# senresearch/BulkLMM.jl

Measured on AMD Instinct MI355X. Metric: trait x marker LOD tests/sec, higher is better.
Workload: dtype f64

## Files before the change

bulklmm.jl_amd/csrc/blmm_api.hip:

```cpp
#include "blmm_internal.h"
#include "fastmath.h"
#include <algorithm>
#include <cmath>
#include <cstddef>
#include <chrono>
#include <cstring>
#include <limits>
#include <cstdlib>
#include <mutex>

using namespace blmm;

namespace blmm {

int fail(blmm_ctx* ctx, int code, const std::string& msg) {
  if (ctx) ctx->err = msg;
  return code;
}

int ensure(blmm_ctx* ctx, DevBuf& b, size_t bytes) {
  if (&b == &ctx->outL) clear_last(ctx);
  if (&b == &ctx->outL || &b == &ctx->outP) ctx->last_P = nullptr;
  if (bytes == 0) bytes = 8;
  if (b.cap >= bytes) return BLMM_OK;
// ... 109 lines not shown
};

void phase_times(const blmm_ctx::EvSet& s, double out[6]) {
  for (int i = 0; i < 6; ++i) out[i] = 0.0;
  for (int i = 0; i + 1 < s.n && i < 5; ++i) { float ms = 0; (void)hipEventElapsedTime(&ms, s.e[i], s.e[i + 1]); out[i] = ms; }
  if (s.n >= 2) { float tot = 0; (void)hipEventElapsedTime(&tot, s.e[0], s.e[s.n - 1]); out[5] = tot; }
}

int to_rowmajor(blmm_ctx* ctx, const double* In, int n, int64_t ncols, double* Out, int npad, int64_t ld) {
  dim3 grid((unsigned)((ld + 31) / 32), (unsigned)((npad + 31) / 32));
  hipLaunchKernelGGL(k_to_rowmajor, grid, dim3(256), 0, ctx->stream, In, n, ncols, Out, npad, ld);
  hipError_t e = hipGetLastError();
  if (e != hipSuccess) return fail(ctx, BLMM_ERR_HIP, std::string("k_to_rowmajor: ") + hipGetErrorString(e));
  return BLMM_OK;
}

int fill(blmm_ctx* ctx, double* p, int64_t n, double v) {
  if (n <= 0) return BLMM_OK;
  hipLaunchKernelGGL(k_fill, dim3((unsigned)((n + 255) / 256)), dim3(256), 0, ctx->stream, p, n, v);
  hipError_t e = hipGetLastError();
  if (e != hipSuccess) return fail(ctx, BLMM_ERR_HIP, std::string("k_fill: ") + hipGetErrorString(e));
  return BLMM_OK;
}

int check_opts(blmm_ctx* ctx, const blmm_opts* o) {
  if (!o) return fail(ctx, BLMM_ERR_INVALID, "opts is NULL");
  if (o->decomp_scheme != BLMM_EIGEN && o->decomp_scheme != BLMM_SVD)
    return fail(ctx, BLMM_ERR_DECOMP, "Please choose either `eigen` or `svd` for decomposition of the kinship matrix.");
  return BLMM_OK;
}

int check_method(blmm_ctx* ctx, const blmm_opts* o) {
  if (o->method != BLMM_NULL_EXACT && o->method != BLMM_NULL_GRID && o->method != BLMM_ALT_GRID)
    return fail(ctx, BLMM_ERR_METHOD, "Unknown method; choose null-exact, null-grid or alt-grid.");
  return BLMM_OK;
}

int reset_stat(blmm_ctx* ctx, int64_t** stat) {
  int rc = ensure(ctx, ctx->stat, sizeof(int64_t) * NSTAT);
  if (rc) return rc;
  *stat = ptr<int64_t>(ctx->stat);
  ctx->audit_ran = false;
  ctx->brent_cnt_used = false;
  BLMM_HIP(hipMemsetAsync(*stat, 0, sizeof(int64_t) * NSTAT, ctx->stream));
  return BLMM_OK;
}

int fill_status(blmm_ctx* ctx, const int64_t* h, blmm_status* st) {
  std::memset(st, 0, sizeof(*st));
  st->n_neg_eig = h[ST_NEG_EIG];
  st->n_nonpos_weight = h[ST_NONPOS_W];
  st->n_zero_norm = h[ST_ZERO_NORM];
  st->n_nan_lod = h[ST_NAN_LOD];
  st->n_brent_maxiter = h[ST_BRENT_MAXIT];
  st->jacobi_sweeps = h[ST_JACOBI_SWEEPS];
  st->jacobi_cycles = h[ST_EIG_CYCLES]; st->jacobi_ticks_100mhz = h[ST_EIG_TICKS];
  st->lowrank_rank = h[ST_LR_RANK];
  st->lowrank_fallback = h[ST_LR_FIX];
  st->lowrank_shared = h[ST_LR_SHARED0] + h[ST_LR_SHARED1];
  st->n_h2_boundary = h[ST_H2_BOUNDARY];
  st->n_h2_multimodal = ctx->audit_ran ? h[ST_H2_MULTIMODAL] : -1;
  st->n_illcond_rescan = h[ST_ILLCOND];
  if (h[ST_LR_RANK] < 0) return fail(ctx, BLMM_ERR_HIP, "weight-basis kernel: a workgroup timed out at the grid barrier");
  if (h[ST_EIG_ABORT] != 0) return fail(ctx, BLMM_ERR_HIP, "the eigensolver did not converge (code " + std::to_string((long long)h[ST_EIG_ABORT]) +
                              ": -7 grid barrier of the tridiagonalisation timed out, -8 QL iteration limit)");
  if (ctx->hflag && *ctx->hflag) return check_sticky(ctx);
  { double r2; std::memcpy(&r2, &h[ST_LR_RESID2], sizeof(double)); st->lowrank_resid = std::sqrt(r2 < 0 ? 0.0 : r2); }
  return BLMM_OK;
}

void add_status(blmm_status* sum, const blmm_status& one) {
  sum->n_neg_eig += one.n_neg_eig; sum->n_nonpos_weight += one.n_nonpos_weight; sum->n_zero_norm += one.n_zero_norm;
  sum->n_nan_lod += one.n_nan_lod; sum->n_brent_maxiter += one.n_brent_maxiter; sum->jacobi_sweeps += one.jacobi_sweeps;
  sum->jacobi_cycles += one.jacobi_cycles; sum->jacobi_ticks_100mhz += one.jacobi_ticks_100mhz;
  sum->lowrank_rank = std::max(sum->lowrank_rank, one.lowrank_rank);
  sum->lowrank_fallback += one.lowrank_fallback; sum->lowrank_shared += one.lowrank_shared;
  sum->lowrank_resid = std::max(sum->lowrank_resid, one.lowrank_resid);
  sum->n_h2_boundary += one.n_h2_boundary; sum->n_h2_multimodal += one.n_h2_multimodal; sum->n_illcond_rescan += one.n_illcond_rescan;
}

double add_phase_times(blmm_status* st, const Timer& tm) {
  if (!tm.set || tm.set->n < 2) return 0.0;
  double t[6];
  phase_times(*tm.set, t);
  st->t_eigen_ms += t[0]; st->t_rotate_ms += t[1]; st->t_h2_ms += t[2]; st->t_prep_ms += t[3]; st->t_scan_ms += t[4];
  return t[5];
}

int finish_status(blmm_ctx* ctx, blmm_status* st, Timer* tm) {
  if (!st) return BLMM_OK;
  int64_t h[NSTAT];
  BLMM_HIP(hipMemcpyAsync(h, ctx->stat.p, sizeof(h), hipMemcpyDeviceToHost, ctx->stream));
  BLMM_HIP(hipStreamSynchronize(ctx->stream));
  int rc = fill_status(ctx, h, st);
  if (rc) return rc;
  if (tm) st->t_total_ms = add_phase_times(st, *tm);
  return BLMM_OK;
}

int end_call(blmm_ctx* ctx, const Pipe& P, blmm_status* st, Timer* tm) {
  if (P.big && ctx->hflag && P.stat) {
    hipLaunchKernelGGL(k_sticky, dim3(1), dim3(1), 0, ctx->stream, P.stat, const_cast<int64_t*>(ctx->hflag));
    hipError_t e = hipGetLastError();
    if (e != hipSuccess) return fail(ctx, BLMM_ERR_HIP, std::string("k_sticky: ") + hipGetErrorString(e));
  }
  return finish_status(ctx, st, tm);
}

struct EigPre { double* Ks; double* V; double* lraw; int64_t* stat; };

struct NullCov { const double* d; int64_t ncov; int add_int; int64_t c; };
NullCov null_cov(const blmm_opts* o, const double* dCovar, int64_t ncov) {
  if (ncov == 0 || !dCovar) return {nullptr, 0, 1, 1};
  const int add_int = o->add_intercept ? 1 : 0;
  return {dCovar, ncov, add_int, ncov + add_int};
}

int prepare_eigen(blmm_ctx* ctx, const blmm_opts* o, int64_t n, const double* dCovar, int64_t ncov, const double* dK,
                  const double* dweights, int centered, Pipe& P, Timer& tm, const EigPre* pre = nullptr) {
  ctx->prep_valid = false;
  if (n < 1 || ncov < 0) return fail(ctx, BLMM_ERR_DIM, "Dimension mismatch.");
  if (n > 2048) return fail(ctx, BLMM_ERR_UNSUPPORTED, "more than 2048 individuals: the device eigensolver (tridiagonalisation + divide and conquer) stops at n = 2048");
  const NullCov nc = null_cov(o, dCovar, ncov);
  const int c = (int)nc.c;
  if (c < 1 || c > CMAX) return fail(ctx, BLMM_ERR_UNSUPPORTED, BLMM_C_ERR);
  if (c >= n) return fail(ctx, BLMM_ERR_DIM, "Dimension mismatch.");
  P.n = (int)n; P.c = c; P.npad = (int)round_up(n, 8); P.ldr = (int)round_up(P.npad, 16);
  int rc;
  if ((rc = ensure(ctx, ctx->U, sizeof(double) * n * n))) return rc;
  if ((rc = ensure(ctx, ctx->lam, sizeof(double) * n))) return rc;
  if ((rc = ensure(ctx, ctx->Zs, sizeof(double) * n * c))) return rc;
  if ((rc = ensure(ctx, ctx->Z0, sizeof(double) * n * c))) return rc;
  if ((rc = ensure(ctx, ctx->Rp, sizeof(double) * (size_t)P.npad * P.ldr))) return rc;
  P.Z0 = ptr<double>(ctx->Z0); P.lam = ptr<double>(ctx->lam);
  if (pre) {
    P.stat = pre->stat;
    ctx->audit_ran = false;
    ctx->brent_cnt_used = false;
    P.big = n > jacobi_lds_max_n();
    bool post_done = false;
    tm.mark();
    if ((rc = launch_jacobi_post(ctx, pre->Ks, pre->V, (int)n, pre->lraw, P.stat, ptr<double>(ctx->Zs), dweights, c, P.npad, P.ldr,
                                 o->decomp_scheme, centered, P.lam, ptr<double>(ctx->U), P.Z0, ptr<double>(ctx->Rp), &post_done))) return rc;
    if (!post_done && (rc = launch_post_eigen(ctx, pre->lraw, pre->V, ptr<double>(ctx->Zs), dweights, (int)n, c, P.npad, P.ldr,
                                              o->decomp_scheme, centered, P.lam, ptr<double>(ctx->U), P.Z0, ptr<double>(ctx->Rp), P.stat))) return rc;
    tm.mark();
    return BLMM_OK;
  }
  if ((rc = ensure(ctx, ctx->Ks, sizeof(double) * n * n))) return rc;
  if ((rc = ensure(ctx, ctx->V, sizeof(double) * (n * n + 4 * n + 16)))) return rc;
  if ((rc = ensure(ctx, ctx->lraw, sizeof(double) * n))) return rc;
  if ((rc = reset_stat(ctx, &P.stat))) return rc;
  tm.mark();
  if ((rc = launch_design(ctx, dK, nc.d, (int)nc.ncov, nc.add_int, dweights, (int)n, ptr<double>(ctx->Ks), ptr<double>(ctx->Zs)))) return rc;
  const double* evec = ptr<double>(ctx->V);
  const char* eig_env = dev_env("BLMM_EIGEN");
  if (!eig_env && ctx->tune.eigen_solver == 1) eig_env = "jacobi";
  if (!eig_env && ctx->tune.eigen_solver == 2) eig_env = "dc";
  const bool big = n > jacobi_lds_max_n();
  P.big = big;
  bool done = false, post_done = false;
  const bool want_dc = eig_env ? std::strcmp(eig_env, "dc") == 0 : big;
  if (!done && want_dc && n >= 3) {
    rc = launch_eig_dc(ctx, ptr<double>(ctx->Ks), (int)n, ptr<double>(ctx->lraw), ptr<double>(ctx->V), P.stat);
    if (rc == BLMM_OK) { done = true; P.big = true; }
    else if (rc != BLMM_ERR_UNSUPPORTED) return rc;
  }
  if (!done) {
    const bool want_fast = !(eig_env && std::strcmp(eig_env, "jacobi") == 0) && n >= 3 && n <= eig_fast_max_n();
    if (want_fast) {
      rc = launch_eig_fast(ctx, ptr<double>(ctx->Ks), (int)n, ptr<double>(ctx->lraw), ptr<double>(ctx->V), P.stat);
      if (rc != BLMM_OK && rc != BLMM_ERR_UNSUPPORTED) return rc;
    }
    if ((rc = launch_jacobi_post(ctx, ptr<double>(ctx->Ks), ptr<double>(ctx->V), (int)n, ptr<double>(ctx->lraw), P.stat, ptr<double>(ctx->Zs),
                                 dweights, c, P.npad, P.ldr, o->decomp_scheme, centered, P.lam, ptr<double>(ctx->U), P.Z0, ptr<double>(ctx->Rp),
                                 &post_done))) return rc;
  }
  if (!post_done && (rc = launch_post_eigen(ctx, ptr<double>(ctx->lraw), evec, ptr<double>(ctx->Zs), dweights, (int)n, c,
                              P.npad, P.ldr, o->decomp_scheme, centered, P.lam, ptr<double>(ctx->U), P.Z0,
                              ptr<double>(ctx->Rp), P.stat))) return rc;
  tm.mark();
  return BLMM_OK;
}

static int flush_upload(blmm_ctx* ctx) {
  if (!ctx->up_pending) return BLMM_OK;
  ctx->up_pending = false;
  for (int i = 0; i < 2; ++i) {
    if (ctx->up_bytes[i]) BLMM_HIP(hipMemcpyAsync(ctx->up_dst[i], ctx->up_src[i], ctx->up_bytes[i], hipMemcpyHostToDevice, ctx->copy));
    if (i == 0) BLMM_HIP(hipEventRecord(ctx->ev_inY, ctx->copy));
  }
  BLMM_HIP(hipEventRecord(ctx->ev_in, ctx->copy));
  ctx->in_wait = true;
  return BLMM_OK;
}

int rotate_markers(blmm_ctx* ctx, Pipe& P, const double* dG, int64_t p);
int start_wbasis(blmm_ctx* ctx, Pipe& P, const double* dG = nullptr, int64_t p = 0, bool xt_recorded = false) {
  int rc;
  const int64_t n = P.n;
  const LrSeg seg = lr_segments(ctx, P.n);
  if ((rc = ensure(ctx, ctx->wbQ, sizeof(double) * (size_t)seg.S * P.npad * n))) return rc;
  if ((rc = ensure(ctx, ctx->wbW, sizeof(double) * (size_t)n * (256 + 16)))) return rc;
  if ((rc = ensure(ctx, ctx->wbRk, sizeof(int) * 4 * LR_SEG_MAX))) return rc;
  if (!xt_recorded) BLMM_HIP(hipEventRecord(ctx->ev_xt, ctx->stream));
  BLMM_HIP(hipStreamWaitEvent(ctx->side, ctx->ev_xt, 0));
  ctx->wb_on_side2 = false;
  if (!dG) {
    OnStream on(ctx, ctx->side);
    return launch_wbasis(ctx, P.lam, (int)n, P.npad, seg, ptr<double>(ctx->wbW), ptr<double>(ctx->wbQ), ptr<int>(ctx->wbRk), P.stat);
  }
  {
    BLMM_HIP(hipStreamWaitEvent(ctx->side2, ctx->ev_xt, 0));
    ctx->wb_on_side2 = true;
    OnStream on(ctx, ctx->side2);
    if ((rc = launch_wbasis(ctx, P.lam, (int)n, P.npad, seg, ptr<double>(ctx->wbW), ptr<double>(ctx->wbQ), ptr<int>(ctx->wbRk), P.stat))) return rc;
  }
  OnStream on(ctx, ctx->side);
  if (ctx->in_wait) BLMM_HIP(hipStreamWaitEvent(ctx->side, ctx->ev_in, 0));
  if ((rc = rotate_markers(ctx, P, dG, p))) return rc;
  BLMM_HIP(hipEventRecord(ctx->ev_wb, ctx->side));
  return BLMM_OK;
}

int rotate_traits(blmm_ctx* ctx, Pipe& P, const double* dY, int64_t m) {
  if (m < 0) return fail(ctx, BLMM_ERR_DIM, "Dimension mismatch.");
  P.m = m; P.ldy = round_up(m > 0 ? m : 1, 128);
  int rc = ensure(ctx, ctx->Yt, sizeof(double) * (size_t)P.npad * P.ldy);
  if (rc) return rc;
  P.Yt = ptr<double>(ctx->Yt);
  return launch_rotate(ctx, ptr<double>(ctx->Rp), P.ldr, P.n, P.npad, dY, m, P.Yt, P.ldy, P.ldy);
}
int rotate_markers(blmm_ctx* ctx, Pipe& P, const double* dG, int64_t p) {
  if (p < 0) return fail(ctx, BLMM_ERR_DIM, "Dimension mismatch.");
  P.p = p; P.ldx = round_up(p > 0 ? p : 1, 128);
  int rc = ensure(ctx, ctx->Xt, sizeof(double) * (size_t)P.npad * P.ldx);
  if (rc) return rc;
  P.Xt = ptr<double>(ctx->Xt);
  return launch_rotate(ctx, ptr<double>(ctx->Rp), P.ldr, P.n, P.npad, dG, p, P.Xt, P.ldx, P.ldx);
}

int prepare(blmm_ctx* ctx, const blmm_opts* o, const double* dY, int64_t n, int64_t m, const double* dG, int64_t p,
            const double* dCovar, int64_t ncov, const double* dK, const double* dweights, int centered, Pipe& P, Timer& tm,
            bool early_wbasis = false, bool grid_side = false, bool skip_markers = false, const EigPre* pre = nullptr) {
  if (m < 0 || p < 0) return fail(ctx, BLMM_ERR_DIM, "Dimension mismatch.");
  const bool forks = m > 0 && p > 0 && (early_wbasis || grid_side);
  ctx->stop_event_used = false;
  ctx->stop_event_next = forks ? ctx->ev_xt : nullptr;
  int rc = prepare_eigen(ctx, o, n, dCovar, ncov, dK, dweights, centered, P, tm, pre);
  const bool xt_recorded = ctx->stop_event_used;
  ctx->stop_event_next = nullptr; ctx->stop_event_used = false;
  if (rc) return rc;
  if (ctx->up_pending) {
    if ((rc = flush_upload(ctx))) return rc;
    BLMM_HIP(hipStreamWaitEvent(ctx->stream, ctx->ev_inY, 0));
  }
  const bool up_flight = ctx->in_wait;
  static const bool rot_side = !(dev_env("BLMM_ROTATE_SIDE") && dev_env("BLMM_ROTATE_SIDE")[0] == '0');
  const bool side_g = early_wbasis && m > 0 && p > 0 && rot_side && n <= 160;
  if (early_wbasis && m > 0 && p > 0 && (rc = start_wbasis(ctx, P, side_g ? dG : nullptr, p, xt_recorded))) return rc;
  P.xt_side = side_g;
  if (grid_side && !early_wbasis && m > 0 && p > 0 && rot_side && n <= 160) {
    if (!xt_recorded) BLMM_HIP(hipEventRecord(ctx->ev_xt, ctx->stream));
    BLMM_HIP(hipStreamWaitEvent(ctx->side, ctx->ev_xt, 0));
    if (ctx->in_wait) BLMM_HIP(hipStreamWaitEvent(ctx->side, ctx->ev_in, 0));
    OnStream on(ctx, ctx->side);
    if ((rc = rotate_markers(ctx, P, dG, p))) return rc;
    P.xt_side = true;
  }
  if ((rc = rotate_traits(ctx, P, dY, m))) return rc;
  if (skip_markers) { P.p = p; P.ldx = round_up(p > 0 ? p : 1, 128); P.Xt = nullptr; }
  else if (!P.xt_side) {
    if (up_flight) BLMM_HIP(hipStreamWaitEvent(ctx->stream, ctx->ev_in, 0));
    if ((rc = rotate_markers(ctx, P, dG, p))) return rc;
  }
  ctx->in_wait = false;
  tm.mark();
  return BLMM_OK;
}

NullModel null_model(const Pipe& P, const blmm_opts* o) {
  NullModel nm;
  nm.n = P.n; nm.c = P.c; nm.npad = P.npad; nm.reml = o->reml ? 1 : 0;
  nm.optim_interval = o->optim_interval < 1 ? 1 : o->optim_interval;
  nm.prior_a = o->prior_variance; nm.prior_b = o->prior_sample_size;
  return nm;
}

int stage_to_device(blmm_ctx* ctx, DevBuf& dst, const void* src, size_t bytes) {
  blmm_ctx::GridSlot* slot = nullptr;
  for (auto& g : ctx->gstage)
    if (g.cap >= bytes && (!g.used || hipEventQuery(g.ev) == hipSuccess)) { slot = &g; break; }
  if (!slot) {
    blmm_ctx::GridSlot g;
    g.cap = bytes < 4096 ? 4096 : bytes;
    void* h = nullptr;
    BLMM_HIP(hipHostMalloc(&h, g.cap, hipHostMallocDefault));
    g.h = h;
    if (hipEventCreateWithFlags(&g.ev, hipEventDisableTiming) != hipSuccess) { (void)hipHostFree(h); return fail(ctx, BLMM_ERR_HIP, "hipEventCreate failed"); }
    ctx->gstage.push_back(g);
    slot = &ctx->gstage.back();
  }
  std::memcpy(slot->h, src, bytes);
  BLMM_HIP(hipMemcpyAsync(dst.p, slot->h, bytes, hipMemcpyHostToDevice, ctx->stream));
  BLMM_HIP(hipEventRecord(slot->ev, ctx->stream));
  slot->used = true;
  return BLMM_OK;
}

int check_grid(blmm_ctx* ctx, const double* h2_grid_host, int64_t ngrid) {
  if (!h2_grid_host || ngrid < 1) return fail(ctx, BLMM_ERR_INVALID, "h2 grid is empty");
  for (int64_t g = 0; g < ngrid; ++g) {
    const double h = h2_grid_host[g];
    if (std::isinf(h / (1.0 - h))) return fail(ctx, BLMM_ERR_H2_ONE, "Heritability of 1 is not allowed.");
  }
  return BLMM_OK;
}

int grid_to_device(blmm_ctx* ctx, const double* h2_grid_host, int64_t ngrid, double** out) {
  int rc;
  if ((rc = check_grid(ctx, h2_grid_host, ngrid)) || (rc = ensure(ctx, ctx->gridd, sizeof(double) * ngrid))) return rc;
  const size_t bytes = sizeof(double) * (size_t)ngrid;
  if (ctx->grid_async) {
    if ((rc = stage_to_device(ctx, ctx->gridd, h2_grid_host, bytes))) return rc;
  } else {
    BLMM_HIP(hipMemcpyAsync(ctx->gridd.p, h2_grid_host, bytes, hipMemcpyHostToDevice, ctx->stream));
    BLMM_HIP(hipStreamSynchronize(ctx->stream));
  }
  *out = ptr<double>(ctx->gridd);
  return BLMM_OK;
}

ScanArgs scan_args(blmm_ctx* ctx, const Pipe& P, const double* panels, int64_t ldp, double* L, int64_t ldL, int64_t m) {
  ScanArgs a;
  a.Xt = P.Xt; a.ldx = P.ldx; a.P = panels; a.ldp = ldp; a.pstride = (int64_t)P.npad * ldp;
  a.ks = P.npad / 4; a.n = P.n; a.p = P.p; a.m = m; a.L = L; a.ldL = ldL;
  a.isx = nullptr; a.ld_isx = 0; a.bin = nullptr; a.stat = P.stat; a.logtab = ptr<double>(ctx->logtab); a.lodtab = ptr<double>(ctx->lodtab);
  a.Pv = ctx->pv_cur; a.ldPv = ctx->pv_cur_ld; a.pvtab = ptr<double>(ctx->pvtab);
  a.red = ctx->red_cur;
  a.c = P.c;
  lod_poly5_host(-0.5 * (double)P.n, a.lodc);
  return a;
}

double lr_tolerance(const blmm_ctx* ctx) {
  const char* e = dev_env("BLMM_LR_TOL");
  return e ? atof(e) : ctx->tune.lr_tol;
}

int64_t lr_ldq(const Pipe& P) { return P.ldy + 128 + LR_TILE * LR_SEG_MAX; }
static LrRegion lr_region(const Pipe& P, int r) {
  LrRegion rg;
  rg.col0 = r * lr_ldq(P); rg.ncol = lr_ldq(P); rg.counts = P.stat + ST_LR_SHARED0 + 2 * r; rg.segcnt = P.stat + 24 + 20 * r;
  return rg;
}

int lr_begin(blmm_ctx* ctx, const Pipe& P, bool wbasis_started) {
  int rc;
  ctx->lr_last_ldq = lr_ldq(P); ctx->lr_last_m = P.m;
  const int64_t ldp = 2 * lr_ldq(P), tstride = (int64_t)P.npad * P.ldx;
  if ((rc = ensure(ctx, ctx->lrPerm, sizeof(int) * (size_t)ldp))) return rc;
  if ((rc = ensure(ctx, ctx->lrDen0, sizeof(double) * (size_t)P.ldx))) return rc;
  const LrSeg seg = lr_segments(ctx, P.n);
  if ((rc = ensure(ctx, ctx->lrT, sizeof(double) * (size_t)seg.S * (1 + P.c) * tstride))) return rc;
  if ((rc = ensure(ctx, ctx->lrC, sizeof(double) * (size_t)P.npad * ldp))) return rc;
  if ((rc = ensure(ctx, ctx->lrL, sizeof(double) * (size_t)(P.c * (P.c + 1) / 2) * ldp))) return rc;
  if ((rc = ensure(ctx, ctx->lrFlag, sizeof(int) * (size_t)ldp))) return rc;
  if ((rc = ensure(ctx, ctx->lrPart, sizeof(double) * 2 * (size_t)((P.n + 63) / 64) * ldp))) return rc;
  if ((rc = ensure(ctx, ctx->panels, sizeof(double) * (size_t)P.npad * ldp))) return rc;
  if ((rc = ensure(ctx, ctx->wbQ, sizeof(double) * (size_t)seg.S * P.npad * P.n))) return rc;
  if ((rc = ensure(ctx, ctx->wbW, sizeof(double) * (size_t)P.n * (256 + 16)))) return rc;
  if ((rc = ensure(ctx, ctx->wbRk, sizeof(int) * 4 * LR_SEG_MAX))) return rc;
  int* rk = ptr<int>(ctx->wbRk);
  if (!(wbasis_started && P.xt_side)) {
    BLMM_HIP(hipEventRecord(ctx->ev_fork, ctx->stream));
    BLMM_HIP(hipStreamWaitEvent(ctx->side, ctx->ev_fork, 0));
  }
  const bool on2 = wbasis_started && P.xt_side && ctx->wb_on_side2;
  hipStream_t lr_side = on2 ? ctx->side2 : ctx->side;
  OnStream on(ctx, lr_side);
  if (!wbasis_started && (rc = launch_wbasis(ctx, P.lam, P.n, P.npad, seg, ptr<double>(ctx->wbW), ptr<double>(ctx->wbQ), rk, P.stat))) return rc;
  BLMM_HIP(hipEventRecord(ctx->ev_q, lr_side));
  if (on2) BLMM_HIP(hipStreamWaitEvent(lr_side, ctx->ev_wb, 0));
  if ((rc = launch_lr_tpanels(ctx, P.Xt, P.ldx, P.p, P.n, P.c, P.npad, P.Z0, ptr<double>(ctx->wbQ), rk, seg, ptr<double>(ctx->lrT), tstride,
                              ptr<double>(ctx->lrDen0)))) return rc;
  BLMM_HIP(hipEventRecord(ctx->ev_join, lr_side));
  return BLMM_OK;
}

namespace {
double lr_shared_tol(const blmm_ctx* ctx) {
  const char* e = dev_env("BLMM_LR_SHARED");
  const bool on = e ? e[0] != '0' : ctx->tune.lr_shared != 0;
  return on ? lr_tolerance(ctx) : 0.0;
}
LrArgs lr_args(blmm_ctx* ctx, const Pipe& P, const LrRegion& rg, double* dL, int64_t ldL) {
  const int64_t ldp = 2 * lr_ldq(P);
  LrArgs la;
  la.s = scan_args(ctx, P, ptr<double>(ctx->panels), ldp, dL, ldL, P.m + 192 < rg.ncol ? P.m + 192 : rg.ncol);
  la.Cp = ptr<double>(ctx->lrC); la.T = ptr<double>(ctx->lrT); la.tstride = (int64_t)P.npad * P.ldx; la.Ls = ptr<double>(ctx->lrL);
  la.rk = ptr<int>(ctx->wbRk); la.c = P.c; la.perm = ptr<int>(ctx->lrPerm); la.rg = rg; la.den0 = ptr<double>(ctx->lrDen0);
  la.skip_shared = 0;
  la.seg = lr_segments(ctx, P.n);
  return la;
}
int lr_region_scan(blmm_ctx* ctx, const Pipe& P, const LrRegion& rg, double* dL, int64_t ldL) {
  static const bool lean = !(dev_env("BLMM_LR_LEAN") && dev_env("BLMM_LR_LEAN")[0] == '0');
  static const bool serial = dev_env("BLMM_LR_SERIAL") && dev_env("BLMM_LR_SERIAL")[0] == '1';
  if (serial) { (void)hipStreamSynchronize(ctx->side); (void)hipStreamSynchronize(ctx->side2); (void)hipStreamSynchronize(ctx->stream); }
  LrArgs la = lr_args(ctx, P, rg, dL, ldL);
  int rc;
  if (lean) {
    ScanArgs a = la.s;
    a.isx = la.den0; a.ld_isx = P.ldx; a.bin = nullptr;
    a.perm = la.perm; a.col0 = rg.col0; a.count = rg.counts;
    if ((rc = launch_scan_shared(ctx, a))) return rc;
    la.skip_shared = 1;
  }
  return launch_scan_lr(ctx, la);
}
int lr_region_panels(blmm_ctx* ctx, const Pipe& P, const NullModel& nm, const double* dh2, const LrRegion& rg) {
  return launch_lr_panels(ctx, nm, P.Yt, P.ldy, P.m, P.Z0, P.lam, dh2, ptr<double>(ctx->wbQ), ptr<int>(ctx->wbRk), lr_segments(ctx, P.n), ptr<int>(ctx->lrPerm),
                          rg, ptr<double>(ctx->panels), ptr<double>(ctx->lrC), ptr<double>(ctx->lrL), 2 * lr_ldq(P), P.stat);
// ... 173 lines not shown
      ensure(ctx, ctx->lodtab, sizeof(blmm_lod_table_host)) != BLMM_OK ||
      hipMemcpy(ctx->lodtab.p, blmm_lod_table_host, sizeof(blmm_lod_table_host), hipMemcpyHostToDevice) != hipSuccess ||
      ensure(ctx, ctx->pvtab, sizeof(blmm_pv_table_host)) != BLMM_OK ||
      hipMemcpy(ctx->pvtab.p, blmm_pv_table_host, sizeof(blmm_pv_table_host), hipMemcpyHostToDevice) != hipSuccess) {
    blmm_destroy(ctx);
    return BLMM_ERR_HIP;
  }
  *out = ctx;
  return BLMM_OK;
}

void blmm_destroy(blmm_ctx* ctx) {
  if (!ctx) return;
  hipSetDevice(ctx->device);
  hipStreamSynchronize(ctx->stream);
  DevBuf* bufs[] = {&ctx->Ks, &ctx->V, &ctx->lam, &ctx->U, &ctx->Zs, &ctx->Z0, &ctx->Rp, &ctx->Yt, &ctx->Xt, &ctx->panels,
                    &ctx->iyy, &ctx->h2, &ctx->h2idx, &ctx->sig2, &ctx->ell, &ctx->isx, &ctx->stat, &ctx->gridd, &ctx->misc,
                    &ctx->EllTab, &ctx->inY, &ctx->inG, &ctx->inK, &ctx->inCov, &ctx->inW, &ctx->outL, &ctx->outH2,
                    &ctx->tmpA, &ctx->tmpB, &ctx->tmpC, &ctx->perm, &ctx->r0, &ctx->altbuf, &ctx->logtab, &ctx->lraw,
                    &ctx->wbQ, &ctx->wbW, &ctx->wbRk, &ctx->lrT, &ctx->lrC, &ctx->lrL, &ctx->lrFlag, &ctx->lrPart, &ctx->lrPerm, &ctx->lrDen0, &ctx->eigW, &ctx->xf32, &ctx->pf32, &ctx->brSt, &ctx->brList, &ctx->illList, &ctx->qrSlab, &ctx->lodtab, &ctx->dynFac, &ctx->pvtab, &ctx->outP, &ctx->redbuf, &ctx->redtrip, &ctx->altC, &ctx->rf32, &ctx->btG, &ctx->redflag, &ctx->bperm,
                    &ctx->locoK, &ctx->locoPart, &ctx->locoChr, &ctx->locoStat, &ctx->locoKs, &ctx->locoV, &ctx->locoLraw,
                    &ctx->locoCmx, &ctx->locoCarg, &ctx->locoPerm, &ctx->mdfR, &ctx->mdfT, &ctx->mdfScr,
                    &ctx->effX, &ctx->effIdx, &ctx->effWork, &ctx->effOut, &ctx->effSlab, &ctx->condIdx, &ctx->condWork,
                    &ctx->stepWork, &ctx->stepOut, &ctx->condScr};
  for (DevBuf* b : bufs) if (b->p) hipFree(b->p);
  for (auto& s : ctx->evsets) for (auto& e : s.e) (void)hipEventDestroy(e);
  if (ctx->side) { (void)hipStreamSynchronize(ctx->side); (void)hipStreamDestroy(ctx->side); }
  if (ctx->ev_fork) (void)hipEventDestroy(ctx->ev_fork);
  if (ctx->ev_join) (void)hipEventDestroy(ctx->ev_join);
  if (ctx->ev_xt) (void)hipEventDestroy(ctx->ev_xt);
  if (ctx->ev_b1) (void)hipEventDestroy(ctx->ev_b1);
  if (ctx->ev_b2) (void)hipEventDestroy(ctx->ev_b2);
  if (ctx->ev_q) (void)hipEventDestroy(ctx->ev_q);
  if (ctx->ev_m) (void)hipEventDestroy(ctx->ev_m);
  if (ctx->ev_wb) (void)hipEventDestroy(ctx->ev_wb);
  if (ctx->ev_in) (void)hipEventDestroy(ctx->ev_in);
  if (ctx->ev_inY) (void)hipEventDestroy(ctx->ev_inY);
  if (ctx->ev_call) (void)hipEventDestroy(ctx->ev_call);
  for (auto& g : ctx->gstage) {
    if (g.ev) { (void)hipEventSynchronize(g.ev); (void)hipEventDestroy(g.ev); }
    if (g.h) (void)hipHostFree(g.h);
  }
  if (ctx->copy) { (void)hipStreamSynchronize(ctx->copy); (void)hipStreamDestroy(ctx->copy); }
  if (ctx->side2) { (void)hipStreamSynchronize(ctx->side2); (void)hipStreamDestroy(ctx->side2); }
  if (ctx->own_stream) hipStreamDestroy(ctx->stream);
  if (ctx->hflag) (void)hipHostFree(const_cast<int64_t*>(ctx->hflag));
  destroy_host_stage(ctx->hstage);
  delete ctx;
}

const char* blmm_last_error(const blmm_ctx* ctx) { return ctx ? ctx->err.c_str() : "ctx is NULL"; }

int blmm_set_stream(blmm_ctx* ctx, void* hip_stream) {
  if (!ctx) return BLMM_ERR_INVALID;
  hipStreamSynchronize(ctx->stream);
  if (ctx->own_stream) { hipStreamDestroy(ctx->stream); ctx->own_stream = false; }
  if (hip_stream == BLMM_STREAM_NULL) ctx->stream = nullptr;
  else if (hip_stream) ctx->stream = reinterpret_cast<hipStream_t>(hip_stream);
  else {
    if (hipStreamCreateWithFlags(&ctx->stream, hipStreamNonBlocking) != hipSuccess) return fail(ctx, BLMM_ERR_HIP, "hipStreamCreate");
    ctx->own_stream = true;
  }
  return BLMM_OK;
}

int blmm_set_timing(blmm_ctx* ctx, int on) {
  if (!ctx) return BLMM_ERR_INVALID;
  ctx->timing = on != 0;
  return BLMM_OK;
}

int blmm_read_timings(blmm_ctx* ctx, double* sums_ms, int64_t* ncalls) {
  if (!ctx || !sums_ms || !ncalls) return BLMM_ERR_INVALID;
  BLMM_HIP(hipStreamSynchronize(ctx->stream));
  for (int i = 0; i < 6; ++i) sums_ms[i] = 0.0;
  for (size_t k = 0; k < ctx->ev_used; ++k) {
    double t[6];
    phase_times(ctx->evsets[k], t);
    for (int i = 0; i < 6; ++i) sums_ms[i] += t[i];
  }
  *ncalls = (int64_t)ctx->ev_used;
  ctx->ev_used = 0;
  return BLMM_OK;
}

int blmm_lowrank_profile(blmm_ctx* ctx, int64_t* out) {
  if (!ctx || !out) return BLMM_ERR_INVALID;
  for (int i = 0; i < 2 + 2 * LR_SEG_MAX; ++i) out[i] = 0;
  if (!ctx->stat.p || !ctx->wbRk.p) return BLMM_OK;
  BLMM_HIP(hipSetDevice(ctx->device));
  int64_t h[NSTAT];
  int rk[4 * LR_SEG_MAX];
  BLMM_HIP(hipMemcpyAsync(h, ctx->stat.p, sizeof(h), hipMemcpyDeviceToHost, ctx->stream));
  BLMM_HIP(hipMemcpyAsync(rk, ctx->wbRk.p, sizeof(rk), hipMemcpyDeviceToHost, ctx->stream));
  BLMM_HIP(hipStreamSynchronize(ctx->stream));
  int S = 0;
  for (int s = 0; s < LR_SEG_MAX; ++s) {
    const int64_t cnt = h[24 + s] + h[44 + s];
    if (cnt > 0) { S = s + 1; out[2 + 2 * s] = cnt; out[3 + 2 * s] = rk[4 * s]; }
  }
  out[0] = S; out[1] = h[ST_LR_SHARED0] + h[ST_LR_SHARED1];
  return BLMM_OK;
}

int blmm_lowrank_columns(blmm_ctx* ctx, int64_t m, int32_t* col_out, int64_t* region_width, int64_t* counts_out) {
  if (!ctx || !col_out || m < 0) return BLMM_ERR_INVALID;
  for (int64_t j = 0; j < m; ++j) col_out[j] = -1;
  if (region_width) *region_width = ctx->lr_last_ldq;
  if (counts_out) for (int i = 0; i < 4; ++i) counts_out[i] = 0;
  if (!ctx->lrPerm.p || !ctx->stat.p || ctx->lr_last_ldq <= 0) return BLMM_OK;
  BLMM_HIP(hipSetDevice(ctx->device));
  const int64_t ldq = ctx->lr_last_ldq;
  std::vector<int> perm((size_t)(2 * ldq));
  int64_t h[NSTAT];
  BLMM_HIP(hipMemcpyAsync(perm.data(), ctx->lrPerm.p, sizeof(int) * perm.size(), hipMemcpyDeviceToHost, ctx->stream));
  BLMM_HIP(hipMemcpyAsync(h, ctx->stat.p, sizeof(h), hipMemcpyDeviceToHost, ctx->stream));
  BLMM_HIP(hipStreamSynchronize(ctx->stream));
  for (int r = 0; r < 2; ++r) {
    const int64_t nsh = h[ST_LR_SHARED0 + 2 * r], noth = h[ST_LR_OTHER0 + 2 * r];
    if (counts_out) { counts_out[2 * r] = nsh; counts_out[2 * r + 1] = noth; }
    for (int64_t cidx = 0; cidx < ldq; ++cidx) {
      if (!(cidx < nsh || cidx >= ldq - noth)) continue;
      const int t = perm[(size_t)(r * ldq + cidx)];
      if (t >= 0 && t < m) col_out[t] = (int32_t)(r * ldq + cidx);
    }
  }
  return BLMM_OK;
}

int blmm_synchronize(blmm_ctx* ctx) {
  if (!ctx) return BLMM_ERR_INVALID;
  BLMM_HIP(hipStreamSynchronize(ctx->stream));
  return check_sticky(ctx);
}

void blmm_default_opts(blmm_opts* o) {
  if (!o) return;
  std::memset(o, 0, sizeof(*o));
  o->method = BLMM_NULL_GRID; o->reml = 0; o->add_intercept = 1; o->decomp_scheme = BLMM_EIGEN;
  o->optim_interval = 1; o->compat_flags = 0; o->prior_variance = 1.0; o->prior_sample_size = 0.0;
}

static const struct { const char* key; int kind; size_t off; double lo, hi; } kTune[] = {
  {"lr_tol", 0, offsetof(blmm::Tuning, lr_tol), 0.0, 1.0},
  {"illcond_rho", 0, offsetof(blmm::Tuning, illcond_rho), 0.0, 1e300},
  {"exact_full_rank", 1, offsetof(blmm::Tuning, exact_full_rank), 0, 1},
  {"pval_libm", 1, offsetof(blmm::Tuning, pval_libm), 0, 1},
  {"pval_fused", 1, offsetof(blmm::Tuning, pval_fused), 0, 1},
  {"lr_segments", 1, offsetof(blmm::Tuning, lr_segments), 0, LR_SEG_MAX},
  {"lr_shared", 1, offsetof(blmm::Tuning, lr_shared), 0, 1},
  {"lr_split", 1, offsetof(blmm::Tuning, lr_split), -1, 1},
  {"eigen_solver", 1, offsetof(blmm::Tuning, eigen_solver), 0, 2},
  {"f32_rotation", 1, offsetof(blmm::Tuning, f32_rotation), 0, 1},
  {"bulk_perm_cols", 1, offsetof(blmm::Tuning, bulk_perm_cols), 0, 2147483647.0},
  {"mdf_red_chunk", 1, offsetof(blmm::Tuning, mdf_red_chunk), 0, 2147483647.0},
  {"cond_red_chunk", 1, offsetof(blmm::Tuning, cond_red_chunk), 0, 2147483647.0},
};
int blmm_set_tuning(blmm_ctx* ctx, const char* key, double value) {
  if (!ctx) return BLMM_ERR_INVALID;
  if (!key) return fail(ctx, BLMM_ERR_INVALID, "set_tuning: key is NULL");
  if (std::strcmp(key, "defaults") == 0) { ctx->tune = blmm::Tuning(); return BLMM_OK; }
  for (const auto& t : kTune)
    if (std::strcmp(key, t.key) == 0) {
      if (!(value >= t.lo && value <= t.hi) || (t.kind == 1 && value != std::floor(value)))
        return fail(ctx, BLMM_ERR_INVALID, std::string("set_tuning: value out of range for ") + key);
      char* base = reinterpret_cast<char*>(&ctx->tune) + t.off;
      if (t.kind == 0) *reinterpret_cast<double*>(base) = value; else *reinterpret_cast<int*>(base) = (int)value;
      return BLMM_OK;
    }
  return fail(ctx, BLMM_ERR_INVALID, std::string("set_tuning: unknown key ") + key);
}
int blmm_get_tuning(const blmm_ctx* ctx, const char* key, double* value) {
  if (!ctx || !key || !value) return BLMM_ERR_INVALID;
  for (const auto& t : kTune)
    if (std::strcmp(key, t.key) == 0) {
      const char* base = reinterpret_cast<const char*>(&ctx->tune) + t.off;
      *value = t.kind == 0 ? *reinterpret_cast<const double*>(base) : (double)*reinterpret_cast<const int*>(base);
      return BLMM_OK;
    }
  return BLMM_ERR_INVALID;
}

int blmm_kinship_dev(blmm_ctx* ctx, const double* dG, int64_t n, int64_t p, double* dK_out) {
  if (!ctx) return BLMM_ERR_INVALID;
  if (!dG || !dK_out || n < 1 || p < 1) return fail(ctx, BLMM_ERR_INVALID, "calcKinship: bad arguments");
  BLMM_HIP(hipSetDevice(ctx->device));
  int rc = ensure(ctx, ctx->tmpA, sizeof(double) * (size_t)64 * n * n);
  if (rc) return rc;
  return launch_kinship(ctx, dG, n, p, dK_out, ptr<double>(ctx->tmpA));
}

__global__ void k_round_digits(double* __restrict__ v, int64_t cnt, double scale) {
  const int64_t i = (int64_t)blockIdx.x * blockDim.x + threadIdx.x;
  if (i < cnt) v[i] = rint(v[i] * scale) / scale;
}

int blmm_kinship_rounded(blmm_ctx* ctx, const double* G, int64_t n, int64_t p, int64_t digits, double* K_out) {
  if (!ctx) return BLMM_ERR_INVALID;
  if (!G || !K_out || n < 1 || p < 1 || digits > 300) return fail(ctx, BLMM_ERR_INVALID, "calcKinship: bad arguments");
  HostCall hc(ctx);
  int rc;
  if ((rc = hc.begin()) || (rc = ensure(ctx, ctx->inK, sizeof(double) * n * n)) || (rc = hc.up(ctx->inG, G, sizeof(double) * n * p))) return rc;
  if ((rc = blmm_kinship_dev(ctx, ptr<double>(ctx->inG), n, p, ptr<double>(ctx->inK)))) return rc;
  if (digits >= 0 && digits <= 17)
    hipLaunchKernelGGL(k_round_digits, dim3((unsigned)((n * n + 255) / 256)), dim3(256), 0, ctx->stream, ptr<double>(ctx->inK), n * n, std::pow(10.0, (double)digits));
  if ((rc = hc.down(K_out, ctx->inK.p, sizeof(double) * n * n))) return rc;
  return hc.finish();
}

int blmm_kinship(blmm_ctx* ctx, const double* G, int64_t n, int64_t p, double* K_out) {
  return blmm_kinship_rounded(ctx, G, n, p, -1, K_out);
}

int blmm_lod_colmax_dev(blmm_ctx* ctx, const double* dL, int64_t p, int64_t m, int64_t ldL, double* dmax_out, int64_t* dargmax_out) {
  if (!ctx) return BLMM_ERR_INVALID;
  if (!dL || !dmax_out || p < 1 || m < 0 || ldL < p) return fail(ctx, BLMM_ERR_INVALID, "lod_colmax: bad arguments");
  BLMM_HIP(hipSetDevice(ctx->device));
  return launch_colmax(ctx, dL, p, m, ldL, dmax_out, dargmax_out);
}

int blmm_lod_colmax(blmm_ctx* ctx, const double* L, int64_t p, int64_t m, double* max_out, int64_t* argmax_out) {
  if (!ctx) return BLMM_ERR_INVALID;
  if (!L || !max_out || p < 1 || m < 0) return fail(ctx, BLMM_ERR_INVALID, "lod_colmax: bad arguments");
  HostCall hc(ctx);
  const size_t mm = m > 0 ? m : 1;
  int rc;
  if ((rc = hc.begin()) || (rc = hc.up(ctx->outL, L, sizeof(double) * (size_t)p * m)) || (rc = ensure(ctx, ctx->tmpA, sizeof(double) * mm)) ||
      (rc = ensure(ctx, ctx->tmpB, sizeof(int64_t) * mm))) return rc;
  if (m > 0) set_last(ctx, ptr<double>(ctx->outL), p, m);
  if ((rc = launch_colmax(ctx, ptr<double>(ctx->outL), p, m, p, ptr<double>(ctx->tmpA), ptr<int64_t>(ctx->tmpB))) ||
      (rc = hc.down(max_out, ctx->tmpA.p, sizeof(double) * (size_t)m)) || (rc = hc.down(argmax_out, ctx->tmpB.p, sizeof(int64_t) * (size_t)m)))
    return rc;
  return hc.finish();
}

int blmm_lod2log10p(blmm_ctx* ctx, const double* L, int64_t p, int64_t m, int64_t chisq_df, double* P_out) {
  if (!ctx) return BLMM_ERR_INVALID;
  if (!L || !P_out || p < 0 || m < 0 || chisq_df < 1 || chisq_df > 1000000) return fail(ctx, BLMM_ERR_INVALID, "lod2log10p: bad arguments");
  if ((size_t)p * m == 0) return BLMM_OK;
  HostCall hc(ctx);
  int rc;
  if ((rc = hc.begin()) || (rc = ensure(ctx, ctx->altbuf, sizeof(double) * (size_t)p * m * 2))) return rc;
  double* dL = ptr<double>(ctx->altbuf);
  double* dP = dL + (size_t)p * m;
  if ((rc = hc.up(dL, L, sizeof(double) * (size_t)p * m)) || (rc = launch_lod2log10p(ctx, dL, p, m, p, (int)chisq_df, dP, p)) ||
      (rc = copy_to_host(ctx, P_out, dP, sizeof(double) * (size_t)p * m))) return rc;
  return hc.finish(false);
}

int blmm_lod_threshold(blmm_ctx* ctx, const double* L, int64_t p, int64_t m, double thr, int64_t cap, int32_t* i_out,
                       int32_t* j_out, double* lod_out, int64_t* count_out) {
  if (!ctx) return BLMM_ERR_INVALID;
  if (!L || p < 1 || m < 1) return fail(ctx, BLMM_ERR_INVALID, "lod_threshold: bad arguments");
  HostCall hc(ctx);
  int rc;
  if ((rc = hc.begin()) || (rc = hc.up(ctx->outL, L, sizeof(double) * (size_t)p * m))) return rc;
  set_last(ctx, ptr<double>(ctx->outL), p, m);
  if ((rc = blmm_last_lod_threshold(ctx, thr, cap, i_out, j_out, lod_out, count_out))) return rc;
  return hc.finish(false);
}

int blmm_get_thresholds(blmm_ctx* ctx, const double* Lperms, int64_t p, int64_t nperms, const double* probs, int64_t nprobs,
                        double* thrs_out) {
  if (!ctx) return BLMM_ERR_INVALID;
  if (!Lperms || p < 1 || nperms < 1) return fail(ctx, BLMM_ERR_INVALID, "get_thresholds: bad arguments");
  HostCall hc(ctx);
  int rc;
  if ((rc = hc.begin()) || (rc = hc.up(ctx->altbuf, Lperms, sizeof(double) * (size_t)p * nperms)) ||
      (rc = blmm_get_thresholds_dev(ctx, ptr<double>(ctx->altbuf), p, nperms, p, probs, nprobs, thrs_out))) return rc;
  return hc.finish(false);
}

extern "C++" {
namespace {
struct PvReq { bool armed = false; double* out = nullptr; int64_t ld = 0, df = 1; };
PvReq pv_take(blmm_ctx* ctx) {
  PvReq r; r.armed = ctx->pv_armed; r.out = ctx->pv_out; r.ld = ctx->pv_ld; r.df = ctx->pv_df;
  ctx->pv_armed = false; ctx->pv_out = nullptr; ctx->pv_ld = 0; ctx->pv_df = 1;
  return r;
}
void pv_hand_over(blmm_ctx* ctx, const PvReq& r) {
  ctx->pv_armed = r.armed; ctx->pv_out = r.out; ctx->pv_ld = r.ld; ctx->pv_df = r.df;
}
struct PvCall {
  blmm_ctx* ctx; PvReq req; double* P = nullptr; int64_t ld = 0; bool fused = false, owned = false;
  PvCall(blmm_ctx* c, const PvReq& r) : ctx(c), req(r) {}
  ~PvCall() { ctx->pv_cur = nullptr; ctx->pv_cur_ld = 0; }
  int resolve(int64_t p, int64_t m) {
    if (!req.armed) return BLMM_OK;
    if (p <= 0 || m <= 0) return BLMM_OK;
    P = req.out; ld = req.ld;
    if (P && ld < p) { P = nullptr; return fail(ctx, BLMM_ERR_INVALID, "log10p output: ldP < p"); }
    if (!P) {
      int rc = ensure(ctx, ctx->outP, sizeof(double) * (size_t)p * (size_t)m);
      if (rc) return rc;
      P = ptr<double>(ctx->outP); ld = p; owned = true;
    }
    return BLMM_OK;
  }
  int begin(const Pipe& Pp, const blmm_opts* o) {
    int rc = resolve(Pp.p, Pp.m);
    if (rc || !P) return rc;
    const char* pf = dev_env("BLMM_PVAL_FUSED");
    fused = req.df == 1 && o->method != BLMM_ALT_GRID && (pf ? pf[0] != '0' : ctx->tune.pval_fused != 0);
    if (fused) { ctx->pv_cur = P; ctx->pv_cur_ld = ld; }
    return BLMM_OK;
  }
  int finish(int64_t p, int64_t m, const double* dL, int64_t ldL) {
    ctx->pv_cur = nullptr; ctx->pv_cur_ld = 0;
    if (!P) return BLMM_OK;
    if (!fused) { int rc = launch_lod2log10p(ctx, dL, p, m, ldL, (int)req.df, P, ld); if (rc) return rc; }
    if (owned) { ctx->last_P = P; ctx->last_P_ld = ld; ctx->last_P_df = req.df; }
    return BLMM_OK;
  }
};
}
}

static int isx_maybe_side(blmm_ctx* ctx, const Pipe& P, const NullModel& nm, const double* dgrid, int ngrid) {
  int rc;
  if ((rc = ensure(ctx, ctx->isx, sizeof(double) * (size_t)ngrid * P.ldx))) return rc;
  {
    OnStream on(ctx, P.xt_side ? ctx->side : ctx->stream);
    if ((rc = launch_isx(ctx, nm, P.Xt, P.ldx, P.p, P.Z0, P.lam, dgrid, ngrid, ptr<double>(ctx->isx), P.ldx, P.stat))) return rc;
  }
  if (P.xt_side) {
    BLMM_HIP(hipEventRecord(ctx->ev_join, ctx->side));
    BLMM_HIP(hipStreamWaitEvent(ctx->stream, ctx->ev_join, 0));
  }
  return BLMM_OK;
}

static int scan_pipeline(blmm_ctx* ctx, const blmm_opts* opts, Pipe& P, Timer& tm, bool lowrank, bool wbasis_started, double* dgrid,
                         const double* h2_grid_host, int64_t ngrid, double* dL_out, int64_t ldL, double* dh2_out, blmm_status* status,
                         const PvReq& pvreq, int64_t ldH = -1) {
  int rc;
  const int64_t m = P.m, p = P.p;
  const NullModel nm = null_model(P, opts);
  const int64_t ldp = P.ldy;
  PvCall pvc(ctx, pvreq);
  if ((rc = pvc.begin(P, opts))) return rc;
  if (m == 0) { tm.mark(); tm.mark(); tm.mark(); return end_call(ctx, P, status, &tm); }
  if (p == 0) {
    if (opts->method == BLMM_NULL_EXACT) {
      if ((rc = launch_brent(ctx, nm, P.Yt, P.ldy, m, P.Z0, P.lam, dh2_out, nullptr, nullptr, P.stat))) return rc;
    } else if (opts->method == BLMM_NULL_GRID) {
      if ((rc = ensure(ctx, ctx->h2idx, sizeof(int) * (size_t)m))) return rc;
      if ((rc = launch_loglik_grid(ctx, nm, P.Yt, P.ldy, m, P.Z0, P.lam, dgrid, (int)ngrid, nullptr, ptr<int>(ctx->h2idx), dh2_out, P.stat))) return rc;
    }
    tm.mark(); tm.mark(); tm.mark();
    return end_call(ctx, P, status, &tm);
  }

  if (opts->method == BLMM_NULL_EXACT) {
    if (lowrank) {
      if ((rc = lr_begin(ctx, P, wbasis_started))) return rc;
      const char* split_env = dev_env("BLMM_LR_SPLIT");
      const bool split_on = (ctx->red_cur.flags && P.c >= 2) ? false
                          : split_env ? split_env[0] != '0' : (ctx->tune.lr_split < 0 ? m >= 8192 : ctx->tune.lr_split != 0);
      BrentSplit sp;
      if ((rc = launch_brent(ctx, nm, P.Yt, P.ldy, m, P.Z0, P.lam, dh2_out, nullptr, nullptr, P.stat, split_on ? 1 : 0, &sp))) return rc;
      tm.mark();
      if (sp.active) { if ((rc = lr_finish_split(ctx, P, nm, dh2_out, dL_out, ldL, tm, sp))) return rc; }
      else if ((rc = lr_finish(ctx, P, nm, dh2_out, dL_out, ldL, tm))) return rc;
    } else {
      if ((rc = launch_brent(ctx, nm, P.Yt, P.ldy, m, P.Z0, P.lam, dh2_out, nullptr, nullptr, P.stat))) return rc;
      tm.mark();
      if ((rc = ensure(ctx, ctx->panels, sizeof(double) * (size_t)(2 + P.c) * P.npad * ldp))) return rc;
      if ((rc = launch_panels(ctx, nm, P.Yt, P.ldy, m, P.Z0, P.lam, dh2_out, 1, ptr<double>(ctx->panels), ldp, P.stat))) return rc;
      tm.mark();
      ScanArgs a = scan_args(ctx, P, ptr<double>(ctx->panels), ldp, dL_out, ldL, m);
      if ((rc = launch_scan_exact(ctx, a, P.c))) return rc;
      if ((rc = illcond_rescan(ctx, P, nm, m, dh2_out, dL_out, ldL))) return rc;
      tm.mark();
    }
    if (opts->compat_flags & BLMM_FLAG_H2_AUDIT) {
      double gridh[16];
      for (int g = 0; g < 16; ++g) gridh[g] = g / 16.0;
      double* dg = nullptr;
      if ((rc = grid_to_device(ctx, gridh, 16, &dg))) return rc;
      if ((rc = ensure(ctx, ctx->EllTab, sizeof(double) * (size_t)16 * m))) return rc;
      if ((rc = launch_loglik_grid(ctx, nm, P.Yt, P.ldy, m, P.Z0, P.lam, dg, 16, ptr<double>(ctx->EllTab), nullptr, nullptr, P.stat))) return rc;
      if ((rc = launch_h2_audit(ctx, ptr<double>(ctx->EllTab), 16, m, P.stat))) return rc;
      ctx->audit_ran = true;
    }
  } else if (opts->method == BLMM_NULL_GRID) {
    if ((rc = ensure(ctx, ctx->h2idx, sizeof(int) * (size_t)m))) return rc;
    if ((rc = launch_loglik_grid(ctx, nm, P.Yt, P.ldy, m, P.Z0, P.lam, dgrid, (int)ngrid, nullptr, ptr<int>(ctx->h2idx), dh2_out, P.stat))) return rc;
    tm.mark();
    if ((rc = ensure(ctx, ctx->panels, sizeof(double) * (size_t)P.npad * ldp))) return rc;
    if ((rc = launch_panels(ctx, nm, P.Yt, P.ldy, m, P.Z0, P.lam, dh2_out, 0, ptr<double>(ctx->panels), ldp, P.stat))) return rc;
    if ((rc = isx_maybe_side(ctx, P, nm, dgrid, (int)ngrid))) return rc;
    tm.mark();
    ScanArgs a = scan_args(ctx, P, ptr<double>(ctx->panels), ldp, dL_out, ldL, m);
    a.isx = ptr<double>(ctx->isx); a.ld_isx = P.ldx; a.bin = ptr<int>(ctx->h2idx);
    if ((rc = launch_scan_table(ctx, a))) return rc;
    tm.mark();
  } else {
    if ((rc = ensure(ctx, ctx->EllTab, sizeof(double) * (size_t)ngrid * m))) return rc;
    if ((rc = launch_loglik_grid(ctx, nm, P.Yt, P.ldy, m, P.Z0, P.lam, dgrid, (int)ngrid, ptr<double>(ctx->EllTab), nullptr, nullptr, P.stat))) return rc;
    tm.mark();
    if ((rc = ensure(ctx, ctx->panels, sizeof(double) * (size_t)ngrid * P.npad * ldp))) return rc;
    if ((rc = ensure(ctx, ctx->h2, sizeof(double) * (size_t)m))) return rc;
    if (nm.c <= CTPL) {
      if ((rc = launch_panels(ctx, nm, P.Yt, P.ldy, m, P.Z0, P.lam, nullptr, 0, ptr<double>(ctx->panels), ldp, P.stat, dgrid, (int)ngrid))) return rc;
    } else {
      for (int64_t g = 0; g < ngrid; ++g) {
        if ((rc = fill(ctx, ptr<double>(ctx->h2), m, h2_grid_host[g]))) return rc;
        if ((rc = launch_panels(ctx, nm, P.Yt, P.ldy, m, P.Z0, P.lam, ptr<double>(ctx->h2), 0,
                                ptr<double>(ctx->panels) + (size_t)g * P.npad * ldp, ldp, P.stat))) return rc;
      }
    }
    if ((rc = isx_maybe_side(ctx, P, nm, dgrid, (int)ngrid))) return rc;
    if ((rc = ensure(ctx, ctx->altC, sizeof(double) * (size_t)ngrid * m))) return rc;
    if ((rc = launch_alt_ctab(ctx, ptr<double>(ctx->EllTab), (int)ngrid, m, P.n, ptr<double>(ctx->altC)))) return rc;
    tm.mark();
    AltArgs aa;
    aa.s = scan_args(ctx, P, ptr<double>(ctx->panels), ldp, dL_out, ldL, m);
    aa.s.isx = ptr<double>(ctx->isx); aa.s.ld_isx = P.ldx;
    aa.ngrid = (int)ngrid; aa.EllTab = ptr<double>(ctx->EllTab); aa.grid_dev = dgrid; aa.H2 = dh2_out; aa.ldH = ldH < 0 ? p : ldH;
    aa.Ctab = ptr<double>(ctx->altC);
    aa.counter_quirk = (opts->compat_flags & BLMM_COMPAT_ALT_COUNTER) ? 1 : 0;
    if ((rc = launch_scan_alt(ctx, aa))) return rc;
    tm.mark();
  }
  if ((rc = pvc.finish(p, m, dL_out, ldL))) return rc;
  return end_call(ctx, P, status, &tm);
}

int blmm_set_log10p_output(blmm_ctx* ctx, double* dP_out, int64_t ldP, int64_t chisq_df) {
  if (!ctx) return BLMM_ERR_INVALID;
  if (chisq_df < 0 || chisq_df > 1000000 || (dP_out && ldP < 1)) return fail(ctx, BLMM_ERR_INVALID, "set_log10p_output: bad arguments");
  ctx->pv_armed = chisq_df > 0;
  ctx->pv_out = dP_out; ctx->pv_ld = ldP; ctx->pv_df = chisq_df > 0 ? chisq_df : 1;
  return BLMM_OK;
}

static bool exact_full(const blmm_ctx* ctx) {
  const char* e = dev_env("BLMM_EXACT");
  return e ? std::strcmp(e, "full") == 0 : ctx->tune.exact_full_rank != 0;
}
static bool lowrank_form(const blmm_ctx* ctx, int c, int64_t n) { return !exact_full(ctx) && c <= 3 && n <= 6000; }
static bool wants_lowrank(const blmm_ctx* ctx, const blmm_opts* opts, int64_t n, const double* dCovar, int64_t ncov) {
  return opts->method == BLMM_NULL_EXACT && lowrank_form(ctx, (int)null_cov(opts, dCovar, ncov).c, n);
}

static int bulkscan_dev_impl(blmm_ctx* ctx, const blmm_opts* opts, const double* dY, int64_t n, int64_t m, const double* dG,
                             int64_t p, const double* dCovar, int64_t ncov, const double* dK, const double* dweights,
                             const double* h2_grid_host, int64_t ngrid, double* dL_out, int64_t ldL, double* dh2_out,
                             blmm_status* status, const PvReq& pvreq) {
  int rc = check_opts(ctx, opts);
  if (rc) return rc;
  if (!dY || !dG || !dK || (!dL_out && !ctx->red_cur.pmax) || !dh2_out) return fail(ctx, BLMM_ERR_INVALID, "bulkscan: NULL buffer");
  if (ldL < p) return fail(ctx, BLMM_ERR_INVALID, "bulkscan: ldL < p");
  if ((rc = check_method(ctx, opts)) || (rc = enter_device(ctx))) return rc;
  Timer tm(ctx);
  Pipe P;
  double* dgrid = nullptr;
  if (opts->method != BLMM_NULL_EXACT) {
    if ((rc = grid_to_device(ctx, h2_grid_host, ngrid, &dgrid))) return rc;
  }
  const bool lowrank = wants_lowrank(ctx, opts, n, dCovar, ncov);
  if ((rc = prepare(ctx, opts, dY, n, m, dG, p, dCovar, ncov, dK, dweights, 1, P, tm, lowrank, opts->method != BLMM_NULL_EXACT))) return rc;
  return scan_pipeline(ctx, opts, P, tm, lowrank,  lowrank && m > 0 && p > 0, dgrid, h2_grid_host, ngrid, dL_out, ldL, dh2_out, status, pvreq);
}

int blmm_bulkscan_dev(blmm_ctx* ctx, const blmm_opts* opts, const double* dY, int64_t n, int64_t m, const double* dG,
                      int64_t p, const double* dCovar, int64_t ncov, const double* dK, const double* dweights,
                      const double* h2_grid_host, int64_t ngrid, double* dL_out, int64_t ldL, double* dh2_out,
                      blmm_status* status) {
  if (!ctx) return BLMM_ERR_INVALID;
  const PvReq pvreq = pv_take(ctx);
  ctx->red_cur = RedArgs();
  return bulkscan_dev_impl(ctx, opts, dY, n, m, dG, p, dCovar, ncov, dK, dweights, h2_grid_host, ngrid, dL_out, ldL, dh2_out, status, pvreq);
}

static int reduced_check(blmm_ctx* ctx, const blmm_opts* opts, const double* dY, int64_t n, int64_t m, const double* dG, int64_t p,
                         const double* dK, const blmm_reduced* out, const double* dh2_out, const char* who) {
  int rc = check_opts(ctx, opts);
  if (rc) return rc;
  if (!out || !dY || !dG || !dK || (!dh2_out && opts->method != BLMM_ALT_GRID)) return fail(ctx, BLMM_ERR_INVALID, std::string(who) + ": NULL buffer");
  if (out->cap < 0 || (out->cap > 0 && (!out->ti || !out->tj || !out->tlod)) || (out->want_triplets && !out->count))
    return fail(ctx, BLMM_ERR_INVALID, std::string(who) + ": triplet buffers");
  if ((rc = check_method(ctx, opts))) return rc;
  if (n < 1 || m < 0 || p < 0 || p > 0x7fffffffLL || m > 0x7fffffffLL) return fail(ctx, BLMM_ERR_DIM, "Dimension mismatch.");
  return BLMM_OK;
}

static int red_state(blmm_ctx* ctx, const blmm_reduced* out, int64_t nslot, int64_t m, RedArgs* r) {
  const int64_t ldm = round_up(m, 64);
  int rc = ensure(ctx, ctx->redbuf, (sizeof(double) + sizeof(int)) * (size_t)nslot * (size_t)ldm);
  if (rc) return rc;
  r->pmax = ptr<double>(ctx->redbuf); r->parg = reinterpret_cast<int*>(r->pmax + (size_t)nslot * ldm); r->ldm = ldm;
  r->want_trip = out->want_triplets ? 1 : 0; r->thr = out->thr; r->cap = out->cap;
  r->ti = out->ti; r->tj = out->tj; r->tl = out->tlod; r->cnt = reinterpret_cast<unsigned long long*>(out->count);
  if (out->count) BLMM_HIP(hipMemsetAsync(out->count, 0, sizeof(int64_t), ctx->stream));
  return BLMM_OK;
}
static int reduced_args(blmm_ctx* ctx, const blmm_reduced* out, int64_t p, int64_t m, RedArgs* r, int* nslot) {
  *nslot = 2 * (int)((p + 127) / 128);
  return red_state(ctx, out, *nslot, m, r);
}

static int reduced_resident(blmm_ctx* ctx, const blmm_opts* opts, const double* dY, int64_t n, int64_t m, const double* dG, int64_t p,
                            const double* dCovar, int64_t ncov, const double* dK, const double* dweights, const double* h2_grid_host,
                            int64_t ngrid, const blmm_reduced* out, double* dh2_out, blmm_status* status) {
  const int64_t ldL = p > 0 ? p : 1;
  const size_t pm = (size_t)ldL * (size_t)(m > 0 ? m : 1);
  int rc;
  if ((rc = ensure(ctx, ctx->outL, sizeof(double) * pm))) return rc;
  double* dL = ptr<double>(ctx->outL);
  double* dH = dh2_out;
  if (opts->method == BLMM_ALT_GRID) {
    if ((rc = ensure(ctx, ctx->altbuf, sizeof(double) * pm))) return rc;
    dH = ptr<double>(ctx->altbuf);
  }
  if ((rc = bulkscan_dev_impl(ctx, opts, dY, n, m, dG, p, dCovar, ncov, dK, dweights, h2_grid_host, ngrid, dL, ldL, dH, status, PvReq()))) return rc;
  if (m > 0) set_last(ctx, dL, p, m);
  if (out->colmax && m > 0 && (rc = launch_colmax(ctx, dL, p, m, ldL, out->colmax, out->argmax))) return rc;
  if (out->want_triplets && (rc = launch_threshold(ctx, dL, p, m, ldL, out->thr, out->cap, out->ti, out->tj, out->tlod, out->count))) return rc;
  return BLMM_OK;
}

static int reduced_impl(blmm_ctx* ctx, const blmm_opts* opts, const double* dY, int64_t n, int64_t m, const double* dG, int64_t p,
                        const double* dCovar, int64_t ncov, const double* dK, const double* dweights, const double* h2_grid_host,
                        int64_t ngrid, const blmm_reduced* out, double* dh2_out, blmm_status* status, int* route_out) {
  int rc = reduced_check(ctx, opts, dY, n, m, dG, p, dK, out, dh2_out, "bulkscan_reduced");
  if (rc) return rc;
  BLMM_HIP(hipSetDevice(ctx->device));
  const bool native = p > 0 && m > 0 && (opts->method == BLMM_NULL_GRID || wants_lowrank(ctx, opts, n, dCovar, ncov));
  if (route_out) *route_out = 0;
  if (native) {
    RedArgs r;
    int nslot;
    if ((rc = reduced_args(ctx, out, p, m, &r, &nslot))) return rc;
    ctx->red_cur = r;
    rc = bulkscan_dev_impl(ctx, opts, dY, n, m, dG, p, dCovar, ncov, dK, dweights, h2_grid_host, ngrid, nullptr, p, dh2_out, status, PvReq());
    ctx->red_cur = RedArgs();
    if (rc) { (void)hipStreamSynchronize(ctx->stream); return rc; }
    if ((rc = launch_red_final(ctx, r, nslot, m, out->colmax, out->argmax))) return rc;
    int64_t h[NSTAT];
    BLMM_HIP(hipMemcpyAsync(h, ctx->stat.p, sizeof(h), hipMemcpyDeviceToHost, ctx->stream));
    BLMM_HIP(hipStreamSynchronize(ctx->stream));
    if ((rc = check_sticky(ctx))) return rc;
    if (h[ST_LR_FIX] == 0 && h[ST_ILLCOND] == 0) { if (route_out) *route_out = 1; return BLMM_OK; }
  }
  if ((rc = reduced_resident(ctx, opts, dY, n, m, dG, p, dCovar, ncov, dK, dweights, h2_grid_host, ngrid, out, dh2_out, status))) {
    (void)hipStreamSynchronize(ctx->stream);
    return rc;
  }
  BLMM_HIP(hipStreamSynchronize(ctx->stream));
  if (route_out) *route_out = 2;
  return check_sticky(ctx);
}

int blmm_bulkscan_reduced_dev(blmm_ctx* ctx, const blmm_opts* opts, const double* dY, int64_t n, int64_t m, const double* dG,
                              int64_t p, const double* dCovar, int64_t ncov, const double* dK, const double* dweights,
                              const double* h2_grid_host, int64_t ngrid, const blmm_reduced* out, double* dh2_out,
                              blmm_status* status) {
  if (!ctx) return BLMM_ERR_INVALID;
  (void)pv_take(ctx);
  return reduced_impl(ctx, opts, dY, n, m, dG, p, dCovar, ncov, dK, dweights, h2_grid_host, ngrid, out, dh2_out, status, &ctx->last_reduced_route);
}

int blmm_prepare_dev(blmm_ctx* ctx, const blmm_opts* opts, int64_t n, const double* dCovar, int64_t ncov, const double* dK,
                     const double* dweights, blmm_status* status) {
  if (!ctx) return BLMM_ERR_INVALID;
  int rc = check_opts(ctx, opts);
  if (rc) return rc;
  if (!dK) return fail(ctx, BLMM_ERR_INVALID, "prepare: NULL buffer");
  if ((rc = enter_device(ctx))) return rc;
  ctx->prep_valid = false;
  Timer tm(ctx);
  Pipe P;
  if ((rc = prepare_eigen(ctx, opts, n, dCovar, ncov, dK, dweights, 1, P, tm))) return rc;
  ctx->prep = P;
  ctx->prep_valid = true;
  return end_call(ctx, P, status, &tm);
}

static Pipe prepared_pipe(blmm_ctx* ctx) {
  Pipe P = ctx->prep;
  P.Z0 = ptr<double>(ctx->Z0); P.lam = ptr<double>(ctx->lam); P.stat = ptr<int64_t>(ctx->stat);
  P.Yt = nullptr; P.Xt = nullptr;
  return P;
}

int64_t blmm_rotated_rows(const blmm_ctx* ctx) { return (ctx && ctx->prep_valid) ? ctx->prep.npad : 0; }

int blmm_rotate_block_dev(blmm_ctx* ctx, const double* dG_block, int64_t pb, double* dXt_block, int64_t ld) {
  if (!ctx) return BLMM_ERR_INVALID;
  if (!ctx->prep_valid) return fail(ctx, BLMM_ERR_INVALID, "rotate_block: blmm_prepare_dev has not run on this context");
  if (!dG_block || !dXt_block || pb < 0 || ld < pb) return fail(ctx, BLMM_ERR_INVALID, "rotate_block: bad arguments");
  BLMM_HIP(hipSetDevice(ctx->device));
  const Pipe P = prepared_pipe(ctx);
  return launch_rotate(ctx, ptr<double>(ctx->Rp), P.ldr, P.n, P.npad, dG_block, pb, dXt_block, ld, ld);
}

static int assemble_prerotated(blmm_ctx* ctx, Pipe& P, int64_t p, const double* dXt_blocks, int64_t nblocks, int64_t block_cols,
                               int64_t block_ld) {
  int rc;
  P.p = p; P.ldx = round_up(p > 0 ? p : 1, 128);
  if ((rc = ensure(ctx, ctx->Xt, sizeof(double) * (size_t)P.npad * P.ldx))) return rc;
  P.Xt = ptr<double>(ctx->Xt);
  if (P.ldx > p) BLMM_HIP(hipMemset2DAsync(P.Xt + p, sizeof(double) * P.ldx, 0, sizeof(double) * (P.ldx - p), P.npad, ctx->stream));
  for (int64_t b = 0; b < nblocks; ++b) {
    const int64_t lo = b * block_cols, hi = (lo + block_cols < p) ? lo + block_cols : p;
    if (hi <= lo) break;
    BLMM_HIP(hipMemcpy2DAsync(P.Xt + lo, sizeof(double) * P.ldx, dXt_blocks + (size_t)b * P.npad * block_ld, sizeof(double) * block_ld,
                              sizeof(double) * (hi - lo), P.npad, hipMemcpyDeviceToDevice, ctx->stream));
  }
  return BLMM_OK;
}

static int reset_prepared(blmm_ctx* ctx, const Pipe& P, Timer& tm) {
  BLMM_HIP(hipMemsetAsync(P.stat + ST_NONPOS_W, 0, sizeof(int64_t) * (ST_JACOBI_SWEEPS - ST_NONPOS_W), ctx->stream));
// ... 1971 lines not shown
```

bulklmm.jl_amd/csrc/blmm_internal.h:

```cpp
#pragma once
#include <hip/hip_runtime.h>
#include <hip/hip_ext.h>
#include <stdint.h>
#include <stdlib.h>
#include <string>
#include <vector>
#include "../../include/bulklmm_hip.h"

namespace blmm {

typedef double d2 __attribute__((ext_vector_type(2)));
typedef double d4 __attribute__((ext_vector_type(4)));

constexpr int CMAX = 32;
constexpr int CTPL = 8;
constexpr int CFAST = 4;
#define BLMM_C_ERR "number of null covariates (incl. intercept) must be 1..32"
#define BLMM_FOR_EACH_C(M) \
  case 1: M(1); break; case 2: M(2); break; case 3: M(3); break; case 4: M(4); break; \
  case 5: M(5); break; case 6: M(6); break; case 7: M(7); break; case 8: M(8); break;
constexpr int TILE_T = 64;
constexpr int TILE_I = 128;
constexpr int NSTAT = 64;

enum StatIdx { ST_NEG_EIG = 0, ST_NONPOS_W = 1, ST_ZERO_NORM = 2, ST_NAN_LOD = 3, ST_BRENT_MAXIT = 4, ST_JACOBI_SWEEPS = 5,
               ST_EIG_CYCLES = 6, ST_EIG_TICKS = 7 ,
               ST_LR_RANK = 8 ,
               ST_LR_RESID2 = 9 , ST_LR_FIX = 10 ,
               ST_EIG_ABORT = 11 ,
               ST_LR_SHARED0 = 12, ST_LR_OTHER0 = 13, ST_LR_SHARED1 = 14, ST_LR_OTHER1 = 15
               ,
               ST_H2_BOUNDARY = 16, ST_H2_MULTIMODAL = 17, ST_ILLCOND = 18,
               ST_EIG_FAST = 19 , ST_EIG_BAD = 20 ,
               ST_BRENT_CNT = 21 ,
               ST_EIG_DONE = 23  };

inline int64_t round_up(int64_t x, int64_t q) { return (x + q - 1) / q * q; }

inline const char* dev_env(const char* name) {
  const char* on = getenv("BLMM_DEV_ENV");
  return (on && on[0] == '1') ? getenv(name) : nullptr;
}
struct Tuning {
  double lr_tol = 1e-13;
  double illcond_rho = 1e-4;
  int exact_full_rank = 0;
  int pval_libm = 0;
  int pval_fused = 1;
  int lr_segments = 0;
  int lr_shared = 1;
  int lr_split = -1;
  int f32_rotation = 1;
  int eigen_solver = 0;
  int mdf_red_chunk = 0;
  int cond_red_chunk = 0;
  int bulk_perm_cols = 0;
};

struct DevBuf {
  void* p = nullptr;
  size_t cap = 0;
};

struct Pipe {
  int n = 0, c = 0, npad = 0, ldr = 0;
  int64_t m = 0, p = 0, ldy = 0, ldx = 0;
  double *Yt = nullptr, *Xt = nullptr, *Z0 = nullptr, *lam = nullptr;
  int64_t* stat = nullptr;
  bool big = false;
  bool xt_side = false;
};

struct RedArgs {
  double* pmax = nullptr; int* parg = nullptr; int64_t ldm = 0;
  int want_trip = 0; double thr = 0.0; int64_t cap = 0;
  int32_t* ti = nullptr; int32_t* tj = nullptr; double* tl = nullptr; unsigned long long* cnt = nullptr;
  int* flags = nullptr;
  int64_t row0 = 0;
};
}

namespace blmm { struct HostStage; }

struct blmm_ctx {
  int device = 0;
  hipStream_t stream = nullptr;
  bool own_stream = false;
  bool timing = false;
  std::string err;
  blmm::DevBuf Ks, V, lam, U, Zs, Z0, Rp, Yt, Xt, panels, iyy, h2, h2idx, sig2, ell, isx, stat, gridd, misc, EllTab,
      inY, inG, inK, inCov, inW, outL, outH2, tmpA, tmpB, tmpC, perm, r0, altbuf, logtab, lraw, wbQ, wbW, wbRk, lrT, lrC, lrL, lrFlag, lrPart, lrPerm, lrDen0, eigW, xf32, pf32, brSt, brList, illList, qrSlab, lodtab, dynFac, pvtab, outP, redbuf, redtrip, altC, rf32, btG, redflag, bperm,
      locoK, locoPart, locoChr, locoStat, locoKs, locoV, locoLraw,
      locoCmx, locoCarg,
      locoPerm,
      mdfR, mdfT,
      mdfScr,
      condIdx, condWork,
      stepWork, stepOut, condScr,
      effX, effIdx, effWork, effOut, effSlab;
  struct EvSet { hipEvent_t e[8]; int n; };
  std::vector<EvSet> evsets;
  size_t ev_used = 0;
  hipStream_t side = nullptr, side2 = nullptr;
  hipEvent_t ev_fork = nullptr, ev_join = nullptr, ev_xt = nullptr, ev_b1 = nullptr, ev_b2 = nullptr, ev_q = nullptr, ev_m = nullptr, ev_wb = nullptr;
  hipEvent_t stop_event_next = nullptr; bool stop_event_used = false;
  bool wb_on_side2 = false;
  hipStream_t copy = nullptr; hipEvent_t ev_in = nullptr, ev_inY = nullptr;
  bool up_pending = false, in_wait = false;
  const void* up_src[2] = {nullptr, nullptr}; void* up_dst[2] = {nullptr, nullptr}; size_t up_bytes[2] = {0, 0};
  int num_cus = 0;
  volatile int64_t* hflag = nullptr;
  const double* last_L = nullptr; int64_t last_p = 0, last_m = 0; bool last_f32 = false;
  bool pv_armed = false; double* pv_out = nullptr; int64_t pv_ld = 0, pv_df = 1;
  double* pv_cur = nullptr; int64_t pv_cur_ld = 0;
  const double* last_P = nullptr; int64_t last_P_ld = 0, last_P_df = 0;
  blmm::RedArgs red_cur; int last_reduced_route = 0;
  bool grid_async = false;
  struct GridSlot { void* h = nullptr; size_t cap = 0; hipEvent_t ev = nullptr; bool used = false; };
  std::vector<GridSlot> gstage;
  hipEvent_t ev_call = nullptr;
  blmm::Tuning tune;
  bool perm_ready = false; int perm_ready_n = 0; int64_t perm_ready_nperms = 0; uint64_t perm_ready_seed = 0;
  int64_t lr_last_ldq = 0, lr_last_m = 0;
  blmm::Pipe prep; bool prep_valid = false;
  bool brent_cnt_used = false;
  bool audit_ran = false;
  int eig_plan_n = -1;
  blmm::HostStage* hstage = nullptr;
};

namespace blmm {

inline void set_last(blmm_ctx* ctx, const double* L, int64_t p, int64_t m, bool f32 = false) {
  ctx->last_L = L; ctx->last_p = p; ctx->last_m = m; ctx->last_f32 = f32;
}
inline void clear_last(blmm_ctx* ctx) { set_last(ctx, nullptr, 0, 0); }

int fail(blmm_ctx* ctx, int code, const std::string& msg);
#define BLMM_HIP(call)                                                                              \
  do {                                                                                              \
    hipError_t e__ = (call);                                                                        \
    if (e__ != hipSuccess)                                                                          \
      return blmm::fail(ctx, BLMM_ERR_HIP, std::string(#call) + ": " + hipGetErrorString(e__));     \
  } while (0)

int ensure(blmm_ctx* ctx, DevBuf& b, size_t bytes);
struct GridKernelGuard {
  blmm_ctx* ctx; int dev; int rc = 0;
  explicit GridKernelGuard(blmm_ctx* c);
  int record();
  ~GridKernelGuard();
  GridKernelGuard(const GridKernelGuard&) = delete;
  GridKernelGuard& operator=(const GridKernelGuard&) = delete;
};
int copy_to_host(blmm_ctx* ctx, void* dst, const void* dsrc, size_t bytes);
struct HostCall {
  blmm_ctx* ctx;
  bool done = false;
  explicit HostCall(blmm_ctx* c) : ctx(c) {}
  ~HostCall();
  HostCall(const HostCall&) = delete;
  HostCall& operator=(const HostCall&) = delete;
  int begin();
  int up(void* dst, const void* src, size_t bytes);
  int up(DevBuf& b, const void* src, size_t bytes);
  int up_opt(DevBuf& b, const double* src, int64_t count, const double** dev);
  int defer_yg(const double* Y, size_t ybytes, const double* G, size_t gbytes);
  struct In { const double *Y, *G, *K, *Cov, *W; int64_t ncov; };
  int inputs(const double* Y, int64_t n, int64_t m, const double* G, int64_t p, const double* K, const double* Covar, int64_t ncov,
             const double* weights, bool defer, In* in);
  int down(void* dst, const void* dsrc, size_t bytes);
  int finish(bool sync = true);
};
void destroy_host_stage(HostStage* hs);
template <typename T>
inline T* ptr(DevBuf& b) { return reinterpret_cast<T*>(b.p); }

struct Design {
  int n = 0, c = 0, npad = 0;
  int ldr = 0;
};

int launch_design(blmm_ctx* ctx, const double* dK, const double* dCovar, int ncov, int add_intercept,
                  const double* dweights, int n, double* Ks, double* Zs);
struct PostEigenArgs;
int launch_jacobi(blmm_ctx* ctx, double* A, double* V, int n, double* lraw, int64_t* stat, const PostEigenArgs* pe = nullptr, bool* fused = nullptr);
int launch_jacobi_post(blmm_ctx* ctx, double* A, double* V, int n, double* lraw, int64_t* stat, const double* Zs, const double* dweights,
                       int c, int npad, int ldr, int decomp, int centered, double* lam, double* U, double* Z0, double* Rp, bool* fused);
int launch_eig_dc(blmm_ctx* ctx, const double* A, int n, double* lraw, double* evec, int64_t* stat);
int eig_dc_max_n(const blmm_ctx* ctx);
int launch_eig_fast(blmm_ctx* ctx, const double* A, int n, double* lraw, double* evec, int64_t* stat);
int launch_eig_fast_batch(blmm_ctx* ctx, const double* A, int64_t sA, int n, int nb, double* lraw, int64_t sL, double* evec, int64_t sE,
                          int64_t* stat, int64_t sS);
int eig_fast_max_n();
int jacobi_lds_max_n();
int launch_post_eigen(blmm_ctx* ctx, const double* lraw, const double* V, const double* Zs, const double* dweights, int n,
                      int c, int npad, int ldr, int decomp, int centered, double* lam, double* U, double* Z0, double* Rp,
                      int64_t* stat);
int launch_rotate(blmm_ctx* ctx, const double* Rp, int ldr, int n, int npad, const double* In, int64_t ncols,
                  double* Out, int64_t ldo, int64_t ncols_pad);
int launch_rotate_single(blmm_ctx* ctx, const double* Rp, int ldr, int n, int npad, const double* In, int64_t ncols, double* Out, int64_t ldo);
int launch_untranspose(blmm_ctx* ctx, const double* In, int64_t ld, int n, int64_t ncols, double* Out);

struct NullModel {
  int n, c, npad, reml, optim_interval;
  double prior_a, prior_b;
};
struct BrentSplit {
  bool active = false;
  const int* fin = nullptr;
  const int* list = nullptr;
  const unsigned int* cnt = nullptr;
};
int launch_brent(blmm_ctx* ctx, const NullModel& nm, const double* Yt, int64_t ldy, int64_t m, const double* Z0,
                 const double* lam, double* h2, double* sigma2, double* ell, int64_t* stat, int phase = 0,
                 BrentSplit* sp = nullptr);
int launch_alt_brent(blmm_ctx* ctx, const NullModel& nm, const double* Yt, int64_t ldy, const double* Xt, int64_t ldx, int64_t p,
                     const double* Z0, const double* lam, const double* h2null, int true_w, double* lod, double* h2each,
                     int64_t* stat, int64_t m = 1, int64_t ldL = 0, int64_t ldH = 0);
int launch_loglik_grid(blmm_ctx* ctx, const NullModel& nm, const double* Yt, int64_t ldy, int64_t m, const double* Z0,
                       const double* lam, const double* grid_dev, int ngrid, double* EllTab, int* h2idx, double* h2,
                       int64_t* stat);
int launch_h2_audit(blmm_ctx* ctx, const double* EllTab, int ngrid, int64_t m, int64_t* stat);
int launch_panels(blmm_ctx* ctx, const NullModel& nm, const double* Yt, int64_t ldy, int64_t m, const double* Z0,
                  const double* lam, const double* h2, int full, double* panels, int64_t ldp, int64_t* stat,
                  const double* gridv = nullptr, int ngrid = 0);
int launch_isx(blmm_ctx* ctx, const NullModel& nm, const double* Xt, int64_t ldx, int64_t p, const double* Z0,
               const double* lam, const double* grid_dev, int ngrid, double* isx, int64_t ld_isx, int64_t* stat);
int launch_kinship(blmm_ctx* ctx, const double* dG, int64_t n, int64_t p, double* dK, double* partial);
int loco_kinship_splits(int64_t n, int64_t nchr);
int launch_kinship_loco(blmm_ctx* ctx, const double* dG, int64_t n, const int64_t* dchr, int64_t nchr, int64_t digits, double* dK,
                        double* partial, int nsplit);
int launch_colmax(blmm_ctx* ctx, const double* L, int64_t p, int64_t m, int64_t ldL, double* mx, int64_t* arg);
int launch_colmax_rows(blmm_ctx* ctx, const double* L, int64_t p, int64_t m, int64_t ldL, double* mx, int64_t* arg, int64_t row0);
int launch_lod2log10p(blmm_ctx* ctx, const double* dL, int64_t p, int64_t m, int64_t ldL, int df, double* dP, int64_t ldP);
int launch_perm_gen(blmm_ctx* ctx, int n, int64_t nperms, uint64_t seed);
int launch_perm_panel(blmm_ctx* ctx, const NullModel& nm, const double* Yt, int64_t ldy, const double* Z0,
                      const double* lam, const double* h2, const int32_t* perm_idx, int64_t nperms, uint64_t seed,
                      int orig, double* panel, int64_t ldp, int64_t* stat);

struct ScanArgs {
  const double* Xt; int64_t ldx;
  const double* P; int64_t ldp; int64_t pstride;
  int ks;
  int n;
  int64_t p, m;
  double* L; int64_t ldL;
  const double* isx; int64_t ld_isx; const int* bin;
  const int* perm = nullptr; int64_t col0 = 0; const int64_t* count = nullptr;
  int c = 1;
  const double* logtab;
  const double* lodtab;
  double lodc[6];
  int64_t* stat;
  double* Pv = nullptr; int64_t ldPv = 0; const double* pvtab = nullptr;
  RedArgs red;
  const int* cflag = nullptr; int64_t* cinfo = nullptr;
};
int launch_threshold(blmm_ctx* ctx, const double* dL, int64_t p, int64_t m, int64_t ldL, double thr, int64_t cap,
                     int32_t* di, int32_t* dj, double* dlod, int64_t* dcount);
int launch_threshold_rows(blmm_ctx* ctx, const double* dL, int64_t p, int64_t m, int64_t ldL, double thr, int64_t cap,
                          int32_t* di, int32_t* dj, double* dlod, int64_t* dcount, int64_t row0);
int launch_red_final(blmm_ctx* ctx, const RedArgs& r, int nslot, int64_t m, double* mx, int64_t* arg);
int launch_red_final_loco(blmm_ctx* ctx, const double* pmax, const int* parg, int64_t ldm, const int64_t* dchr, int64_t nchr, int64_t m,
                          double* cmx, int64_t* carg, double* mx, int64_t* arg);
int launch_red_info(blmm_ctx* ctx, const int64_t* stat, int route, const int64_t* count, int64_t* info);
int launch_scan_exact(blmm_ctx* ctx, const ScanArgs& a, int c);
int launch_scan_cond(blmm_ctx* ctx, const ScanArgs& a, int ct);
constexpr int LR_TILE = 64;
struct LrRegion {
  int64_t col0 = 0, ncol = 0;
  int64_t* counts = nullptr;
  int64_t* segcnt = nullptr;
};
constexpr int LR_SEG_MAX = 8;
struct LrSeg {
  int S = 1;
  double edge[LR_SEG_MAX + 1] = {0.0, 2.0, 2.0, 2.0, 2.0, 2.0, 2.0, 2.0, 2.0};
};
__host__ __device__ inline int64_t lr_seg_width(int64_t cnt) { return (cnt + LR_TILE - 1) / LR_TILE * LR_TILE; }
__host__ __device__ inline int lr_seg_of(int64_t dist, const int64_t* segcnt, int S) {
  for (int s = 0; s + 1 < S; ++s) {
    const int64_t w = lr_seg_width(segcnt[s]);
    if (dist < w) return s;
    dist -= w;
  }
  return S - 1;
}
struct LrArgs {
  ScanArgs s;
  const double* Cp;
  const double* T; int64_t tstride;
  const double* Ls;
  const int* rk;
  LrSeg seg;
  const int* perm;
  LrRegion rg;
  const double* den0;
  int skip_shared;
  int c;
};
int launch_scan_lr(blmm_ctx* ctx, const LrArgs& la);
int launch_lr_resid(blmm_ctx* ctx, const NullModel& nm, int64_t m, double tol, const double* lam, const double* h2,
                    const double* Q, const int* rk, const LrSeg& seg, const int* perm, const LrRegion& rg, const double* Cp, int64_t ldp,
                    int* flag_list, double* part, int64_t* stat, int* flags = nullptr);
int launch_scan_fix(blmm_ctx* ctx, const NullModel& nm, const double* Xt, int64_t ldx, int64_t p, const double* P0,
                    const double* Ls, int64_t ldp, const double* Z0, const double* lam, const double* h2,
                    const int* flag_list, const int* perm, double* L, int64_t ldL, int64_t* stat, const RedArgs& red = RedArgs());
int launch_lr_classify(blmm_ctx* ctx, int n, int64_t m, double tol, const double* lam, const double* h2, const int* fin,
                       const int* list, const unsigned int* list_cnt, int* perm, const LrRegion& rg, const LrSeg& seg);
int launch_cvt_f32(blmm_ctx* ctx, const double* M, int64_t ld_in, int rows_valid, int64_t cols_valid, float* F,
                   int64_t ld_out, int kblocks);
int launch_rotate_f32(blmm_ctx* ctx, const double* Rp, int ldr, int n, int npad, const double* dG, int64_t p, float* RF, float* XF, int64_t ldxf,
                      const double* a0, int64_t lda, double* v_work , double* num );
int launch_lod_from_num(blmm_ctx* ctx, const double* num, const double* isx, int n, int64_t p, double* lod, int64_t* stat);
int launch_isx_f32(blmm_ctx* ctx, const NullModel& nm, const float* XF, int64_t ldxf, int64_t p, const double* Z0, const double* lam,
                   const double* h2_dev, double* isx, int64_t ld_isx, int64_t* stat);
int launch_scan_f32(blmm_ctx* ctx, const float* XF, int64_t ldxf, const float* PF, int64_t ldpf, int npad, int n,
                    int64_t p, int64_t m, const double* isx, float* L, int64_t ldL, int64_t* stat);
int launch_dyn_brent(blmm_ctx* ctx, const NullModel& nm, const double* Yt, int64_t ldy, int64_t m, const double* Z0, const double* lam,
                     double* h2, double* sigma2, double* ell, int64_t* stat);
int launch_dyn_alt_brent(blmm_ctx* ctx, const NullModel& nm, const double* Yt, int64_t ldy, const double* Xt, int64_t ldx, int64_t p,
                         const double* Z0, const double* lam, const double* h2null, int true_w, double* lod, double* h2each,
                         int64_t* stat, int64_t m, int64_t ldL, int64_t ldH);
int launch_dyn_loglik_grid(blmm_ctx* ctx, const NullModel& nm, const double* Yt, int64_t ldy, int64_t m, const double* Z0,
                           const double* lam, const double* grid_dev, int ngrid, double* EllTab, int* h2idx, double* h2, int64_t* stat);
int launch_dyn_panels(blmm_ctx* ctx, const NullModel& nm, const double* Yt, int64_t ldy, int64_t m, const double* Z0, const double* lam,
                      const double* h2, int full, double* panels, int64_t ldp, int64_t* stat);
int launch_dyn_isx(blmm_ctx* ctx, const NullModel& nm, const double* Xt, int64_t ldx, int64_t p, const double* Z0, const double* lam,
                   const double* grid_dev, int ngrid, double* isx, int64_t ld_isx, int64_t* stat);
int launch_dyn_perm(blmm_ctx* ctx, const NullModel& nm, const double* Yt, int64_t ldy, const double* Z0, const double* lam, const double* h2,
                    const int32_t* perm, int64_t ncols, int orig, double* r0, double* panel, int64_t ldp, int64_t* stat);
int launch_illcond_flag(blmm_ctx* ctx, const NullModel& nm, int64_t m, const double* Z0, const double* lam, const double* h2,
                        int* list, int64_t* stat, int* flags = nullptr);
int launch_scan_qr(blmm_ctx* ctx, const NullModel& nm, const double* Yt, int64_t ldy, const double* Xt, int64_t ldx, int64_t p,
                   const double* Z0, const double* lam, const double* h2, const int* list, double* L, int64_t ldL, int64_t* stat,
                   const RedArgs& red = RedArgs());
inline int qr_workspace(blmm_ctx* ctx, int cols, int n, size_t* lds, double** slab, unsigned* grid) {
  const size_t per = (size_t)(cols + 2) * n;
  *grid = (unsigned)(2 * (ctx->num_cus > 0 ? ctx->num_cus : 256));
  *lds = sizeof(double) * per;
  *slab = nullptr;
  if (*lds <= 64 * 1024) return BLMM_OK;
  if (int rc = ensure(ctx, ctx->qrSlab, sizeof(double) * per * *grid)) return rc;
  *slab = ptr<double>(ctx->qrSlab);
  *lds = 0;
  return BLMM_OK;
}
LrSeg lr_segments(const blmm_ctx* ctx, int n);
int launch_wbasis(blmm_ctx* ctx, const double* lam, int n, int npad, const LrSeg& seg, double* Wk, double* Q, int* rk, int64_t* stat);
int launch_lr_tpanels(blmm_ctx* ctx, const double* Xt, int64_t ldx, int64_t p, int n, int c, int npad, const double* Z0,
                      const double* Q, const int* rk, const LrSeg& seg, double* T, int64_t tstride, double* den0);
int launch_lr_panels(blmm_ctx* ctx, const NullModel& nm, const double* Yt, int64_t ldy, int64_t m, const double* Z0,
                     const double* lam, const double* h2, const double* Q, const int* rk, const LrSeg& seg, const int* perm, const LrRegion& rg,
                     double* P0, double* Cp, double* Ls, int64_t ldp, int64_t* stat);
int launch_scan_table(blmm_ctx* ctx, const ScanArgs& a);
int launch_scan_shared(blmm_ctx* ctx, const ScanArgs& a);
struct AltArgs {
  ScanArgs s;
  int ngrid; const double* EllTab;  const double* grid_dev; double* H2; int64_t ldH; int counter_quirk;
  const double* Ctab;
};
int launch_scan_alt(blmm_ctx* ctx, const AltArgs& a);
int launch_alt_ctab(blmm_ctx* ctx, const double* EllTab, int ngrid, int64_t m, int n, double* C);
int launch_bperm_panels(blmm_ctx* ctx, const NullModel& nm, const double* Yt, int64_t ldy, const double* Z0, const double* lam,
                        const double* h2c, int64_t mt, const int32_t* perm, int64_t nperms, double* panel, int64_t ldp, int* bin,
                        int64_t* stat);
__host__ __device__ inline bool key_less(double a, double b) {
  if (a != a) return false;
// ... 96 lines not shown
```

bulklmm.jl_amd/csrc/kernels_prep.hip:

```cpp
#include "blmm_internal.h"
#include "fastmath.h"
#include <cmath>
#include <cstring>
#include <algorithm>
#include <cstdlib>
#include <type_traits>

namespace blmm {

#define KCHECK()                                                                                      \
  do {                                                                                                \
    hipError_t e__ = hipGetLastError();                                                               \
    if (e__ != hipSuccess) return fail(ctx, BLMM_ERR_HIP, std::string("kernel launch: ") + hipGetErrorString(e__)); \
  } while (0)

__global__ void k_design(const double* __restrict__ K, const double* __restrict__ Covar, int ncov, int add_intercept,
                         const double* __restrict__ wd, int n, double* __restrict__ Ks, double* __restrict__ Zs) {
  const int64_t tid = blockIdx.x * (int64_t)blockDim.x + threadIdx.x;
  const int64_t stride = (int64_t)gridDim.x * blockDim.x;
  for (int64_t e = tid; e < (int64_t)n * n; e += stride) {
    const int i = (int)(e % n), j = (int)(e / n);
    double v = K[e];
    if (wd) v *= wd[i] * wd[j];
    Ks[e] = v;
  }
  const int c = ncov + (add_intercept ? 1 : 0);
  for (int64_t e = tid; e < (int64_t)n * c; e += stride) {
    const int i = (int)(e % n), q = (int)(e / n);
    double v;
    if (add_intercept) v = (q == 0) ? 1.0 : Covar[(int64_t)(q - 1) * n + i];
    else v = Covar[(int64_t)q * n + i];
    if (wd) v *= wd[i];
    Zs[e] = v;
  }
}

int launch_design(blmm_ctx* ctx, const double* dK, const double* dCovar, int ncov, int add_intercept,
                  const double* dweights, int n, double* Ks, double* Zs) {
  int blocks = (int)std::min<int64_t>(1024, ((int64_t)n * n + 255) / 256);
  hipLaunchKernelGGL(k_design, dim3(blocks), dim3(256), 0, ctx->stream, dK, dCovar, ncov, add_intercept, dweights, n, Ks, Zs);
  KCHECK();
  return BLMM_OK;
}


constexpr int JAC_NMAX = 124;
constexpr int JAC_NWG = 20;

__device__ __forceinline__ int jac_pi(int pos, int NP2) {
  if (NP2 <= 1 || pos == 0) return pos;
  const int s = pos >> 1;
  if (pos & 1) return (s == 0) ? 2 : 2 * (s - 1) + 1;
  return (s == NP2 - 1) ? 2 * s + 1 : 2 * (s + 1);
}

struct PostEigenArgs {
  const double* Zs; const double* wd; int c, npad, ldr, decomp, centered;
  double* lam; double* U; double* Z0; double* Rp; double* tmp;
};
template <bool VLDS>
__device__ __forceinline__ void post_eigen_body(const double* __restrict__ lraw_in, const double* __restrict__ Vg, int n, const PostEigenArgs& pa,
                                                int64_t* stat, double* shv, double* Ginv , double* Gw ,
                                                int* s_neg) {
  const double* __restrict__ Zs_g = pa.Zs; const double* __restrict__ wd = pa.wd;
  const int c = pa.c, npad = pa.npad, ldr = pa.ldr, decomp = pa.decomp, centered = pa.centered;
  double* __restrict__ lam = pa.lam; double* __restrict__ Ug = pa.U; double* __restrict__ Z0g = pa.Z0; double* __restrict__ Rp = pa.Rp;
  double* __restrict__ tmp = pa.tmp;
  const int tid = threadIdx.x, nt = blockDim.x;
  double* Vl = shv;
  double* Ul = shv + (size_t)n * n;
  double* Zsl = Ul + (size_t)n * n;
  double* Z0l = Zsl + (size_t)n * c;
  double* Bql = Z0l + (size_t)n * c;
  double* lrl = Bql + (size_t)n * c;
  if (VLDS) {
    for (int e = tid; e < n * n; e += nt) Vl[e] = Vg[e];
    for (int e = tid; e < n * c; e += nt) Zsl[e] = Zs_g[e];
  }
  const double* V = VLDS ? Vl : Vg;
  const double* Zs = VLDS ? Zsl : Zs_g;
  double* U = VLDS ? Ul : Ug;
  double* Z0 = VLDS ? Z0l : Z0g;
  double* lraw = VLDS ? lrl : tmp;
  double* Bq = VLDS ? Bql : tmp + n;
  if (tid == 0) *s_neg = 0;
  for (int i = tid; i < n; i += nt) lraw[i] = (decomp == BLMM_SVD) ? fabs(lraw_in[i]) : lraw_in[i];
  __syncthreads();
  for (int i = tid; i < n; i += nt) {
    const double li = lraw[i];
    int rank = 0;
    for (int j = 0; j < n; ++j) {
      const double lj = lraw[j];
      if (decomp == BLMM_SVD) rank += (lj > li) || (lj == li && j < i);
      else rank += (lj < li) || (lj == li && j < i);
    }
    lam[rank] = li;
    if (li < -1e-7) atomicAdd(s_neg, 1);
    double big = 0.0;
    for (int k = 0; k < n; ++k) { const double v = V[(size_t)i * n + k]; if (fabs(v) > fabs(big)) big = v; }
    const double sg = (big < 0.0) ? -1.0 : 1.0;
    for (int k = 0; k < n; ++k) U[(size_t)rank * n + k] = sg * V[(size_t)i * n + k];
  }
  __syncthreads();
  if (tid == 0 && *s_neg) stat[ST_NEG_EIG] += *s_neg;
  if (VLDS) { for (int e = tid; e < n * n; e += nt) Ug[e] = Ul[e]; }
  for (int e = tid; e < n * c; e += nt) {
    const int k = e % n, q = e / n;
    double s = 0;
    for (int i = 0; i < n; ++i) s = fma(U[(size_t)k * n + i], Zs[(size_t)q * n + i], s);
    Z0[e] = s;
    if (VLDS) Z0g[e] = s;
  }
  __syncthreads();
  if (tid == 0) {
    auto G = [&](int r_, int c_) -> double& { return Gw[r_ * (2 * CMAX) + c_]; };
    for (int a = 0; a < c; ++a)
      for (int b = 0; b < c; ++b) {
        double s = 0;
        for (int k = 0; k < n; ++k) s = fma(Z0[(size_t)a * n + k], Z0[(size_t)b * n + k], s);
        G(a, b) = s; G(a, c + b) = (a == b) ? 1.0 : 0.0;
      }
    for (int a = 0; a < c; ++a) {
      int piv = a;
      for (int r = a + 1; r < c; ++r) if (fabs(G(r, a)) > fabs(G(piv, a))) piv = r;
      if (piv != a) for (int b = 0; b < 2 * c; ++b) { double t = G(a, b); G(a, b) = G(piv, b); G(piv, b) = t; }
      const double d = 1.0 / G(a, a);
      for (int b = 0; b < 2 * c; ++b) G(a, b) *= d;
      for (int r = 0; r < c; ++r) if (r != a) { const double f = G(r, a); for (int b = 0; b < 2 * c; ++b) G(r, b) -= f * G(a, b); }
    }
    for (int a = 0; a < c; ++a) for (int b = 0; b < c; ++b) Ginv[a * CMAX + b] = G(a, c + b);
  }
  __syncthreads();
  for (int e = tid; e < n * c; e += nt) {
    const int i = e % n, q = e / n;
    double s = 0;
    for (int r = 0; r < c; ++r) s = fma(Ginv[q * CMAX + r], Zs[(size_t)r * n + i], s);
    Bq[(size_t)q * n + i] = s * (wd ? wd[i] : 1.0);
  }
  __syncthreads();
  for (int e = tid; e < npad * ldr; e += nt) {
    const int k = e % ldr, i = e / ldr;
    double v = 0.0;
    if (i < n && k < n) {
      v = U[(size_t)k * n + i] * (wd ? wd[i] : 1.0);
      if (centered)
        for (int q = 0; q < c; ++q) v = fma(-Z0[(size_t)q * n + k], Bq[(size_t)q * n + i], v);
    }
    Rp[e] = v;
  }
}

template <bool VLDS>
__global__ void __launch_bounds__(1024) k_post_eigen(const double* __restrict__ lraw_in, const double* __restrict__ Vg, int n, PostEigenArgs pa,
                                                     int64_t* stat) {
  __shared__ double Ginv[CMAX * CMAX];
  __shared__ double Gw[CMAX * 2 * CMAX];
  __shared__ int s_neg;
  extern __shared__ __attribute__((aligned(16))) double shv[];
  post_eigen_body<VLDS>(lraw_in, Vg, n, pa, stat, shv, Ginv, Gw, &s_neg);
}

__global__ void __launch_bounds__(1024) k_jacobi_lds(const double* __restrict__ Ag, double* __restrict__ Vg, int n,
                                                     double* __restrict__ lraw, int64_t* stat, double stop2, PostEigenArgs pa, int fuse_post,
                                                     int pe_off ) {
  extern __shared__ __attribute__((aligned(16))) double smem[];
  __shared__ double s_anorm;
  __shared__ int s_pe_neg, s_pe_last;
  if (stat[ST_EIG_FAST] == 1 && __longlong_as_double((long long)stat[ST_EIG_BAD]) <= 1.0) {
    if (fuse_post && blockIdx.x == 0) post_eigen_body<true>(lraw, Vg, n, pa, stat, smem, smem + pe_off, smem + pe_off + CMAX * CMAX, &s_pe_neg);
    return;
  }
  const int tid = threadIdx.x, nt = blockDim.x;
  const unsigned long long dbg_t0 = __builtin_amdgcn_s_memtime(), dbg_r0 = __builtin_amdgcn_s_memrealtime();
  const int N = n + (n & 1), NP2 = N / 2, ld = N + 1;
  const int rows_per = (n + gridDim.x - 1) / gridDim.x;
  const int r0 = blockIdx.x * rows_per, r1 = min(n, r0 + rows_per), nr = max(0, r1 - r0);
  const int PL = (NP2 * (NP2 - 1) / 2 + 1) & ~1;
  const int DG = 4 * PL;
  const int AO = (4 * PL + 3 * NP2 + 1) & ~1;
  const int VO = rows_per * ld;
  const int V0 = 2 * AO;
  const int REC = (2 * AO + 2 * VO + 1) & ~1;
  const int REL = REC + 4 * NP2;
  auto aidx = [&](int r, int c) -> int {
    if (r > c) { const int t = r; r = c; c = t; }
    const int sr = r >> 1, sc = c >> 1;
    if (sr == sc) return DG + ((r == c) ? ((r & 1) ? NP2 + sr : sr) : 2 * NP2 + sr);
    return ((r & 1) * 2 + (c & 1)) * PL + sc * (sc - 1) / 2 + sr;
  };
  for (int e = tid; e < 2 * AO + 2 * VO; e += nt) smem[e] = 0.0;
  __syncthreads();
  for (int e = tid; e < n * n; e += nt) { const int i = e % n, j = e / n; if (i <= j) smem[aidx(i, j)] = Ag[e]; }
  for (int r = tid; r < nr; r += nt) smem[V0 + r * ld + (r0 + r)] = 1.0;
  __syncthreads();
  if (tid == 0) {
    double m = 0.0;
    for (int i = 0; i < n; ++i) m = fmax(m, fabs(smem[aidx(i, i)]));
    s_anorm = m;
  }
  __syncthreads();
  const double eps = 2.220446049250313e-16;
  const double tol2 = (4.0 * eps) * (4.0 * eps);
  const double floor2 = (eps * s_anorm) * (eps * s_anorm);
  const int nblk = NP2 * (NP2 - 1) / 2;
  constexpr int MAXB = 2;
  const int NW = nt - 64;
  int b_s1[MAXB], b_s2[MAXB], b_src[MAXB], b_dst[MAXB][4];
  bool b_ok[MAXB];
#pragma unroll
  for (int u = 0; u < MAXB; ++u) {
    const int b = (tid < NW) ? tid + u * NW : nblk;
    b_s1[u] = 0; b_s2[u] = 0; b_src[u] = 0; b_ok[u] = false;
#pragma unroll
    for (int w = 0; w < 4; ++w) b_dst[u][w] = 0;
    if (b < nblk) {
      b_ok[u] = true;
      int row = (int)((sqrt(8.0 * b + 1.0) - 1.0) * 0.5);
      while (row * (row + 1) / 2 > b) --row;
      while ((row + 1) * (row + 2) / 2 <= b) ++row;
      const int s2 = row + 1, s1 = b - row * (row + 1) / 2;
      b_s1[u] = s1; b_s2[u] = s2;
      b_src[u] = b;
      const int rp = jac_pi(2 * s1, NP2), rq = jac_pi(2 * s1 + 1, NP2), cp = jac_pi(2 * s2, NP2), cq = jac_pi(2 * s2 + 1, NP2);
      b_dst[u][0] = aidx(rp, cp); b_dst[u][1] = aidx(rp, cq);
      b_dst[u][2] = aidx(rq, cp); b_dst[u][3] = aidx(rq, cq);
    }
  }
  const int nvit = NP2 * nr;
  const int nvthr = NW;
  const int vitem = (tid < nvthr) ? nvthr - 1 - tid : -1;
// ... 173 lines not shown
#endif
  const double* A = smem + (cur ? AO : 0);
  const double* Vc = smem + V0 + (cur ? VO : 0);
  const bool odd = (n & 1) != 0;
  if (blockIdx.x == 0) {
    for (int pos = tid; pos < N; pos += nt) {
      if (odd && pos == dpos) continue;
      const int o = (odd && pos > dpos) ? pos - 1 : pos;
      lraw[o] = A[aidx(pos, pos)];
    }
    if (tid == 0) {
      stat[ST_JACOBI_SWEEPS] = sweep + 1;
      stat[ST_EIG_CYCLES] = (int64_t)(__builtin_amdgcn_s_memtime() - dbg_t0);
      stat[ST_EIG_TICKS] = (int64_t)(__builtin_amdgcn_s_memrealtime() - dbg_r0);
    }
  }
  for (int e = tid; e < nr * N; e += nt) {
    const int r = e % nr, pos = e / nr;
    if (odd && pos == dpos) continue;
    const int o = (odd && pos > dpos) ? pos - 1 : pos;
    Vg[(size_t)o * n + (r0 + r)] = Vc[r * ld + pos];
  }
  if (!fuse_post) return;
  __threadfence();
  __syncthreads();
  if (tid == 0) s_pe_last = (atomicAdd((unsigned long long*)&stat[ST_EIG_DONE], 1ull) == (unsigned long long)gridDim.x - 1ull) ? 1 : 0;
  __syncthreads();
  if (!s_pe_last) return;
  __threadfence();
  post_eigen_body<true>(lraw, Vg, n, pa, stat, smem, smem + pe_off, smem + pe_off + CMAX * CMAX, &s_pe_neg);
}

__global__ void __launch_bounds__(1024) k_jacobi_glb(double* __restrict__ A, double* __restrict__ V, int n,
                                                     double* __restrict__ lraw, int64_t* stat) {
  __shared__ int s_rot;
  __shared__ double s_anorm;
  const int tid = threadIdx.x, nt = blockDim.x;
  const int N = n + (n & 1), NP2 = N / 2, ld = n;
  double* cs = V + (size_t)n * n;
  int* pq = reinterpret_cast<int*>(cs + 2 * NP2);
  if (tid == 0) { s_rot = 0; s_anorm = 0.0; }
  for (int e = tid; e < n * n; e += nt) V[e] = ((e % n) == (e / n)) ? 1.0 : 0.0;
  __syncthreads();
  if (tid == 0) {
    double m = 0.0;
    for (int i = 0; i < n; ++i) m = fmax(m, fabs(A[(size_t)i * ld + i]));
    s_anorm = m;
  }
  __syncthreads();
  const double eps = 2.220446049250313e-16;
  const double tol2 = (4.0 * eps) * (4.0 * eps);
  const double floor2 = (eps * s_anorm) * (eps * s_anorm);
  int sweep = 0;
  for (; sweep < 30; ++sweep) {
    for (int round = 0; round < N - 1; ++round) {
      for (int slot = tid; slot < NP2; slot += nt) {
        int p, q;
        if (slot == 0) { p = N - 1; q = round; }
        else { p = (round + slot) % (N - 1); q = (round - slot + (N - 1)) % (N - 1); }
        if (p > q) { const int t = p; p = q; q = t; }
        double c = 1.0, s = 0.0;
        if (q < n) {
          const double app = A[(size_t)p * ld + p], aqq = A[(size_t)q * ld + q], apq = A[(size_t)q * ld + p];
          const double pp = fabs(app * aqq), a2 = apq * apq;
          if (a2 > tol2 * fmax(pp, floor2)) {
            const double d = aqq - app;
            const double h = sqrt(fma(d, d, 4.0 * a2));
            const double t = copysign(2.0 * apq, apq * copysign(1.0, d)) / (fabs(d) + h);
            c = 1.0 / sqrt(fma(t, t, 1.0));
            s = t * c;
            s_rot = 1;
          }
        } else { q = p; }
        cs[2 * slot] = c; cs[2 * slot + 1] = s;
        pq[2 * slot] = p; pq[2 * slot + 1] = q;
      }
      __threadfence_block();
      __syncthreads();
      for (int item = tid; item < NP2 * n * 2; item += nt) {
        const int slot = item / (2 * n), off = item % (2 * n);
        const double s = cs[2 * slot + 1];
        if (s != 0.0) {
          const double c = cs[2 * slot];
          const int p = pq[2 * slot], q = pq[2 * slot + 1];
          double* M = (off >= n) ? V : A;
          const int k = (off >= n) ? off - n : off;
          const double x = M[(size_t)p * ld + k], y = M[(size_t)q * ld + k];
          M[(size_t)p * ld + k] = fma(c, x, -s * y);
          M[(size_t)q * ld + k] = fma(s, x, c * y);
        }
      }
      __threadfence_block();
      __syncthreads();
      for (int item = tid; item < NP2 * n; item += nt) {
        const int slot = item / n, j = item - slot * n;
        const double s = cs[2 * slot + 1];
        if (s != 0.0) {
          const double c = cs[2 * slot];
          const int p = pq[2 * slot], q = pq[2 * slot + 1];
          const double x = A[(size_t)j * ld + p], y = A[(size_t)j * ld + q];
          A[(size_t)j * ld + p] = fma(c, x, -s * y);
          A[(size_t)j * ld + q] = fma(s, x, c * y);
        }
      }
      __threadfence_block();
      __syncthreads();
    }
    const int rot = s_rot;
    __syncthreads();
    if (tid == 0) s_rot = 0;
    __syncthreads();
    if (!rot) break;
  }
  for (int i = tid; i < n; i += nt) lraw[i] = A[(size_t)i * ld + i];
  if (tid == 0) stat[ST_JACOBI_SWEEPS] = sweep + 1;
}

int jacobi_lds_max_n() { return JAC_NMAX; }

int launch_jacobi(blmm_ctx* ctx, double* A, double* V, int n, double* lraw, int64_t* stat, const PostEigenArgs* pe, bool* fused) {
  if (fused) *fused = false;
  if (n <= JAC_NMAX) {
    const int N = n + (n & 1), NP2 = N / 2, ld = N + 1;
    static const int nwg_env = dev_env("BLMM_JAC_NWG") ? atoi(dev_env("BLMM_JAC_NWG")) : 0;
    const int nwg = (nwg_env >= 1 && nwg_env <= 64) ? nwg_env : JAC_NWG;
    const int rows_per = (n + nwg - 1) / nwg;
    const int PL = (NP2 * (NP2 - 1) / 2 + 1) & ~1, AO = (4 * PL + 3 * NP2 + 1) & ~1;
    size_t lds = sizeof(double) * ((size_t)2 * AO + (size_t)2 * rows_per * ld + 5 * NP2 + 2) + 64;
    static const bool fuse_on = !(dev_env("BLMM_EIG_FUSE_POST") && dev_env("BLMM_EIG_FUSE_POST")[0] == '0');
    PostEigenArgs pa{};
    int fuse = 0, pe_off = 0;
    if (pe && fuse_on) {
      pe_off = (int)(((size_t)2 * n * n + (size_t)3 * n * pe->c + n + 1) & ~(size_t)1);
      const size_t lds_pe = sizeof(double) * ((size_t)pe_off + 3 * CMAX * CMAX) + 64;
      if (lds_pe <= 150 * 1024) { fuse = 1; pa = *pe; if (lds_pe > lds) lds = lds_pe; }
    }
    if (fused) *fused = fuse != 0;
    BLMM_HIP(hipFuncSetAttribute(reinterpret_cast<const void*>(&k_jacobi_lds), hipFuncAttributeMaxDynamicSharedMemorySize, (int)lds));
    static const double stop2 = dev_env("BLMM_JAC_STOP2") ? atof(dev_env("BLMM_JAC_STOP2")) : 1e-15;
    static const int nt_env = dev_env("BLMM_JAC_NT") ? atoi(dev_env("BLMM_JAC_NT")) : 0;
    const int nblk = NP2 * (NP2 - 1) / 2;
    int nthr = (nblk <= 2 * (768 - 64)) ? 768 : 1024;
    if (nt_env >= 256 && nt_env <= 1024 && nt_env % 64 == 0 && nblk <= 2 * (nt_env - 64)) nthr = nt_env;
    if (fuse) BLMM_LAUNCH_STOP(ctx, k_jacobi_lds, dim3(nwg), dim3(nthr), lds, A, V, n, lraw, stat, stop2, pa, fuse, pe_off);
    else hipLaunchKernelGGL(k_jacobi_lds, dim3(nwg), dim3(nthr), lds, ctx->stream, A, V, n, lraw, stat, stop2, pa, fuse, pe_off);
  } else {
    hipLaunchKernelGGL(k_jacobi_glb, dim3(1), dim3(1024), 0, ctx->stream, A, V, n, lraw, stat);
  }
  KCHECK();
  return BLMM_OK;
}

int launch_jacobi_post(blmm_ctx* ctx, double* A, double* V, int n, double* lraw, int64_t* stat, const double* Zs, const double* dweights,
                       int c, int npad, int ldr, int decomp, int centered, double* lam, double* U, double* Z0, double* Rp, bool* fused) {
  const PostEigenArgs pa{Zs, dweights, c, npad, ldr, decomp, centered, lam, U, Z0, Rp, nullptr};
  return launch_jacobi(ctx, A, V, n, lraw, stat, &pa, fused);
}

__global__ void __launch_bounds__(256) k_pe_rank(const double* __restrict__ lraw_in, int n, int decomp, double* __restrict__ lam,
                                                 int* __restrict__ rankof, int64_t* stat) {
  __shared__ double s_l[256];
  const int i = blockIdx.x * blockDim.x + threadIdx.x;
  const bool svd = decomp == BLMM_SVD;
  const double li = (i < n) ? (svd ? fabs(lraw_in[i]) : lraw_in[i]) : 0.0;
  int unsorted = svd ? 1 : 0;
  if (!svd)
    for (int j = threadIdx.x; j + 1 < n; j += blockDim.x) unsorted |= !(lraw_in[j] <= lraw_in[j + 1]);
  if (!__syncthreads_or(unsorted)) {
    if (i >= n) return;
    lam[i] = li;
    rankof[i] = i;
    if (li < -1e-7) atomicAdd((unsigned long long*)&stat[ST_NEG_EIG], 1ull);
    return;
  }
  int rank = 0;
  for (int j0 = 0; j0 < n; j0 += 256) {
    const int jn = (n - j0 < 256) ? n - j0 : 256;
    __syncthreads();
    if ((int)threadIdx.x < jn) { const double v = lraw_in[j0 + threadIdx.x]; s_l[threadIdx.x] = svd ? fabs(v) : v; }
    __syncthreads();
    for (int u = 0; u < jn; ++u) {
      const double lj = s_l[u];
      const int j = j0 + u;
      if (svd) rank += (lj > li) || (lj == li && j < i);
      else rank += (lj < li) || (lj == li && j < i);
    }
  }
  if (i >= n) return;
  lam[rank] = li;
  rankof[i] = rank;
  if (li < -1e-7) atomicAdd((unsigned long long*)&stat[ST_NEG_EIG], 1ull);
}
__global__ void __launch_bounds__(256) k_pe_cols(const double* __restrict__ V, const int* __restrict__ rankof,
                                                 const double* __restrict__ Zs, int n, int c, double* __restrict__ U,
                                                 double* __restrict__ Z0) {
  __shared__ double s_v[256];
  __shared__ int s_k[256];
  __shared__ double s_z[CMAX][4];
  const int i = blockIdx.x, t = threadIdx.x, lane = t & 63, wave = t >> 6;
  const double* v = V + (size_t)i * n;
  double big = 0.0; int bk = n;
  for (int k = t; k < n; k += 256) { const double x = v[k]; if (fabs(x) > fabs(big)) { big = x; bk = k; } }
  s_v[t] = big; s_k[t] = bk;
  __syncthreads();
  for (int o = 128; o > 0; o >>= 1) {
    if (t < o) {
      const double a = s_v[t], b = s_v[t + o];
      if (fabs(b) > fabs(a) || (fabs(b) == fabs(a) && s_k[t + o] < s_k[t])) { s_v[t] = b; s_k[t] = s_k[t + o]; }
    }
    __syncthreads();
  }
  const double sg = (s_v[0] < 0.0) ? -1.0 : 1.0;
  const int rank = rankof[i];
  double zacc[CMAX] = {};
  for (int k = t; k < n; k += 256) {
    const double u = sg * v[k];
    U[(size_t)rank * n + k] = u;
    for (int q = 0; q < c; ++q) zacc[q] = fma(u, Zs[(size_t)q * n + k], zacc[q]);
  }
  for (int q = 0; q < c; ++q) {
    double z = zacc[q];
    for (int o = 32; o > 0; o >>= 1) z += __shfl_xor(z, o, 64);
    if (lane == 0) s_z[q][wave] = z;
  }
  __syncthreads();
  if (t < c) Z0[(size_t)t * n + rank] = (s_z[t][0] + s_z[t][1]) + (s_z[t][2] + s_z[t][3]);
}
__global__ void __launch_bounds__(256) k_pe_bq(const double* __restrict__ Z0, const double* __restrict__ Zs,
                                               const double* __restrict__ wd, int n, int c, double* __restrict__ Bq) {
  __shared__ double Ginv[CMAX * CMAX], s_g[CMAX * CMAX][4];
  const int t = threadIdx.x, lane = t & 63, wave = t >> 6;
  for (int ab = 0; ab < c * c; ++ab) {
    const int a = ab / c, b = ab % c;
    double g = 0.0;
    for (int k = t; k < n; k += 256) g = fma(Z0[(size_t)a * n + k], Z0[(size_t)b * n + k], g);
    for (int o = 32; o > 0; o >>= 1) g += __shfl_xor(g, o, 64);
    if (lane == 0) s_g[ab][wave] = g;
  }
  __syncthreads();
  if (t == 0) {
    __shared__ double G[CMAX][2 * CMAX];
    for (int a = 0; a < c; ++a)
      for (int b = 0; b < c; ++b) {
        const int ab = a * c + b;
        G[a][b] = (s_g[ab][0] + s_g[ab][1]) + (s_g[ab][2] + s_g[ab][3]);
        G[a][c + b] = (a == b) ? 1.0 : 0.0;
      }
    for (int a = 0; a < c; ++a) {
      int piv = a;
      for (int r = a + 1; r < c; ++r) if (fabs(G[r][a]) > fabs(G[piv][a])) piv = r;
      if (piv != a) for (int b = 0; b < 2 * c; ++b) { double tt = G[a][b]; G[a][b] = G[piv][b]; G[piv][b] = tt; }
      const double d = 1.0 / G[a][a];
      for (int b = 0; b < 2 * c; ++b) G[a][b] *= d;
      for (int r = 0; r < c; ++r) if (r != a) { const double f = G[r][a]; for (int b = 0; b < 2 * c; ++b) G[r][b] -= f * G[a][b]; }
    }
    for (int a = 0; a < c; ++a) for (int b = 0; b < c; ++b) Ginv[a * CMAX + b] = G[a][c + b];
  }
  __syncthreads();
  for (int e = t; e < n * c; e += 256) {
    const int i = e % n, q = e / n;
    double sacc = 0;
    for (int r = 0; r < c; ++r) sacc = fma(Ginv[q * CMAX + r], Zs[(size_t)r * n + i], sacc);
    Bq[(size_t)q * n + i] = sacc * (wd ? wd[i] : 1.0);
  }
}
__global__ void __launch_bounds__(256) k_pe_rp(const double* __restrict__ U, const double* __restrict__ Z0,
                                               const double* __restrict__ Bq, const double* __restrict__ wd, int n, int c,
                                               int npad, int ldr, int centered, double* __restrict__ Rp) {
  __shared__ double tile[32][33];
  const int k0 = blockIdx.x * 32, i0 = blockIdx.y * 32;
  const int tx = threadIdx.x & 31, ty = threadIdx.x >> 5;
  for (int r = ty; r < 32; r += 8) {
    const int k = k0 + r, i = i0 + tx;
    tile[r][tx] = (k < n && i < n) ? U[(size_t)k * n + i] : 0.0;
  }
  __syncthreads();
  for (int r = ty; r < 32; r += 8) {
    const int i = i0 + r, k = k0 + tx;
    if (i >= npad || k >= ldr) continue;
    double v = 0.0;
    if (i < n && k < n) {
      v = tile[tx][r] * (wd ? wd[i] : 1.0);
      if (centered)
        for (int q = 0; q < c; ++q) v = fma(-Z0[(size_t)q * n + k], Bq[(size_t)q * n + i], v);
    }
    Rp[(size_t)i * ldr + k] = v;
  }
}

int launch_post_eigen(blmm_ctx* ctx, const double* lraw, const double* V, const double* Zs, const double* dweights, int n,
                      int c, int npad, int ldr, int decomp, int centered, double* lam, double* U, double* Z0, double* Rp,
                      int64_t* stat) {
  int rc = ensure(ctx, ctx->misc, sizeof(double) * ((size_t)n + (size_t)c * n + 64));
  if (rc) return rc;
  const size_t lds = sizeof(double) * ((size_t)2 * n * n + (size_t)3 * n * c + n);
  static const size_t lds_static = [] {
    hipFuncAttributes fa;
    return hipFuncGetAttributes(&fa, reinterpret_cast<const void*>(&k_post_eigen<true>)) == hipSuccess ? (size_t)fa.sharedSizeBytes : (size_t)32768;
  }();
  const PostEigenArgs pa{Zs, dweights, c, npad, ldr, decomp, centered, lam, U, Z0, Rp, ptr<double>(ctx->misc)};
  if (lds + lds_static <= 158 * 1024) {
    BLMM_HIP(hipFuncSetAttribute(reinterpret_cast<const void*>(&k_post_eigen<true>), hipFuncAttributeMaxDynamicSharedMemorySize, (int)lds));
    BLMM_LAUNCH_STOP(ctx, (k_post_eigen<true>), dim3(1), dim3(1024), lds, lraw, V, n, pa, stat);
  } else {
    double* Bq = ptr<double>(ctx->misc);
    int* rankof = reinterpret_cast<int*>(Bq + (size_t)c * n);
    hipLaunchKernelGGL(k_pe_rank, dim3((unsigned)((n + 255) / 256)), dim3(256), 0, ctx->stream, lraw, n, decomp, lam, rankof, stat);
    hipLaunchKernelGGL(k_pe_cols, dim3((unsigned)n), dim3(256), 0, ctx->stream, V, rankof, Zs, n, c, U, Z0);
    hipLaunchKernelGGL(k_pe_bq, dim3(1), dim3(256), 0, ctx->stream, Z0, Zs, dweights, n, c, Bq);
    hipLaunchKernelGGL(k_pe_rp, dim3((unsigned)((ldr + 31) / 32), (unsigned)((npad + 31) / 32)), dim3(256), 0, ctx->stream, U, Z0,
                       Bq, dweights, n, c, npad, ldr, centered, Rp);
  }
  KCHECK();
  return BLMM_OK;
}

template <int MBLK>
__global__ void __launch_bounds__(256) k_rotate(const double* __restrict__ Rp, int ldr, int n, int npad,
                                                const double* __restrict__ In, int64_t ncols,
                                                double* __restrict__ Out, int64_t ldo, int64_t ncols_pad) {
  const int lane = threadIdx.x & 63, wave = threadIdx.x >> 6;
  const int64_t col = ((int64_t)blockIdx.x * 4 + wave) * 16 + (lane & 15);
  const int rb0 = blockIdx.y * MBLK;
  const int kk = lane >> 4;
  d4 acc[MBLK];
#pragma unroll
  for (int b = 0; b < MBLK; ++b) acc[b] = (d4){0, 0, 0, 0};
  const bool colok = col < ncols;
  const double* pin = In + (colok ? col : 0) * (int64_t)n;
  for (int i0 = 0; i0 < npad; i0 += 16) {
    double bv[4], av[4][MBLK];
#pragma unroll
    for (int u = 0; u < 4; ++u) {
      const int i = i0 + 4 * u + kk;
      bv[u] = (colok && i < n) ? pin[i] : 0.0;
      const double* pr = Rp + (size_t)(i < npad ? i : 0) * ldr + (lane & 15);
#pragma unroll
      for (int b = 0; b < MBLK; ++b) {
        const int r0 = (rb0 + b) * 16;
        av[u][b] = (r0 < ldr && i < npad) ? pr[r0] : 0.0;
      }
    }
#pragma unroll
    for (int u = 0; u < 4; ++u)
#pragma unroll
      for (int b = 0; b < MBLK; ++b) acc[b] = __builtin_amdgcn_mfma_f64_16x16x4f64(av[u][b], bv[u], acc[b], 0, 0, 0);
  }
  if (col < ncols_pad) {
#pragma unroll
    for (int b = 0; b < MBLK; ++b)
#pragma unroll
      for (int r = 0; r < 4; ++r) {
        const int row = (rb0 + b) * 16 + kk + 4 * r;
        if (row < npad) Out[(int64_t)row * ldo + col] = acc[b][r];
      }
  }
}

__global__ void __launch_bounds__(256) k_rotate_vec(const double* __restrict__ Rp, int ldr, int n, int npad,
                                                    const double* __restrict__ In, int64_t col, double* __restrict__ Out,
                                                    int64_t ldo) {
  __shared__ double s_acc[4][64];
  const int lane = threadIdx.x & 63, wave = threadIdx.x >> 6;
  const int k = blockIdx.x * 64 + lane;
  const double* x = In + col * (int64_t)n;
  double a0 = 0.0, a1 = 0.0, a2 = 0.0, a3 = 0.0;
  const int kc = (k < npad) ? k : 0;
  int i = wave;
  for (; i + 28 < n; i += 32) {
    double r[8], xv[8];
#pragma unroll
    for (int u = 0; u < 8; ++u) { r[u] = Rp[(size_t)(i + 4 * u) * ldr + kc]; xv[u] = x[i + 4 * u]; }
    a0 = fma(r[0], xv[0], a0); a1 = fma(r[1], xv[1], a1); a2 = fma(r[2], xv[2], a2); a3 = fma(r[3], xv[3], a3);
    a0 = fma(r[4], xv[4], a0); a1 = fma(r[5], xv[5], a1); a2 = fma(r[6], xv[6], a2); a3 = fma(r[7], xv[7], a3);
  }
  for (; i < n; i += 4) a0 = fma(Rp[(size_t)i * ldr + kc], x[i], a0);
  const double acc = (k < npad) ? (a0 + a1) + (a2 + a3) : 0.0;
  s_acc[wave][lane] = acc;
  __syncthreads();
  if (wave == 0 && k < npad) Out[(int64_t)k * ldo + col] = (s_acc[0][lane] + s_acc[1][lane]) + (s_acc[2][lane] + s_acc[3][lane]);
}

typedef double d2ua __attribute__((ext_vector_type(2), aligned(8)));
template <int NB, bool PREF, int TR = 8>
__global__ void __launch_bounds__(256, 2) k_rotate_big(const double* __restrict__ Rp, int ldr, int n, int npad,
                                                       const double* __restrict__ In, int64_t ncols,
                                                       double* __restrict__ Out, int64_t ldo, int64_t ncols_pad, int nkt,
                                                       int64_t nct) {
  constexpr int MB = 4;
  const int lane = threadIdx.x & 63, wave = threadIdx.x >> 6;
  const int c16 = lane & 15, gq = lane >> 4;
  const int64_t bid = blockIdx.x;
  const int64_t xcd = bid & 7, idx = bid >> 3;
  const int64_t ctile = (idx / nkt) * 8 + xcd;
  const int ktile = (int)(idx % nkt);
  if (ctile >= nct) return;
  const int k0 = ktile * 128 + (wave >> 1) * 64;
  const int64_t col0 = ctile * (32 * NB) + (wave & 1) * (16 * NB);
  d4 acc[MB][NB];
#pragma unroll
  for (int a = 0; a < MB; ++a)
#pragma unroll
    for (int b = 0; b < NB; ++b) acc[a][b] = (d4){0, 0, 0, 0};
  const double* pcol[NB];
  bool cok[NB];
#pragma unroll
  for (int b = 0; b < NB; ++b) {
    const int64_t col = col0 + 16 * b + c16;
    cok[b] = col < ncols;
    pcol[b] = In + (cok[b] ? col : 0) * (int64_t)n;
  }
  auto loadB = [&](double (&bv)[NB][TR], int i0) {
#pragma unroll
    for (int b = 0; b < NB; ++b) {
      const int ib = i0 + TR * gq;
      if (cok[b] && ib + TR <= n) {
#pragma unroll
        for (int h = 0; h < TR / 2; ++h) { const d2ua v = *reinterpret_cast<const d2ua*>(pcol[b] + ib + 2 * h); bv[b][2 * h] = v[0]; bv[b][2 * h + 1] = v[1]; }
      } else {
#pragma unroll
        for (int s = 0; s < TR; ++s) bv[b][s] = (cok[b] && ib + s < n) ? pcol[b][ib + s] : 0.0;
      }
    }
  };
  auto loadA = [&](double (&av)[MB], int i) {
    const double* pr = Rp + (size_t)(i < npad ? i : 0) * ldr + c16;
#pragma unroll
    for (int a = 0; a < MB; ++a) { const int k = k0 + 16 * a; av[a] = (i < npad && k + c16 < ldr) ? pr[k] : 0.0; }
  };
  typedef unsigned int u32x4r __attribute__((ext_vector_type(4)));
  typedef unsigned int u32x2r __attribute__((ext_vector_type(2)));
  const uint64_t bytesA = (uint64_t)npad * (uint64_t)ldr * 8u, bytesB = (uint64_t)ncols * (uint64_t)n * 8u;
  const bool fast = bytesA < 0xffffff00ull && bytesB < 0xffffff00ull;
  const __amdgpu_buffer_rsrc_t srdA = __builtin_amdgcn_make_buffer_rsrc(const_cast<double*>(Rp), 0, (unsigned)(fast ? bytesA : 0), 0x00020000);
  const __amdgpu_buffer_rsrc_t srdB = __builtin_amdgcn_make_buffer_rsrc(const_cast<double*>(In), 0, (unsigned)(fast ? bytesB : 0), 0x00020000);
  uint32_t voffA[MB];
#pragma unroll
  for (int a = 0; a < MB; ++a) {
    const int kc = k0 + 16 * a + c16;
    voffA[a] = (uint32_t)((((int64_t)TR * gq) * ldr + (kc < ldr ? kc : ldr - 1)) * 8);
  }
  uint32_t voffB[NB];
#pragma unroll
  for (int b = 0; b < NB; ++b) {
    const int64_t col = col0 + 16 * b + c16;
    voffB[b] = (col < ncols) ? (uint32_t)((col * (int64_t)n + TR * gq) * 8) : 0xffffff00u;
  }
  auto loadB_fast = [&](double (&bv)[NB][TR], int i0) {
#pragma unroll
    for (int b = 0; b < NB; ++b)
#pragma unroll
      for (int h = 0; h < TR / 2; ++h) {
        const u32x4r v = __builtin_amdgcn_raw_buffer_load_b128(srdB, voffB[b] + 16 * h, (unsigned)i0 * 8u, 0);
        const d2 w = __builtin_bit_cast(d2, v);
// ... 347 lines not shown
  const double rss = syy - tt;
  const double prior_df = prior_b > 0.0 ? prior_b + 2.0 : prior_b;
  const double num = rss + prior_a * prior_b;
  const double den = (reml ? (double)(n - C) : (double)n) + prior_df;
  const double sigma2 = num * fast_rcp(den);
  const double ls = (sigma2 >= 2.2250738585072014e-308) ? fast_log<false>(sigma2, s_ln) : log(sigma2);
  double ell = -0.5 * (((double)n + prior_b) * ls + logsum + den);
  if (reml) ell += 0.5 * ((double)C * ls - ((detA >= 2.2250738585072014e-308) ? fast_log<false>(detA, s_ln) : log(detA)));
  EllOut o; o.ell = ell; o.sigma2 = sigma2; o.yy = rss;
  return o;
}

constexpr int BRENT_LPT = 4;
#ifndef BRENT_PHASE1_IT
#define BRENT_PHASE1_IT 20
#endif
constexpr int BRENT_PHASE1 = BRENT_PHASE1_IT;

template <typename F>
__device__ __forceinline__ double brent_search(F& f, int nint, bool valid, int* hit_max) {
  const double golden = 0.5 * (3.0 - sqrt(5.0));
  const double rel_tol = 1.4901161193847656e-08, abs_tol = 2.220446049250313e-16;
  double best_x = 0.0, best_f = INFINITY;
  for (int iv = 0; iv < nint; ++iv) {
    double x_lower = (double)iv / (double)nint, x_upper = (iv + 1 == nint) ? 1.0 : (double)(iv + 1) / (double)nint;
    double new_minimizer = x_lower + golden * (x_upper - x_lower);
    double new_minimum = f(new_minimizer);
    double step = 0.0, old_step = 0.0;
    double old_minimizer = new_minimizer, old_old_minimizer = new_minimizer;
    double old_minimum = new_minimum, old_old_minimum = new_minimum;
    bool done = !valid;
    int it = 0;
    for (; it < 1000; ++it) {
      double p = 0.0, q = 0.0;
      const double x_tol = rel_tol * fabs(new_minimizer) + abs_tol;
      const double x_mid = (x_upper + x_lower) / 2;
      if (fabs(new_minimizer - x_mid) <= 2 * x_tol - (x_upper - x_lower) / 2) done = true;
      if (__all(done)) break;
      if (fabs(old_step) > x_tol) {
        const double r = (new_minimizer - old_minimizer) * (new_minimum - old_old_minimum);
        q = (new_minimizer - old_old_minimizer) * (new_minimum - old_minimum);
        p = (new_minimizer - old_old_minimizer) * q - (new_minimizer - old_minimizer) * r;
        q = 2 * (q - r);
        if (q > 0) p = -p; else q = -q;
      }
      double nstep, nold;
      if (fabs(p) < fabs(q * old_step / 2) && p < q * (x_upper - new_minimizer) && p < q * (new_minimizer - x_lower)) {
        nold = step;
        nstep = p / q;
        const double x_temp = new_minimizer + nstep;
        if ((x_temp - x_lower) < 2 * x_tol || (x_upper - x_temp) < 2 * x_tol) nstep = (new_minimizer < x_mid) ? x_tol : -x_tol;
      } else {
        nold = (new_minimizer < x_mid) ? x_upper - new_minimizer : x_lower - new_minimizer;
        nstep = golden * nold;
      }
      const double new_x = (fabs(nstep) >= x_tol) ? new_minimizer + nstep : new_minimizer + ((nstep > 0) ? x_tol : -x_tol);
      const double new_f = f(done ? new_minimizer : new_x);
      if (!done) {
        old_step = nold; step = nstep;
        if (new_f < new_minimum) {
          if (new_x < new_minimizer) x_upper = new_minimizer; else x_lower = new_minimizer;
          old_old_minimizer = old_minimizer; old_old_minimum = old_minimum;
          old_minimizer = new_minimizer; old_minimum = new_minimum;
          new_minimizer = new_x; new_minimum = new_f;
        } else {
          if (new_x < new_minimizer) x_lower = new_x; else x_upper = new_x;
          if (new_f <= old_minimum || old_minimizer == new_minimizer) {
            old_old_minimizer = old_minimizer; old_old_minimum = old_minimum;
            old_minimizer = new_x; old_minimum = new_f;
          } else if (new_f <= old_old_minimum || old_old_minimizer == new_minimizer || old_old_minimizer == old_minimizer) {
            old_old_minimizer = new_x; old_old_minimum = new_f;
          }
        }
      }
    }
    if (it >= 1000 && !done) *hit_max = 1;
    if (new_minimum < best_f || iv == 0) { best_f = new_minimum; best_x = new_minimizer; }
  }
  return best_x;
}

struct BrentState {
  double xl, xu, x, fx, step, old_step, ox, oox, ofx, oofx;
  int done;
};
template <typename F>
__device__ __forceinline__ void brent_init(F& f, BrentState& S, double a, double b, bool valid) {
  const double golden = 0.5 * (3.0 - sqrt(5.0));
  S.xl = a; S.xu = b;
  S.x = a + golden * (b - a);
  S.fx = f(S.x);
  S.step = 0.0; S.old_step = 0.0;
  S.ox = S.x; S.oox = S.x; S.ofx = S.fx; S.oofx = S.fx;
  S.done = !valid;
}
template <typename F>
__device__ __forceinline__ int brent_run(F& f, BrentState& S, int max_it) {
  const double golden = 0.5 * (3.0 - sqrt(5.0));
  const double rel_tol = 1.4901161193847656e-08, abs_tol = 2.220446049250313e-16;
  int it = 0;
  for (; it < max_it; ++it) {
    double p = 0.0, q = 0.0;
    const double x_tol = rel_tol * fabs(S.x) + abs_tol;
    const double x_mid = (S.xu + S.xl) / 2;
    if (fabs(S.x - x_mid) <= 2 * x_tol - (S.xu - S.xl) / 2) S.done = 1;
    if (__all(S.done)) break;
    if (fabs(S.old_step) > x_tol) {
      const double r = (S.x - S.ox) * (S.fx - S.oofx);
      q = (S.x - S.oox) * (S.fx - S.ofx);
      p = (S.x - S.oox) * q - (S.x - S.ox) * r;
      q = 2 * (q - r);
      if (q > 0) p = -p; else q = -q;
    }
    double nstep, nold;
    if (fabs(p) < fabs(q * S.old_step / 2) && p < q * (S.xu - S.x) && p < q * (S.x - S.xl)) {
      nold = S.step;
      nstep = p / q;
      const double x_temp = S.x + nstep;
      if ((x_temp - S.xl) < 2 * x_tol || (S.xu - x_temp) < 2 * x_tol) nstep = (S.x < x_mid) ? x_tol : -x_tol;
    } else {
      nold = (S.x < x_mid) ? S.xu - S.x : S.xl - S.x;
      nstep = golden * nold;
    }
    const double new_x = (fabs(nstep) >= x_tol) ? S.x + nstep : S.x + ((nstep > 0) ? x_tol : -x_tol);
    const double new_f = f(S.done ? S.x : new_x);
    if (!S.done) {
      S.old_step = nold; S.step = nstep;
      if (new_f < S.fx) {
        if (new_x < S.x) S.xu = S.x; else S.xl = S.x;
        S.oox = S.ox; S.oofx = S.ofx;
        S.ox = S.x; S.ofx = S.fx;
        S.x = new_x; S.fx = new_f;
      } else {
        if (new_x < S.x) S.xl = new_x; else S.xu = new_x;
        if (new_f <= S.ofx || S.ox == S.x) {
          S.oox = S.ox; S.oofx = S.ofx;
          S.ox = new_x; S.ofx = new_f;
        } else if (new_f <= S.oofx || S.oox == S.x || S.oox == S.ox) {
          S.oox = new_x; S.oofx = new_f;
        }
      }
    }
  }
  return it;
}

struct BrentCont {
  double* st;
  int* list;
  unsigned int* cnt;
  int* fin;
};

template <int C, int LPT, bool REG>
__global__ void __launch_bounds__(256, BRENT_MINW) k_brent(NullModel nm, const double* __restrict__ Yt, int64_t ldy, int64_t m,
                                               const double* __restrict__ Z0, const double* __restrict__ lam,
                                               const double* __restrict__ logtab, double* __restrict__ h2out,
                                               double* __restrict__ s2out, double* __restrict__ ellout, int64_t* stat,
                                               BrentCont cont) {
  extern __shared__ __attribute__((aligned(16))) double sh[];
  __shared__ dpair s_ln[BLMM_LOG_TABLE_N];
  const int n = nm.n;
  double* sLam = sh;
  double* sZ = sh + n;
  if (!REG) {
    for (int e = threadIdx.x; e < n; e += blockDim.x) sLam[e] = lam[e];
    for (int e = threadIdx.x; e < n * C; e += blockDim.x) sZ[e] = Z0[e];
  } else {
    stage_null_lz<C, LPT>(sh, n, Z0, lam);
  }
  stage_log_table<false>(s_ln, logtab);
  __syncthreads();
  const int64_t j = ((int64_t)blockIdx.x * blockDim.x + threadIdx.x) / LPT;
  const int sub = threadIdx.x % LPT;
  const bool valid = j < m;
  const double* ycol = Yt + (valid ? j : 0);
  int nonpos = 0, hit_max = 0;
  const int nint = nm.optim_interval < 1 ? 1 : nm.optim_interval;
  double best_x;
  EllOut fin;
  double* sY = sh + LPT * NULL_NK * (1 + C);
  if constexpr (REG) {
    stage_null_y<LPT>(sY, ycol, ldy, sub, n, valid);
    __syncthreads();
  }
  if constexpr (REG && (64 / LPT) > 1) {
    if (nint == 1) {
      constexpr int TPW = 256 / LPT;
      constexpr int TPV = 64 / LPT;
      __shared__ double s_bst[10][TPW];
      __shared__ int s_bit[TPW], s_blist[TPW], s_bnp[TPW], s_bcnt;
      NullRegs<C, LPT> R;
      R.base = sh; R.lo = sub * NULL_NK * (1 + C); R.yo = LPT * NULL_NK * (1 + C) + threadIdx.x;
      auto f = [&](double h2) { return -null_ell_reg<C, LPT>(h2, R, n, nm.prior_a, nm.prior_b, nm.reml, s_ln, &nonpos).ell; };
      BrentState S;
      brent_init(f, S, 0.0, 1.0, valid);
      const int it1 = brent_run(f, S, BRENT_PHASE1);
      fin = null_ell_reg<C, LPT>(S.x, R, n, nm.prior_a, nm.prior_b, nm.reml, s_ln, &nonpos);
      const int ts = threadIdx.x / LPT;
      wave_count(&stat[ST_H2_BOUNDARY], sub == 0 && valid && S.done && h2_on_boundary(S.x));
      if (sub == 0) {
        if (valid && cont.fin) cont.fin[j] = S.done ? 1 : 0;
        if (valid && S.done) {
          h2out[j] = S.x;
          if (s2out) s2out[j] = fin.sigma2;
          if (ellout) ellout[j] = fin.ell;
          if (nonpos) atomicAdd((unsigned long long*)&stat[ST_NONPOS_W], 1ull);
        }
        s_bst[0][ts] = S.xl; s_bst[1][ts] = S.xu; s_bst[2][ts] = S.x; s_bst[3][ts] = S.fx; s_bst[4][ts] = S.step;
        s_bst[5][ts] = S.old_step; s_bst[6][ts] = S.ox; s_bst[7][ts] = S.oox; s_bst[8][ts] = S.ofx; s_bst[9][ts] = S.oofx;
        s_bit[ts] = S.done ? -1 : it1;
        s_bnp[ts] = nonpos;
      }
      __syncthreads();
      if (threadIdx.x == 0) {
        int cnt = 0;
        for (int e = 0; e < TPW; ++e) if (s_bit[e] >= 0) s_blist[cnt++] = e;
        s_bcnt = cnt;
      }
      __syncthreads();
      const int U = s_bcnt;
      if (cont.list) {
        __shared__ unsigned int s_bbase;
        if (threadIdx.x == 0 && U > 0) s_bbase = atomicAdd(cont.cnt, (unsigned int)U);
        __syncthreads();
        for (int e = threadIdx.x; e < U; e += blockDim.x) cont.list[s_bbase + e] = (int)(blockIdx.x * TPW + s_blist[e]);
        for (int e = threadIdx.x; e < U * 12; e += blockDim.x) {
          const int fi = e / U, src = s_blist[e % U];
          const int64_t jt = (int64_t)blockIdx.x * TPW + src;
          cont.st[(int64_t)fi * m + jt] = (fi < 10) ? s_bst[fi][src] : (fi == 10 ? (double)s_bit[src] : (double)s_bnp[src]);
        }
        return;
      }
      const int wave = ((threadIdx.x >> 6) + 4 - (int)(blockIdx.x & 3)) & 3;
      if (wave * TPV >= U) return;
      const int qslot = wave * TPV + (threadIdx.x & 63) / LPT;
      const bool valid2 = qslot < U;
      const int src = s_blist[valid2 ? qslot : 0];
      const int64_t j2 = (int64_t)blockIdx.x * TPW + src;
      R.yo = LPT * NULL_NK * (1 + C) + src * LPT + sub;
      S.xl = s_bst[0][src]; S.xu = s_bst[1][src]; S.x = s_bst[2][src]; S.fx = s_bst[3][src]; S.step = s_bst[4][src];
      S.old_step = s_bst[5][src]; S.ox = s_bst[6][src]; S.oox = s_bst[7][src]; S.ofx = s_bst[8][src]; S.oofx = s_bst[9][src];
      S.done = !valid2;
      nonpos = s_bnp[src];
      const int it0 = s_bit[src];
      const int it2 = brent_run(f, S, 1000 - it0);
      fin = null_ell_reg<C, LPT>(S.x, R, n, nm.prior_a, nm.prior_b, nm.reml, s_ln, &nonpos);
      wave_count(&stat[ST_H2_BOUNDARY], valid2 && sub == 0 && h2_on_boundary(S.x));
      if (valid2 && sub == 0) {
        h2out[j2] = S.x;
        if (s2out) s2out[j2] = fin.sigma2;
        if (ellout) ellout[j2] = fin.ell;
        if (it0 + it2 >= 1000 && !S.done) atomicAdd((unsigned long long*)&stat[ST_BRENT_MAXIT], 1ull);
        if (nonpos) atomicAdd((unsigned long long*)&stat[ST_NONPOS_W], 1ull);
      }
      return;
    }
  }
  if constexpr (REG) {
    NullRegs<C, LPT> R;
    R.base = sh; R.lo = sub * NULL_NK * (1 + C); R.yo = LPT * NULL_NK * (1 + C) + threadIdx.x;
    auto f = [&](double h2) { return -null_ell_reg<C, LPT>(h2, R, n, nm.prior_a, nm.prior_b, nm.reml, s_ln, &nonpos).ell; };
    best_x = brent_search(f, nint, valid, &hit_max);
    fin = null_ell_reg<C, LPT>(best_x, R, n, nm.prior_a, nm.prior_b, nm.reml, s_ln, &nonpos);
  } else {
    auto f = [&](double h2) { return -null_ell<C, LPT>(h2, ycol, ldy, sub, n, sZ, sLam, nm.prior_a, nm.prior_b, nm.reml, &nonpos).ell; };
    best_x = brent_search(f, nint, valid, &hit_max);
    fin = null_ell<C, LPT>(best_x, ycol, ldy, sub, n, sZ, sLam, nm.prior_a, nm.prior_b, nm.reml, &nonpos);
  }
  wave_count(&stat[ST_H2_BOUNDARY], valid && sub == 0 && h2_on_boundary(best_x));
  if (valid && sub == 0) {
    h2out[j] = best_x;
    if (s2out) s2out[j] = fin.sigma2;
    if (ellout) ellout[j] = fin.ell;
    if (hit_max) atomicAdd((unsigned long long*)&stat[ST_BRENT_MAXIT], 1ull);
    if (nonpos) atomicAdd((unsigned long long*)&stat[ST_NONPOS_W], 1ull);
  }
}

template <int C, int LPT, int NK = NULL_NK>
__global__ void __launch_bounds__(256, BRENT_MINW2) k_brent2(NullModel nm, const double* __restrict__ Yt, int64_t ldy, int64_t m,
                                                const double* __restrict__ Z0, const double* __restrict__ lam,
                                                const double* __restrict__ logtab, double* __restrict__ h2out,
                                                double* __restrict__ s2out, double* __restrict__ ellout, int64_t* stat,
                                                BrentCont cont) {
  extern __shared__ __attribute__((aligned(16))) double sh[];
  __shared__ dpair s_ln[BLMM_LOG_TABLE_N];
  constexpr int TPW = 256 / LPT;
  const unsigned int U = *cont.cnt;
  if ((unsigned int)blockIdx.x * TPW >= U) return;
  const int n = nm.n;
  stage_null_lz<C, LPT, NK>(sh, n, Z0, lam);
  stage_log_table<false>(s_ln, logtab);
  double* sY = sh + LPT * NK * (1 + C);
  const unsigned int q = (unsigned int)blockIdx.x * TPW + threadIdx.x / LPT;
  const int sub = threadIdx.x % LPT;
  const bool valid = q < U;
  const int64_t j = cont.list[valid ? q : (unsigned int)blockIdx.x * TPW];
  stage_null_y<LPT, NK>(sY, Yt + j, ldy, sub, n, true);
  __syncthreads();
  int nonpos = (int)cont.st[(int64_t)11 * m + j];
  NullRegs<C, LPT> R;
  R.base = sh; R.lo = sub * NK * (1 + C); R.yo = LPT * NK * (1 + C) + threadIdx.x;
  auto f = [&](double h2) { return -null_ell_reg<C, LPT, (NK / 4 < BRENT_UNROLL2 ? NK / 4 : BRENT_UNROLL2), NK>(h2, R, n, nm.prior_a, nm.prior_b, nm.reml, s_ln, &nonpos).ell; };
  BrentState S;
  S.xl = cont.st[j]; S.xu = cont.st[m + j]; S.x = cont.st[2 * m + j]; S.fx = cont.st[3 * m + j];
  S.step = cont.st[4 * m + j]; S.old_step = cont.st[5 * m + j]; S.ox = cont.st[6 * m + j]; S.oox = cont.st[7 * m + j];
  S.ofx = cont.st[8 * m + j]; S.oofx = cont.st[9 * m + j];
  S.done = !valid;
  const int it0 = (int)cont.st[(int64_t)10 * m + j];
  const int it2 = brent_run(f, S, 1000 - it0);
  const EllOut fin = null_ell_reg<C, LPT, (NK / 4 < BRENT_UNROLL2 ? NK / 4 : BRENT_UNROLL2), NK>(S.x, R, n, nm.prior_a, nm.prior_b, nm.reml, s_ln, &nonpos);
  wave_count(&stat[ST_H2_BOUNDARY], valid && sub == 0 && h2_on_boundary(S.x));
  if (valid && sub == 0) {
    h2out[j] = S.x;
    if (s2out) s2out[j] = fin.sigma2;
    if (ellout) ellout[j] = fin.ell;
    if (it0 + it2 >= 1000 && !S.done) atomicAdd((unsigned long long*)&stat[ST_BRENT_MAXIT], 1ull);
    if (nonpos) atomicAdd((unsigned long long*)&stat[ST_NONPOS_W], 1ull);
  }
}

template <int C, int LPT, bool REG>
static int launch_brent_t(blmm_ctx* ctx, const NullModel& nm, const double* Yt, int64_t ldy, int64_t m, const double* Z0,
                          const double* lam, double* h2, double* sigma2, double* ell, int64_t* stat, int phase, BrentSplit* sp) {
  const int64_t threads = m * LPT;
  const unsigned blocks = (unsigned)((threads + 255) / 256);
  const size_t lds = REG ? sizeof(double) * ((size_t)LPT * NULL_NK * (1 + C) + (size_t)NULL_NK * 256) : sizeof(double) * (size_t)nm.n * (1 + C);
  if (lds > 48 * 1024)
    BLMM_HIP(hipFuncSetAttribute(reinterpret_cast<const void*>(&k_brent<C, LPT, REG>), hipFuncAttributeMaxDynamicSharedMemorySize, (int)lds));
  BrentCont cont{nullptr, nullptr, nullptr, nullptr};
  static const char* two_env = dev_env("BLMM_BRENT_TWO");
  const bool two = REG && (64 / LPT) > 1 && nm.optim_interval <= 1 && m >= 1024 && !(two_env && two_env[0] == '0');
  if (two) {
    int rc = ensure(ctx, ctx->brSt, sizeof(double) * (size_t)12 * m);
    if (!rc) rc = ensure(ctx, ctx->brList, sizeof(int) * 2 * (size_t)m + 16);
    if (rc) return rc;
    cont.st = ptr<double>(ctx->brSt);
    cont.cnt = reinterpret_cast<unsigned int*>(stat + ST_BRENT_CNT);
    cont.list = ptr<int>(ctx->brList) + 4;
    cont.fin = cont.list + m;
    if (phase != 2) {
      if (ctx->brent_cnt_used) BLMM_HIP(hipMemsetAsync(cont.cnt, 0, 16, ctx->stream));
      ctx->brent_cnt_used = true;
    }
  }
  if (sp) { sp->active = two && phase == 1; sp->fin = cont.fin; sp->list = cont.list; sp->cnt = cont.cnt; }
  if (phase != 2) {
    hipLaunchKernelGGL((k_brent<C, LPT, REG>), dim3(blocks), dim3(256), lds, ctx->stream, nm, Yt, ldy, m, Z0, lam,
                       ptr<double>(ctx->logtab), h2, sigma2, ell, stat, cont);
    KCHECK();
  }
  if (phase == 1 && two) return BLMM_OK;
  if (phase == 2 && !two) return BLMM_OK;
  if constexpr (REG) {
    if (two) {
      static const int lpt2_env = dev_env("BLMM_BRENT2_LPT") ? atoi(dev_env("BLMM_BRENT2_LPT")) : 0;
      auto launch2 = [&](auto kern, int lpt2, int nk2) -> int {
        const size_t lds2 = sizeof(double) * ((size_t)lpt2 * nk2 * (1 + C) + (size_t)nk2 * 256);
        if (lds2 > 48 * 1024)
          BLMM_HIP(hipFuncSetAttribute(reinterpret_cast<const void*>(kern), hipFuncAttributeMaxDynamicSharedMemorySize, (int)lds2));
        const unsigned blocks2 = (unsigned)((m * lpt2 + 255) / 256);
        hipLaunchKernelGGL(kern, dim3(blocks2), dim3(256), lds2, ctx->stream, nm, Yt, ldy, m, Z0, lam, ptr<double>(ctx->logtab), h2,
                           sigma2, ell, stat, cont);
        KCHECK();
        return BLMM_OK;
      };
      if constexpr (LPT == 4) {
        if (lpt2_env == 16 && nm.n <= 16 * 8) return launch2(&k_brent2<C, 16, 8>, 16, 8);
        if (lpt2_env == 8 && nm.n <= 8 * 12) return launch2(&k_brent2<C, 8, 12>, 8, 12);
      }
      return launch2(&k_brent2<C, LPT, NULL_NK>, LPT, NULL_NK);
    }
  }
  return BLMM_OK;
}

template <int C>
static int launch_brent_c(blmm_ctx* ctx, const NullModel& nm, const double* Yt, int64_t ldy, int64_t m, const double* Z0,
                          const double* lam, double* h2, double* sigma2, double* ell, int64_t* stat, int phase, BrentSplit* sp) {
  const int n = nm.n;
  static const int lpt_env = dev_env("BLMM_BRENT_LPT") ? atoi(dev_env("BLMM_BRENT_LPT")) : 0;
  if (lpt_env == 8 && n <= 8 * NULL_NK) return launch_brent_t<C, 8, true>(ctx, nm, Yt, ldy, m, Z0, lam, h2, sigma2, ell, stat, phase, sp);
  if (lpt_env == 16 && n <= 16 * NULL_NK) return launch_brent_t<C, 16, true>(ctx, nm, Yt, ldy, m, Z0, lam, h2, sigma2, ell, stat, phase, sp);
  if (n <= 4 * NULL_NK) return launch_brent_t<C, 4, true>(ctx, nm, Yt, ldy, m, Z0, lam, h2, sigma2, ell, stat, phase, sp);
  if (n <= 8 * NULL_NK) return launch_brent_t<C, 8, true>(ctx, nm, Yt, ldy, m, Z0, lam, h2, sigma2, ell, stat, phase, sp);
  if (n <= 16 * NULL_NK) return launch_brent_t<C, 16, true>(ctx, nm, Yt, ldy, m, Z0, lam, h2, sigma2, ell, stat, phase, sp);
  if (n <= 32 * NULL_NK) return launch_brent_t<C, 32, true>(ctx, nm, Yt, ldy, m, Z0, lam, h2, sigma2, ell, stat, phase, sp);
  if (n <= 64 * NULL_NK) return launch_brent_t<C, 64, true>(ctx, nm, Yt, ldy, m, Z0, lam, h2, sigma2, ell, stat, phase, sp);
  return launch_brent_t<C, BRENT_LPT, false>(ctx, nm, Yt, ldy, m, Z0, lam, h2, sigma2, ell, stat, phase, sp);
}

int launch_brent(blmm_ctx* ctx, const NullModel& nm, const double* Yt, int64_t ldy, int64_t m, const double* Z0,
                 const double* lam, double* h2, double* sigma2, double* ell, int64_t* stat, int phase, BrentSplit* sp) {
  if (nm.c > CTPL && nm.c <= CMAX) {
    if (sp) sp->active = false;
    return phase == 2 ? BLMM_OK : launch_dyn_brent(ctx, nm, Yt, ldy, m, Z0, lam, h2, sigma2, ell, stat);
  }
  switch (nm.c) {
    case 1: return launch_brent_c<1>(ctx, nm, Yt, ldy, m, Z0, lam, h2, sigma2, ell, stat, phase, sp);
    case 2: return launch_brent_c<2>(ctx, nm, Yt, ldy, m, Z0, lam, h2, sigma2, ell, stat, phase, sp);
    case 3: return launch_brent_c<3>(ctx, nm, Yt, ldy, m, Z0, lam, h2, sigma2, ell, stat, phase, sp);
    case 4: return launch_brent_c<4>(ctx, nm, Yt, ldy, m, Z0, lam, h2, sigma2, ell, stat, phase, sp);
#define BG(C) return launch_brent_t<C, 16, false>(ctx, nm, Yt, ldy, m, Z0, lam, h2, sigma2, ell, stat, phase, sp)
    case 5: BG(5);
    case 6: BG(6);
    case 7: BG(7);
    case 8: BG(8);
#undef BG
  }
  return fail(ctx, BLMM_ERR_UNSUPPORTED, BLMM_C_ERR);
}

template <int C, int X, int LPT, bool SQW>
__device__ __forceinline__ EllOut alt_ell(double h2, const double* __restrict__ xcol, int64_t xstride, int sub, int n,
                                          const double* __restrict__ sY, const double* __restrict__ sZ,
                                          const double* __restrict__ sLam, double prior_a, double prior_b, int reml, int* nonpos) {
  constexpr int D = C + X, NA = D * (D + 1) / 2;
  const double delta = h2 / (1.0 - h2);
  double A[NA], v[D], syy = 0.0, logsum = 0.0, prod = 1.0;
#pragma unroll
  for (int a = 0; a < NA; ++a) A[a] = 0.0;
#pragma unroll
  for (int q = 0; q < D; ++q) v[q] = 0.0;
  int cnt = 0, bad = 0;
  for (int k = sub; k < n; k += LPT) {
    const double t = fma(delta, sLam[k], 1.0);
    double w = 1.0 / t;
    bad |= !(w > 0.0);
    if (SQW) w = sqrt(w);
    prod *= t;
    if (++cnt == 8) { logsum += log(prod); prod = 1.0; cnt = 0; }
    const double y = sY[k];
    const double wy = w * y;
    syy = fma(wy, y, syy);
    double col[D];
#pragma unroll
    for (int q = 0; q < C; ++q) col[q] = sZ[q * n + k];
    if (X) col[D - 1] = xcol[(int64_t)k * xstride];
#pragma unroll
    for (int q = 0; q < D; ++q) {
      v[q] = fma(wy, col[q], v[q]);
      const double wz = w * col[q];
#pragma unroll
      for (int r = 0; r <= q; ++r) A[q * (q + 1) / 2 + r] = fma(wz, col[r], A[q * (q + 1) / 2 + r]);
    }
  }
  logsum += log(prod);
  if (SQW) logsum *= 0.5;
  syy = group_sum<LPT>(syy); logsum = group_sum<LPT>(logsum);
#pragma unroll
  for (int a = 0; a < NA; ++a) A[a] = group_sum<LPT>(A[a]);
#pragma unroll
  for (int q = 0; q < D; ++q) v[q] = group_sum<LPT>(v[q]);
  if (bad && nonpos) *nonpos = 1;
  double L[NA], t[D], logdet = 0.0, tt = 0.0;
#pragma unroll
  for (int q = 0; q < D; ++q) {
#pragma unroll
    for (int r = 0; r <= q; ++r) {
      double s = A[q * (q + 1) / 2 + r];
#pragma unroll
      for (int u = 0; u < r; ++u) s = fma(-L[q * (q + 1) / 2 + u], L[r * (r + 1) / 2 + u], s);
      if (r == q) { L[q * (q + 1) / 2 + q] = sqrt(s); logdet += log(s); }
      else L[q * (q + 1) / 2 + r] = s / L[r * (r + 1) / 2 + r];
    }
    double s = v[q];
#pragma unroll
    for (int u = 0; u < q; ++u) s = fma(-L[q * (q + 1) / 2 + u], t[u], s);
    t[q] = s / L[q * (q + 1) / 2 + q];
    tt = fma(t[q], t[q], tt);
  }
  const double rss = syy - tt;
  const double prior_df = prior_b > 0.0 ? prior_b + 2.0 : prior_b;
  const double num = rss + prior_a * prior_b;
  const double sigma2 = num / ((reml ? (double)(n - D) : (double)n) + prior_df);
  const double ls = log(sigma2);
  double ell = -0.5 * (((double)n + prior_b) * ls + logsum + num / sigma2);
  if (reml) ell += 0.5 * ((double)D * ls - logdet);
  EllOut o; o.ell = ell; o.sigma2 = sigma2; o.yy = rss;
  return o;
}

template <int C, int LPT>
__global__ void __launch_bounds__(256) k_alt_brent(NullModel nm, const double* __restrict__ Yt, int64_t ldy,
                                                   const double* __restrict__ Xt, int64_t ldx, int64_t p, const double* __restrict__ Z0,
                                                   const double* __restrict__ lam, const double* __restrict__ h2null,
                                                   int true_w, double* __restrict__ lod, double* __restrict__ h2each,
                                                   int64_t* stat, int64_t trait0, int64_t ldL, int64_t ldH) {
  extern __shared__ __attribute__((aligned(16))) double sh[];
  const int n = nm.n;
  const int64_t tr = trait0 + blockIdx.y;
  lod += tr * ldL; h2each += tr * ldH;
  double* sLam = sh;
  double* sY = sh + n;
  double* sZ = sh + 2 * n;
  for (int e = threadIdx.x; e < n; e += blockDim.x) { sLam[e] = lam[e]; sY[e] = Yt[(int64_t)e * ldy + tr]; }
  for (int e = threadIdx.x; e < n * C; e += blockDim.x) sZ[e] = Z0[e];
  __syncthreads();
  const int64_t j = ((int64_t)blockIdx.x * blockDim.x + threadIdx.x) / LPT;
  const int sub = threadIdx.x % LPT;
  const bool valid = j < p;
  const double* xcol = Xt + (valid ? j : 0);
  int nonpos = 0, hit_max = 0;
  const int nint = nm.optim_interval < 1 ? 1 : nm.optim_interval;
  auto f = [&](double h2) { return -alt_ell<C, 1, LPT, false>(h2, xcol, ldx, sub, n, sY, sZ, sLam, nm.prior_a, nm.prior_b, nm.reml, &nonpos).ell; };
  const double hx = brent_search(f, nint, valid, &hit_max);
  const double h0 = h2null[tr];
  double e1, e0;
  if (true_w) {
    e1 = alt_ell<C, 1, LPT, false>(hx, xcol, ldx, sub, n, sY, sZ, sLam, nm.prior_a, nm.prior_b, 0, nullptr).ell;
    e0 = alt_ell<C, 0, LPT, false>(h0, xcol, ldx, sub, n, sY, sZ, sLam, nm.prior_a, nm.prior_b, 0, nullptr).ell;
  } else {
    e1 = alt_ell<C, 1, LPT, true>(hx, xcol, ldx, sub, n, sY, sZ, sLam, nm.prior_a, nm.prior_b, 0, nullptr).ell;
    e0 = alt_ell<C, 0, LPT, true>(h0, xcol, ldx, sub, n, sY, sZ, sLam, nm.prior_a, nm.prior_b, 0, nullptr).ell;
  }
  if (valid && sub == 0) {
    lod[j] = (e1 - e0) / log(10.0);
    h2each[j] = hx;
    if (hit_max) atomicAdd((unsigned long long*)&stat[ST_BRENT_MAXIT], 1ull);
    if (nonpos) atomicAdd((unsigned long long*)&stat[ST_NONPOS_W], 1ull);
  }
}

template <int C, int LPT>
static int launch_alt_brent_t(blmm_ctx* ctx, const NullModel& nm, const double* Yt, int64_t ldy, const double* Xt, int64_t ldx, int64_t p,
                              const double* Z0, const double* lam, const double* h2null, int true_w, double* lod,
                              double* h2each, int64_t* stat, int64_t m, int64_t ldL, int64_t ldH) {
  const size_t lds = sizeof(double) * (size_t)nm.n * (2 + C);
  if (lds > 160 * 1024 - 512) return fail(ctx, BLMM_ERR_UNSUPPORTED, "scan_alt: n too large for the LDS-resident trait");
  if (lds > 48 * 1024) BLMM_HIP(hipFuncSetAttribute(reinterpret_cast<const void*>(&k_alt_brent<C, LPT>), hipFuncAttributeMaxDynamicSharedMemorySize, (int)lds));
  const int64_t threads = p * LPT;
  for (int64_t t0 = 0; t0 < m; t0 += 65535) {
    const int64_t mt = (m - t0 < 65535) ? m - t0 : 65535;
    hipLaunchKernelGGL((k_alt_brent<C, LPT>), dim3((unsigned)((threads + 255) / 256), (unsigned)mt), dim3(256), lds, ctx->stream, nm, Yt, ldy, Xt, ldx, p,
                       Z0, lam, h2null, true_w, lod, h2each, stat, t0, ldL, ldH);
    KCHECK();
  }
  return BLMM_OK;
}

int launch_alt_brent(blmm_ctx* ctx, const NullModel& nm, const double* Yt, int64_t ldy, const double* Xt, int64_t ldx, int64_t p,
                     const double* Z0, const double* lam, const double* h2null, int true_w, double* lod, double* h2each,
                     int64_t* stat, int64_t m, int64_t ldL, int64_t ldH) {
  if (p < 1 || m < 1) return BLMM_OK;
#define AB(C) (nm.n <= 160 ? launch_alt_brent_t<C, 4>(ctx, nm, Yt, ldy, Xt, ldx, p, Z0, lam, h2null, true_w, lod, h2each, stat, m, ldL, ldH) \
                           : launch_alt_brent_t<C, 16>(ctx, nm, Yt, ldy, Xt, ldx, p, Z0, lam, h2null, true_w, lod, h2each, stat, m, ldL, ldH))
  switch (nm.c) {
    case 1: return AB(1);
    case 2: return AB(2);
    case 3: return AB(3);
    case 4: return AB(4);
#define AG(C) return launch_alt_brent_t<C, 16>(ctx, nm, Yt, ldy, Xt, ldx, p, Z0, lam, h2null, true_w, lod, h2each, stat, m, ldL, ldH)
    case 5: AG(5);
    case 6: AG(6);
    case 7: AG(7);
    case 8: AG(8);
// ... 890 lines not shown
```

Before: 162.9 billion.

## Fuse design-matrix build into post-eigen and trait rotation into null Brent kernel

Skips the separate k_design launch for small unweighted problems. The kernel matrix is passed directly to the eigen solver, and the covariate design entries are generated on the fly inside the post-eigen kernel. The trait rotation launch is deferred and folded into the null-model Brent kernel: each workgroup rotates its own trait columns with f64 MFMA, writes Yt, then stages them. This removes kernel launches and a separate global pass over Y, but every Brent workgroup now repeats reads of Rp, and the rotation runs on the critical path instead of possibly overlapping other work.

```diff
diff --git a/bulklmm.jl_amd/csrc/blmm_api.hip b/bulklmm.jl_amd/csrc/blmm_api.hip
--- a/bulklmm.jl_amd/csrc/blmm_api.hip
+++ b/bulklmm.jl_amd/csrc/blmm_api.hip
@@ -285,7 +285,13 @@
   if ((rc = ensure(ctx, ctx->lraw, sizeof(double) * n))) return rc;
   if ((rc = reset_stat(ctx, &P.stat))) return rc;
   tm.mark();
-  if ((rc = launch_design(ctx, dK, nc.d, (int)nc.ncov, nc.add_int, dweights, (int)n, ptr<double>(ctx->Ks), ptr<double>(ctx->Zs)))) return rc;
+  const bool inline_design = ctx->tune.front_design_side != 0 && n <= jacobi_lds_max_n();
+  const ZsInline zsrc{nc.d, (int)nc.ncov, nc.add_int ? 1 : 0};
+  const ZsInline* zi = inline_design ? &zsrc : nullptr;
+  double* Ks = inline_design && !dweights ? const_cast<double*>(dK) : ptr<double>(ctx->Ks);
+  if (!inline_design || dweights) {
+    if ((rc = launch_design(ctx, dK, nc.d, (int)nc.ncov, nc.add_int, dweights, (int)n, ptr<double>(ctx->Ks), inline_design ? nullptr : ptr<double>(ctx->Zs)))) return rc;
+  }
   const double* evec = ptr<double>(ctx->V);
   const char* eig_env = dev_env("BLMM_EIGEN");
   if (!eig_env && ctx->tune.eigen_solver == 1) eig_env = "jacobi";
@@ -295,23 +301,23 @@
   bool done = false, post_done = false;
   const bool want_dc = eig_env ? std::strcmp(eig_env, "dc") == 0 : big;
   if (!done && want_dc && n >= 3) {
-    rc = launch_eig_dc(ctx, ptr<double>(ctx->Ks), (int)n, ptr<double>(ctx->lraw), ptr<double>(ctx->V), P.stat);
+    rc = launch_eig_dc(ctx, Ks, (int)n, ptr<double>(ctx->lraw), ptr<double>(ctx->V), P.stat);
     if (rc == BLMM_OK) { done = true; P.big = true; }
     else if (rc != BLMM_ERR_UNSUPPORTED) return rc;
   }
   if (!done) {
     const bool want_fast = !(eig_env && std::strcmp(eig_env, "jacobi") == 0) && n >= 3 && n <= eig_fast_max_n();
     if (want_fast) {
-      rc = launch_eig_fast(ctx, ptr<double>(ctx->Ks), (int)n, ptr<double>(ctx->lraw), ptr<double>(ctx->V), P.stat);
+      rc = launch_eig_fast(ctx, Ks, (int)n, ptr<double>(ctx->lraw), ptr<double>(ctx->V), P.stat);
       if (rc != BLMM_OK && rc != BLMM_ERR_UNSUPPORTED) return rc;
     }
-    if ((rc = launch_jacobi_post(ctx, ptr<double>(ctx->Ks), ptr<double>(ctx->V), (int)n, ptr<double>(ctx->lraw), P.stat, ptr<double>(ctx->Zs),
+    if ((rc = launch_jacobi_post(ctx, Ks, ptr<double>(ctx->V), (int)n, ptr<double>(ctx->lraw), P.stat, ptr<double>(ctx->Zs),
                                  dweights, c, P.npad, P.ldr, o->decomp_scheme, centered, P.lam, ptr<double>(ctx->U), P.Z0, ptr<double>(ctx->Rp),
-                                 &post_done))) return rc;
+                                 &post_done, zi))) return rc;
   }
   if (!post_done && (rc = launch_post_eigen(ctx, ptr<double>(ctx->lraw), evec, ptr<double>(ctx->Zs), dweights, (int)n, c,
                               P.npad, P.ldr, o->decomp_scheme, centered, P.lam, ptr<double>(ctx->U), P.Z0,
-                              ptr<double>(ctx->Rp), P.stat))) return rc;
+                              ptr<double>(ctx->Rp), P.stat, zi))) return rc;
   tm.mark();
   return BLMM_OK;
 }
@@ -375,7 +381,8 @@
 
 int prepare(blmm_ctx* ctx, const blmm_opts* o, const double* dY, int64_t n, int64_t m, const double* dG, int64_t p,
             const double* dCovar, int64_t ncov, const double* dK, const double* dweights, int centered, Pipe& P, Timer& tm,
-            bool early_wbasis = false, bool grid_side = false, bool skip_markers = false, const EigPre* pre = nullptr) {
+            bool early_wbasis = false, bool grid_side = false, bool skip_markers = false, const EigPre* pre = nullptr,
+            bool defer_traits = false) {
   if (m < 0 || p < 0) return fail(ctx, BLMM_ERR_DIM, "Dimension mismatch.");
   const bool forks = m > 0 && p > 0 && (early_wbasis || grid_side);
   ctx->stop_event_used = false;
@@ -401,7 +408,11 @@
     if ((rc = rotate_markers(ctx, P, dG, p))) return rc;
     P.xt_side = true;
   }
-  if ((rc = rotate_traits(ctx, P, dY, m))) return rc;
+  if (defer_traits) {
+    P.m = m; P.ldy = round_up(m > 0 ? m : 1, 128);
+    if ((rc = ensure(ctx, ctx->Yt, sizeof(double) * (size_t)P.npad * P.ldy))) return rc;
+    P.Yt = ptr<double>(ctx->Yt); P.y_raw = dY;
+  } else if ((rc = rotate_traits(ctx, P, dY, m))) return rc;
   if (skip_markers) { P.p = p; P.ldx = round_up(p > 0 ? p : 1, 128); P.Xt = nullptr; }
   else if (!P.xt_side) {
     if (up_flight) BLMM_HIP(hipStreamWaitEvent(ctx->stream, ctx->ev_in, 0));
@@ -881,6 +892,8 @@
   {"lr_split", 1, offsetof(blmm::Tuning, lr_split), -1, 1},
   {"eigen_solver", 1, offsetof(blmm::Tuning, eigen_solver), 0, 2},
   {"f32_rotation", 1, offsetof(blmm::Tuning, f32_rotation), 0, 1},
+  {"front_design_side", 1, offsetof(blmm::Tuning, front_design_side), 0, 1},
+  {"front_rotate_fused", 1, offsetof(blmm::Tuning, front_rotate_fused), 0, 1},
   {"bulk_perm_cols", 1, offsetof(blmm::Tuning, bulk_perm_cols), 0, 2147483647.0},
   {"mdf_red_chunk", 1, offsetof(blmm::Tuning, mdf_red_chunk), 0, 2147483647.0},
   {"cond_red_chunk", 1, offsetof(blmm::Tuning, cond_red_chunk), 0, 2147483647.0},
@@ -1088,7 +1101,8 @@
       const bool split_on = (ctx->red_cur.flags && P.c >= 2) ? false
                           : split_env ? split_env[0] != '0' : (ctx->tune.lr_split < 0 ? m >= 8192 : ctx->tune.lr_split != 0);
       BrentSplit sp;
-      if ((rc = launch_brent(ctx, nm, P.Yt, P.ldy, m, P.Z0, P.lam, dh2_out, nullptr, nullptr, P.stat, split_on ? 1 : 0, &sp))) return rc;
+      const BrentRot rot{ptr<double>(ctx->Rp), P.ldr, P.npad, P.y_raw, P.Yt};
+      if ((rc = launch_brent(ctx, nm, P.Yt, P.ldy, m, P.Z0, P.lam, dh2_out, nullptr, nullptr, P.stat, split_on ? 1 : 0, &sp, P.y_raw ? &rot : nullptr))) return rc;
       tm.mark();
       if (sp.active) { if ((rc = lr_finish_split(ctx, P, nm, dh2_out, dL_out, ldL, tm, sp))) return rc; }
       else if ((rc = lr_finish(ctx, P, nm, dh2_out, dL_out, ldL, tm))) return rc;
@@ -1190,7 +1204,8 @@
     if ((rc = grid_to_device(ctx, h2_grid_host, ngrid, &dgrid))) return rc;
   }
   const bool lowrank = wants_lowrank(ctx, opts, n, dCovar, ncov);
-  if ((rc = prepare(ctx, opts, dY, n, m, dG, p, dCovar, ncov, dK, dweights, 1, P, tm, lowrank, opts->method != BLMM_NULL_EXACT))) return rc;
+  const bool fuse_rot = lowrank && m > 0 && p > 0 && ctx->tune.front_rotate_fused != 0 && brent_can_rotate((int)n, (int)null_cov(opts, dCovar, ncov).c);
+  if ((rc = prepare(ctx, opts, dY, n, m, dG, p, dCovar, ncov, dK, dweights, 1, P, tm, lowrank, opts->method != BLMM_NULL_EXACT, false, nullptr, fuse_rot))) return rc;
   return scan_pipeline(ctx, opts, P, tm, lowrank,  lowrank && m > 0 && p > 0, dgrid, h2_grid_host, ngrid, dL_out, ldL, dh2_out, status, pvreq);
 }
 
diff --git a/bulklmm.jl_amd/csrc/blmm_internal.h b/bulklmm.jl_amd/csrc/blmm_internal.h
--- a/bulklmm.jl_amd/csrc/blmm_internal.h
+++ b/bulklmm.jl_amd/csrc/blmm_internal.h
@@ -54,6 +54,8 @@
   int eigen_solver = 0;
   int mdf_red_chunk = 0;
   int cond_red_chunk = 0;
+  int front_design_side = 1;
+  int front_rotate_fused = 1;
   int bulk_perm_cols = 0;
 };
 
@@ -68,6 +70,7 @@
   double *Yt = nullptr, *Xt = nullptr, *Z0 = nullptr, *lam = nullptr;
   int64_t* stat = nullptr;
   bool big = false;
+  const double* y_raw = nullptr;
   bool xt_side = false;
 };
 
@@ -184,9 +187,11 @@
 int launch_design(blmm_ctx* ctx, const double* dK, const double* dCovar, int ncov, int add_intercept,
                   const double* dweights, int n, double* Ks, double* Zs);
 struct PostEigenArgs;
+struct ZsInline { const double* Covar; int ncov, add_intercept; };
 int launch_jacobi(blmm_ctx* ctx, double* A, double* V, int n, double* lraw, int64_t* stat, const PostEigenArgs* pe = nullptr, bool* fused = nullptr);
 int launch_jacobi_post(blmm_ctx* ctx, double* A, double* V, int n, double* lraw, int64_t* stat, const double* Zs, const double* dweights,
-                       int c, int npad, int ldr, int decomp, int centered, double* lam, double* U, double* Z0, double* Rp, bool* fused);
+                       int c, int npad, int ldr, int decomp, int centered, double* lam, double* U, double* Z0, double* Rp, bool* fused,
+                       const ZsInline* zi = nullptr);
 int launch_eig_dc(blmm_ctx* ctx, const double* A, int n, double* lraw, double* evec, int64_t* stat);
 int eig_dc_max_n(const blmm_ctx* ctx);
 int launch_eig_fast(blmm_ctx* ctx, const double* A, int n, double* lraw, double* evec, int64_t* stat);
@@ -196,7 +201,7 @@
 int jacobi_lds_max_n();
 int launch_post_eigen(blmm_ctx* ctx, const double* lraw, const double* V, const double* Zs, const double* dweights, int n,
                       int c, int npad, int ldr, int decomp, int centered, double* lam, double* U, double* Z0, double* Rp,
-                      int64_t* stat);
+                      int64_t* stat, const ZsInline* zi = nullptr);
 int launch_rotate(blmm_ctx* ctx, const double* Rp, int ldr, int n, int npad, const double* In, int64_t ncols,
                   double* Out, int64_t ldo, int64_t ncols_pad);
 int launch_rotate_single(blmm_ctx* ctx, const double* Rp, int ldr, int n, int npad, const double* In, int64_t ncols, double* Out, int64_t ldo);
@@ -212,9 +217,11 @@
   const int* list = nullptr;
   const unsigned int* cnt = nullptr;
 };
+struct BrentRot { const double* Rp = nullptr; int ldr = 0, npad = 0; const double* Y = nullptr; double* Yt = nullptr; };
+bool brent_can_rotate(int n, int c);
 int launch_brent(blmm_ctx* ctx, const NullModel& nm, const double* Yt, int64_t ldy, int64_t m, const double* Z0,
                  const double* lam, double* h2, double* sigma2, double* ell, int64_t* stat, int phase = 0,
-                 BrentSplit* sp = nullptr);
+                 BrentSplit* sp = nullptr, const BrentRot* rot = nullptr);
 int launch_alt_brent(blmm_ctx* ctx, const NullModel& nm, const double* Yt, int64_t ldy, const double* Xt, int64_t ldx, int64_t p,
                      const double* Z0, const double* lam, const double* h2null, int true_w, double* lod, double* h2each,
                      int64_t* stat, int64_t m = 1, int64_t ldL = 0, int64_t ldH = 0);
diff --git a/bulklmm.jl_amd/csrc/kernels_prep.hip b/bulklmm.jl_amd/csrc/kernels_prep.hip
--- a/bulklmm.jl_amd/csrc/kernels_prep.hip
+++ b/bulklmm.jl_amd/csrc/kernels_prep.hip
@@ -14,30 +14,31 @@
     if (e__ != hipSuccess) return fail(ctx, BLMM_ERR_HIP, std::string("kernel launch: ") + hipGetErrorString(e__)); \
   } while (0)
 
+__device__ __forceinline__ double design_entry(const double* __restrict__ Covar, int add_intercept, const double* __restrict__ wd, int n, int e) {
+  const int i = e % n, q = e / n;
+  double v;
+  if (add_intercept) v = (q == 0) ? 1.0 : Covar[(int64_t)(q - 1) * n + i];
+  else v = Covar[(int64_t)q * n + i];
+  if (wd) v *= wd[i];
+  return v;
+}
 __global__ void k_design(const double* __restrict__ K, const double* __restrict__ Covar, int ncov, int add_intercept,
                          const double* __restrict__ wd, int n, double* __restrict__ Ks, double* __restrict__ Zs) {
   const int64_t tid = blockIdx.x * (int64_t)blockDim.x + threadIdx.x;
   const int64_t stride = (int64_t)gridDim.x * blockDim.x;
-  for (int64_t e = tid; e < (int64_t)n * n; e += stride) {
+  for (int64_t e = tid; Ks && e < (int64_t)n * n; e += stride) {
     const int i = (int)(e % n), j = (int)(e / n);
     double v = K[e];
     if (wd) v *= wd[i] * wd[j];
     Ks[e] = v;
   }
   const int c = ncov + (add_intercept ? 1 : 0);
-  for (int64_t e = tid; e < (int64_t)n * c; e += stride) {
-    const int i = (int)(e % n), q = (int)(e / n);
-    double v;
-    if (add_intercept) v = (q == 0) ? 1.0 : Covar[(int64_t)(q - 1) * n + i];
-    else v = Covar[(int64_t)q * n + i];
-    if (wd) v *= wd[i];
-    Zs[e] = v;
-  }
+  for (int64_t e = tid; Zs && e < (int64_t)n * c; e += stride) Zs[e] = design_entry(Covar, add_intercept, wd, n, (int)e);
 }
 
 int launch_design(blmm_ctx* ctx, const double* dK, const double* dCovar, int ncov, int add_intercept,
                   const double* dweights, int n, double* Ks, double* Zs) {
-  int blocks = (int)std::min<int64_t>(1024, ((int64_t)n * n + 255) / 256);
+  int blocks = (int)std::min<int64_t>(1024, ((int64_t)n * (Ks ? n : ncov + 1) + 255) / 256);
   hipLaunchKernelGGL(k_design, dim3(blocks), dim3(256), 0, ctx->stream, dK, dCovar, ncov, add_intercept, dweights, n, Ks, Zs);
   KCHECK();
   return BLMM_OK;
@@ -57,6 +58,7 @@
 struct PostEigenArgs {
   const double* Zs; const double* wd; int c, npad, ldr, decomp, centered;
   double* lam; double* U; double* Z0; double* Rp; double* tmp;
+  int zs_inline; const double* Covar; int add_intercept;
 };
 template <bool VLDS>
 __device__ __forceinline__ void post_eigen_body(const double* __restrict__ lraw_in, const double* __restrict__ Vg, int n, const PostEigenArgs& pa,
@@ -75,7 +77,8 @@
   double* lrl = Bql + (size_t)n * c;
   if (VLDS) {
     for (int e = tid; e < n * n; e += nt) Vl[e] = Vg[e];
-    for (int e = tid; e < n * c; e += nt) Zsl[e] = Zs_g[e];
+    if (pa.zs_inline) { for (int e = tid; e < n * c; e += nt) Zsl[e] = design_entry(pa.Covar, pa.add_intercept, wd, n, e); }
+    else { for (int e = tid; e < n * c; e += nt) Zsl[e] = Zs_g[e]; }
   }
   const double* V = VLDS ? Vl : Vg;
   const double* Zs = VLDS ? Zsl : Zs_g;
@@ -555,8 +558,10 @@
 }
 
 int launch_jacobi_post(blmm_ctx* ctx, double* A, double* V, int n, double* lraw, int64_t* stat, const double* Zs, const double* dweights,
-                       int c, int npad, int ldr, int decomp, int centered, double* lam, double* U, double* Z0, double* Rp, bool* fused) {
-  const PostEigenArgs pa{Zs, dweights, c, npad, ldr, decomp, centered, lam, U, Z0, Rp, nullptr};
+                       int c, int npad, int ldr, int decomp, int centered, double* lam, double* U, double* Z0, double* Rp, bool* fused,
+                       const ZsInline* zi) {
+  const PostEigenArgs pa{Zs, dweights, c, npad, ldr, decomp, centered, lam, U, Z0, Rp, nullptr, zi ? 1 : 0, zi ? zi->Covar : nullptr,
+                         zi ? zi->add_intercept : 0};
   return launch_jacobi(ctx, A, V, n, lraw, stat, &pa, fused);
 }
 
@@ -693,7 +698,7 @@
 
 int launch_post_eigen(blmm_ctx* ctx, const double* lraw, const double* V, const double* Zs, const double* dweights, int n,
                       int c, int npad, int ldr, int decomp, int centered, double* lam, double* U, double* Z0, double* Rp,
-                      int64_t* stat) {
+                      int64_t* stat, const ZsInline* zi) {
   int rc = ensure(ctx, ctx->misc, sizeof(double) * ((size_t)n + (size_t)c * n + 64));
   if (rc) return rc;
   const size_t lds = sizeof(double) * ((size_t)2 * n * n + (size_t)3 * n * c + n);
@@ -701,8 +706,11 @@
     hipFuncAttributes fa;
     return hipFuncGetAttributes(&fa, reinterpret_cast<const void*>(&k_post_eigen<true>)) == hipSuccess ? (size_t)fa.sharedSizeBytes : (size_t)32768;
   }();
-  const PostEigenArgs pa{Zs, dweights, c, npad, ldr, decomp, centered, lam, U, Z0, Rp, ptr<double>(ctx->misc)};
-  if (lds + lds_static <= 158 * 1024) {
+  const bool in_lds = lds + lds_static <= 158 * 1024;
+  if (zi && !in_lds && (rc = launch_design(ctx, nullptr, zi->Covar, zi->ncov, zi->add_intercept, dweights, n, nullptr, const_cast<double*>(Zs)))) return rc;
+  const PostEigenArgs pa{Zs, dweights, c, npad, ldr, decomp, centered, lam, U, Z0, Rp, ptr<double>(ctx->misc), zi && in_lds ? 1 : 0,
+                         zi ? zi->Covar : nullptr, zi ? zi->add_intercept : 0};
+  if (in_lds) {
     BLMM_HIP(hipFuncSetAttribute(reinterpret_cast<const void*>(&k_post_eigen<true>), hipFuncAttributeMaxDynamicSharedMemorySize, (int)lds));
     BLMM_LAUNCH_STOP(ctx, (k_post_eigen<true>), dim3(1), dim3(1024), lds, lraw, V, n, pa, stat);
   } else {
@@ -1356,15 +1364,62 @@
   int* fin;
 };
 
-template <int C, int LPT, bool REG>
+template <int LPT>
+__device__ __forceinline__ void rotate_own_traits(const BrentRot& rt, int n, int64_t m, int64_t ldy) {
+  constexpr int TPW = 256 / LPT, NCB = TPW / 16, NRG = 4 / NCB;
+  constexpr int MB = NRG == 1 ? 5 : 4;
+  static_assert(TPW % 16 == 0 && NCB * NRG == 4, "whole MFMA column blocks per workgroup");
+  const int lane = threadIdx.x & 63, wave = threadIdx.x >> 6, kk = lane >> 4;
+  const int64_t col = (int64_t)blockIdx.x * TPW + (wave % NCB) * 16 + (lane & 15);
+  const int npad = rt.npad, ldr = rt.ldr, nrb = (npad + 15) / 16;
+  const bool colok = col < m;
+  const double* pin = rt.Y + (colok ? col : 0) * (int64_t)n;
+  for (int rb0 = (wave / NCB) * MB; rb0 < nrb; rb0 += NRG * MB) {
+    d4 acc[MB];
+#pragma unroll
+    for (int b = 0; b < MB; ++b) acc[b] = (d4){0, 0, 0, 0};
+    for (int i0 = 0; i0 < npad; i0 += 16) {
+      double bv[4], av[4][MB];
+#pragma unroll
+      for (int u = 0; u < 4; ++u) {
+        const int i = i0 + 4 * u + kk;
+        bv[u] = (colok && i < n) ? pin[i] : 0.0;
+        const double* pr = rt.Rp + (size_t)(i < npad ? i : 0) * ldr + (lane & 15);
+#pragma unroll
+        for (int b = 0; b < MB; ++b) {
+          const int r0 = (rb0 + b) * 16;
+          av[u][b] = (r0 < ldr && i < npad) ? pr[r0] : 0.0;
+        }
+      }
+#pragma unroll
+      for (int u = 0; u < 4; ++u)
+#pragma unroll
+        for (int b = 0; b < MB; ++b) acc[b] = __builtin_amdgcn_mfma_f64_16x16x4f64(av[u][b], bv[u], acc[b], 0, 0, 0);
+    }
+    if (col < ldy) {
+#pragma unroll
+      for (int b = 0; b < MB; ++b)
+#pragma unroll
+        for (int r = 0; r < 4; ++r) {
+          const int row = (rb0 + b) * 16 + kk + 4 * r;
+          if (row < npad) rt.Yt[(int64_t)row * ldy + col] = acc[b][r];
+        }
+    }
+  }
+}
+bool brent_can_rotate(int n, int c) { return c >= 1 && c <= 3 && n <= 128; }
+
+template <int C, int LPT, bool REG, bool ROT = false>
 __global__ void __launch_bounds__(256, BRENT_MINW) k_brent(NullModel nm, const double* __restrict__ Yt, int64_t ldy, int64_t m,
                                                const double* __restrict__ Z0, const double* __restrict__ lam,
                                                const double* __restrict__ logtab, double* __restrict__ h2out,
                                                double* __restrict__ s2out, double* __restrict__ ellout, int64_t* stat,
-                                               BrentCont cont) {
+                                               BrentCont cont, BrentRot rt) {
+  static_assert(!ROT || REG, "the fused rotation stages from the workgroup's own columns");
   extern __shared__ __attribute__((aligned(16))) double sh[];
   __shared__ dpair s_ln[BLMM_LOG_TABLE_N];
   const int n = nm.n;
+  if constexpr (ROT) rotate_own_traits<LPT>(rt, n, m, ldy);
   double* sLam = sh;
   double* sZ = sh + n;
   if (!REG) {
@@ -1378,13 +1433,21 @@
   const int64_t j = ((int64_t)blockIdx.x * blockDim.x + threadIdx.x) / LPT;
   const int sub = threadIdx.x % LPT;
   const bool valid = j < m;
-  const double* ycol = Yt + (valid ? j : 0);
+  const double* ycol = ROT ? nullptr : Yt + (valid ? j : 0);
   int nonpos = 0, hit_max = 0;
   const int nint = nm.optim_interval < 1 ? 1 : nm.optim_interval;
   double best_x;
   EllOut fin;
   double* sY = sh + LPT * NULL_NK * (1 + C);
-  if constexpr (REG) {
+  if constexpr (ROT) {
+    const double* yc = rt.Yt + (valid ? j : 0);
+#pragma unroll
+    for (int i = 0; i < NULL_NK; ++i) {
+      const int k = sub + LPT * i;
+      sY[i * 256 + threadIdx.x] = (k < n && valid) ? yc[(int64_t)k * ldy] : 0.0;
+    }
+    __syncthreads();
+  } else if constexpr (REG) {
     stage_null_y<LPT>(sY, ycol, ldy, sub, n, valid);
     __syncthreads();
   }
@@ -1527,8 +1590,12 @@
 
 template <int C, int LPT, bool REG>
 static int launch_brent_t(blmm_ctx* ctx, const NullModel& nm, const double* Yt, int64_t ldy, int64_t m, const double* Z0,
-                          const double* lam, double* h2, double* sigma2, double* ell, int64_t* stat, int phase, BrentSplit* sp) {
-  const int64_t threads = m * LPT;
+                          const double* lam, double* h2, double* sigma2, double* ell, int64_t* stat, int phase, BrentSplit* sp,
+                          const BrentRot* rot) {
+  constexpr bool CAN_ROT = REG && C <= 3 && LPT <= 16;
+  if (rot && phase != 2 && (!CAN_ROT || !brent_can_rotate(nm.n, C) || ldy % (256 / LPT) != 0))
+    return fail(ctx, BLMM_ERR_UNSUPPORTED, "launch_brent: no fused rotation for this shape");
+  const int64_t threads = (rot && phase != 2 ? ldy : m) * LPT;
   const unsigned blocks = (unsigned)((threads + 255) / 256);
   const size_t lds = REG ? sizeof(double) * ((size_t)LPT * NULL_NK * (1 + C) + (size_t)NULL_NK * 256) : sizeof(double) * (size_t)nm.n * (1 + C);
   if (lds > 48 * 1024)
@@ -1551,8 +1618,16 @@
   }
   if (sp) { sp->active = two && phase == 1; sp->fin = cont.fin; sp->list = cont.list; sp->cnt = cont.cnt; }
   if (phase != 2) {
-    hipLaunchKernelGGL((k_brent<C, LPT, REG>), dim3(blocks), dim3(256), lds, ctx->stream, nm, Yt, ldy, m, Z0, lam,
-                       ptr<double>(ctx->logtab), h2, sigma2, ell, stat, cont);
+    if constexpr (CAN_ROT) {
+      if (rot) {
+        if (lds > 48 * 1024)
+          BLMM_HIP(hipFuncSetAttribute(reinterpret_cast<const void*>(&k_brent<C, LPT, REG, true>), hipFuncAttributeMaxDynamicSharedMemorySize, (int)lds));
+        hipLaunchKernelGGL((k_brent<C, LPT, REG, true>), dim3(blocks), dim3(256), lds, ctx->stream, nm, (const double*)nullptr, ldy, m,
+                           Z0, lam, ptr<double>(ctx->logtab), h2, sigma2, ell, stat, cont, *rot);
+      }
+    }
+    if (!rot) hipLaunchKernelGGL((k_brent<C, LPT, REG>), dim3(blocks), dim3(256), lds, ctx->stream, nm, Yt, ldy, m, Z0, lam,
+                                 ptr<double>(ctx->logtab), h2, sigma2, ell, stat, cont, BrentRot{});
     KCHECK();
   }
   if (phase == 1 && two) return BLMM_OK;
@@ -1582,31 +1657,34 @@
 
 template <int C>
 static int launch_brent_c(blmm_ctx* ctx, const NullModel& nm, const double* Yt, int64_t ldy, int64_t m, const double* Z0,
-                          const double* lam, double* h2, double* sigma2, double* ell, int64_t* stat, int phase, BrentSplit* sp) {
+                          const double* lam, double* h2, double* sigma2, double* ell, int64_t* stat, int phase, BrentSplit* sp,
+                          const BrentRot* rot) {
   const int n = nm.n;
   static const int lpt_env = dev_env("BLMM_BRENT_LPT") ? atoi(dev_env("BLMM_BRENT_LPT")) : 0;
-  if (lpt_env == 8 && n <= 8 * NULL_NK) return launch_brent_t<C, 8, true>(ctx, nm, Yt, ldy, m, Z0, lam, h2, sigma2, ell, stat, phase, sp);
-  if (lpt_env == 16 && n <= 16 * NULL_NK) return launch_brent_t<C, 16, true>(ctx, nm, Yt, ldy, m, Z0, lam, h2, sigma2, ell, stat, phase, sp);
-  if (n <= 4 * NULL_NK) return launch_brent_t<C, 4, true>(ctx, nm, Yt, ldy, m, Z0, lam, h2, sigma2, ell, stat, phase, sp);
-  if (n <= 8 * NULL_NK) return launch_brent_t<C, 8, true>(ctx, nm, Yt, ldy, m, Z0, lam, h2, sigma2, ell, stat, phase, sp);
-  if (n <= 16 * NULL_NK) return launch_brent_t<C, 16, true>(ctx, nm, Yt, ldy, m, Z0, lam, h2, sigma2, ell, stat, phase, sp);
-  if (n <= 32 * NULL_NK) return launch_brent_t<C, 32, true>(ctx, nm, Yt, ldy, m, Z0, lam, h2, sigma2, ell, stat, phase, sp);
-  if (n <= 64 * NULL_NK) return launch_brent_t<C, 64, true>(ctx, nm, Yt, ldy, m, Z0, lam, h2, sigma2, ell, stat, phase, sp);
-  return launch_brent_t<C, BRENT_LPT, false>(ctx, nm, Yt, ldy, m, Z0, lam, h2, sigma2, ell, stat, phase, sp);
+  if (lpt_env == 8 && n <= 8 * NULL_NK) return launch_brent_t<C, 8, true>(ctx, nm, Yt, ldy, m, Z0, lam, h2, sigma2, ell, stat, phase, sp, rot);
+  if (lpt_env == 16 && n <= 16 * NULL_NK) return launch_brent_t<C, 16, true>(ctx, nm, Yt, ldy, m, Z0, lam, h2, sigma2, ell, stat, phase, sp, rot);
+  if (n <= 4 * NULL_NK) return launch_brent_t<C, 4, true>(ctx, nm, Yt, ldy, m, Z0, lam, h2, sigma2, ell, stat, phase, sp, rot);
+  if (n <= 8 * NULL_NK) return launch_brent_t<C, 8, true>(ctx, nm, Yt, ldy, m, Z0, lam, h2, sigma2, ell, stat, phase, sp, rot);
+  if (n <= 16 * NULL_NK) return launch_brent_t<C, 16, true>(ctx, nm, Yt, ldy, m, Z0, lam, h2, sigma2, ell, stat, phase, sp, rot);
+  if (n <= 32 * NULL_NK) return launch_brent_t<C, 32, true>(ctx, nm, Yt, ldy, m, Z0, lam, h2, sigma2, ell, stat, phase, sp, rot);
+  if (n <= 64 * NULL_NK) return launch_brent_t<C, 64, true>(ctx, nm, Yt, ldy, m, Z0, lam, h2, sigma2, ell, stat, phase, sp, rot);
+  return launch_brent_t<C, BRENT_LPT, false>(ctx, nm, Yt, ldy, m, Z0, lam, h2, sigma2, ell, stat, phase, sp, rot);
 }
 
 int launch_brent(blmm_ctx* ctx, const NullModel& nm, const double* Yt, int64_t ldy, int64_t m, const double* Z0,
-                 const double* lam, double* h2, double* sigma2, double* ell, int64_t* stat, int phase, BrentSplit* sp) {
+                 const double* lam, double* h2, double* sigma2, double* ell, int64_t* stat, int phase, BrentSplit* sp,
+                 const BrentRot* rot) {
+  if (rot && !brent_can_rotate(nm.n, nm.c)) return fail(ctx, BLMM_ERR_UNSUPPORTED, "launch_brent: no fused rotation for this shape");
   if (nm.c > CTPL && nm.c <= CMAX) {
     if (sp) sp->active = false;
     return phase == 2 ? BLMM_OK : launch_dyn_brent(ctx, nm, Yt, ldy, m, Z0, lam, h2, sigma2, ell, stat);
   }
   switch (nm.c) {
-    case 1: return launch_brent_c<1>(ctx, nm, Yt, ldy, m, Z0, lam, h2, sigma2, ell, stat, phase, sp);
-    case 2: return launch_brent_c<2>(ctx, nm, Yt, ldy, m, Z0, lam, h2, sigma2, ell, stat, phase, sp);
-    case 3: return launch_brent_c<3>(ctx, nm, Yt, ldy, m, Z0, lam, h2, sigma2, ell, stat, phase, sp);
-    case 4: return launch_brent_c<4>(ctx, nm, Yt, ldy, m, Z0, lam, h2, sigma2, ell, stat, phase, sp);
-#define BG(C) return launch_brent_t<C, 16, false>(ctx, nm, Yt, ldy, m, Z0, lam, h2, sigma2, ell, stat, phase, sp)
+    case 1: return launch_brent_c<1>(ctx, nm, Yt, ldy, m, Z0, lam, h2, sigma2, ell, stat, phase, sp, rot);
+    case 2: return launch_brent_c<2>(ctx, nm, Yt, ldy, m, Z0, lam, h2, sigma2, ell, stat, phase, sp, rot);
+    case 3: return launch_brent_c<3>(ctx, nm, Yt, ldy, m, Z0, lam, h2, sigma2, ell, stat, phase, sp, rot);
+    case 4: return launch_brent_c<4>(ctx, nm, Yt, ldy, m, Z0, lam, h2, sigma2, ell, stat, phase, sp, rot);
+#define BG(C) return launch_brent_t<C, 16, false>(ctx, nm, Yt, ldy, m, Z0, lam, h2, sigma2, ell, stat, phase, sp, rot)
     case 5: BG(5);
     case 6: BG(6);
     case 7: BG(7);
```

Result: no change. 164.1 billion, median of 5 (+0.8%).
